# rvaser/rala

Hardware: AMD Instinct MI355X
Metric: overlaps/sec (pile build + transitive reduction) (higher is better)
Workload: dtype u16/u32 (+f64 compares)

## Files before the change

include/rala_hip.h:

```cpp
#ifndef RALA_HIP_H_
#define RALA_HIP_H_

#include <stddef.h>
#include <stdint.h>

#ifdef __cplusplus
extern "C" {
#endif

#define RALA_HIP_NO_READ 0xFFFFFFFFu

enum {
    RALA_HIP_OK = 0,
    RALA_HIP_EDEVICE = -1,
    RALA_HIP_EINVAL = -2,
    RALA_HIP_ECAPACITY = -3,
    RALA_HIP_EFILTERED = -4,
    RALA_HIP_ENOMEM = -5,
    RALA_HIP_ENOTAFILE = -6,
    RALA_HIP_ETOOLARGE = -7
};

enum { RALA_HIP_TYPE_X = 0, RALA_HIP_TYPE_A = 1, RALA_HIP_TYPE_B = 2, RALA_HIP_TYPE_AB = 3, RALA_HIP_TYPE_BA = 4 };

enum { RALA_HIP_MEM_HOST = 0, RALA_HIP_MEM_DEVICE = 1, RALA_HIP_MEM_HOST_ASYNC = 2 };

typedef struct rala_hip_ctx rala_hip_ctx;

typedef struct rala_hip_overlaps {
    const uint32_t* a_id;
    const uint32_t* b_id;
    const uint32_t* a_begin;
    const uint32_t* a_end;
    const uint32_t* b_begin;
    const uint32_t* b_end;
    const uint32_t* length;
    const uint8_t* strand;
} rala_hip_overlaps;

typedef struct rala_hip_timings {
    float dedupe_ms, bucket_ms, pile_ms, classify_ms, death_ms, finish_ms, tail_host_ms, tr_ms, total_ms;
    uint32_t pile_launches, death_rounds, pile_overflow_reads, pile_position_reads;
    uint32_t pile_unbounded_reads, pool_regrown;
    float repeats_ms;
} rala_hip_timings;

int rala_hip_create(int device, rala_hip_ctx** out);
void rala_hip_destroy(rala_hip_ctx* ctx);
const char* rala_hip_last_error(const rala_hip_ctx* ctx);
int rala_hip_set_option(rala_hip_ctx* ctx, const char* key, int64_t value);
void* rala_hip_stream(rala_hip_ctx* ctx);

int rala_hip_set_reads(rala_hip_ctx* ctx, const uint32_t* read_len, uint64_t n_reads);
int rala_hip_set_overlaps(rala_hip_ctx* ctx, const rala_hip_overlaps* ovl, uint64_t n, int mem);

typedef struct rala_hip_ingest_timings {
    float ship_ms;
    float tokenize_ms;
    uint64_t bytes, lines;
} rala_hip_ingest_timings;
int rala_hip_set_name_table(rala_hip_ctx* ctx, const void* buckets, uint64_t n_buckets, const char* arena, uint64_t arena_bytes);
int rala_hip_set_overlaps_from_paf(rala_hip_ctx* ctx, const char* path, int check_lengths, uint32_t threads,
                                   int64_t* length_error_read, int* irregular);
int rala_hip_set_overlaps_from_mhap(rala_hip_ctx* ctx, const char* path, int check_lengths, uint32_t threads,
                                    int64_t* length_error_read, int* irregular);
int rala_hip_get_ingest_timings(rala_hip_ctx* ctx, rala_hip_ingest_timings* out);
typedef struct rala_hip_inflate_timings {
    float inflate_ms;
    uint64_t compressed_bytes;
    uint64_t members;
} rala_hip_inflate_timings;
int rala_hip_get_inflate_timings(rala_hip_ctx* ctx, rala_hip_inflate_timings* out);
typedef struct rala_hip_gzip_timings {
    float find_ms;
    float decode_ms;
    float resolve_ms;
    uint64_t compressed_bytes;
    uint64_t text_bytes;
    uint64_t chunks;
    uint64_t chunks_with_candidate;
    uint64_t chunks_confirmed;
    uint64_t chunks_refuted;
    uint64_t max_wave_text_bytes;
} rala_hip_gzip_timings;
int rala_hip_get_gzip_timings(rala_hip_ctx* ctx, rala_hip_gzip_timings* out);
int rala_hip_gzip_head(const uint8_t* bytes, uint64_t n, uint64_t* deflate_off, int* valid);
int rala_hip_gzip_chain(const uint64_t* starts, const uint64_t* end_bit, const uint64_t* text, const uint32_t* next,
                        const uint32_t* status, const uint32_t* refuted, uint64_t n_chunks, uint64_t end, uint32_t isize, uint64_t cap,
                        uint64_t* n_jobs, uint64_t* start_bit, uint64_t* stop_bit, uint64_t* text_off, uint64_t* text_n,
                        rala_hip_gzip_timings* stats, int* valid);
int rala_hip_gzip_chain_members(const uint64_t* starts, const uint64_t* end_bit, const uint64_t* text, const uint32_t* next,
                                const uint32_t* status, const uint32_t* refuted, uint64_t n_chunks, const uint64_t* cand_header_off,
                                const uint64_t* cand_deflate_bit, const uint32_t* cand_prev_crc, const uint32_t* cand_prev_isize,
                                const uint64_t* cand_end_bit, const uint64_t* cand_text, const uint32_t* cand_next,
                                const uint32_t* cand_status, uint64_t n_cands, uint64_t file_n, uint32_t last_crc, uint32_t last_isize,
                                uint64_t cap, uint64_t* n_jobs, uint64_t* start_bit, uint64_t* stop_bit, uint64_t* text_off,
                                uint64_t* text_n, uint32_t* first, uint64_t member_cap, uint64_t* n_members, uint64_t* member_text_off,
                                uint64_t* member_text_n, uint32_t* member_crc32, rala_hip_gzip_timings* stats, int* valid);
int rala_hip_gzip_find_members(rala_hip_ctx* ctx, const uint8_t* bytes, uint64_t n, uint64_t cap, uint64_t* n_found, uint64_t* header_off,
                               uint64_t* deflate_off);
int rala_hip_get_gzip_members(rala_hip_ctx* ctx, uint64_t* n, uint64_t cap, uint64_t* text_off, uint64_t* text_n, uint32_t* crc32);
int rala_hip_bgzf_index(const uint8_t* bytes, uint64_t n, uint64_t block_bytes, uint64_t cap, uint64_t* n_members, uint64_t* file_off,
                        uint32_t* comp_bytes, uint32_t* text_bytes, uint64_t* text_off, int* valid);
int rala_hip_bgzf_index_range(const uint8_t* bytes, uint64_t n, uint64_t lo, uint64_t hi, uint64_t block_bytes, uint64_t cap,
                              uint64_t* n_members, uint64_t* file_off, uint32_t* comp_bytes, uint32_t* text_bytes, uint64_t* begin,
                              uint64_t* end, int* empty, int* valid);
int rala_hip_bgzf_pieces_chain(const uint64_t* begin, const uint64_t* end, const int* empty, uint32_t n_pieces, uint64_t file_bytes);
int rala_hip_index_sequences(rala_hip_ctx* ctx, const char* path, int format, uint32_t threads, uint64_t* n_records,
                             uint64_t* name_bytes, int* irregular);
int rala_hip_get_sequence_index(rala_hip_ctx* ctx, uint64_t* name_off, uint32_t* name_len, uint64_t* data_off,
                                uint64_t* data_span, uint32_t* length, char* names);
int rala_hip_get_sequence_timings(rala_hip_ctx* ctx, rala_hip_ingest_timings* out);
int rala_hip_build_name_table(rala_hip_ctx* ctx, uint64_t* n_buckets, uint64_t* n_distinct);
int rala_hip_get_name_table(rala_hip_ctx* ctx, void* buckets, char* arena, uint64_t* n_buckets, uint64_t* arena_bytes);
int rala_hip_copy_name_table(rala_hip_ctx* dst, rala_hip_ctx* src);
uint64_t rala_hip_name_hash(const char* p, uint64_t n);
typedef struct rala_hip_name_table_info {
    uint64_t names;
    uint64_t distinct;
    uint64_t n_buckets;
    uint32_t longest_probe;
    float device_ms;
} rala_hip_name_table_info;
int rala_hip_get_name_table_info(rala_hip_ctx* ctx, rala_hip_name_table_info* out);
int rala_hip_slice_sequences(rala_hip_ctx* ctx, const char* path, const uint64_t* wanted, uint64_t n_wanted, const uint64_t* base_off,
                             uint8_t* bases, uint32_t threads, int* irregular);
typedef struct rala_hip_sequence_slice_info {
    uint64_t windows;
    uint64_t max_window_text_bytes;
    uint64_t bases;
    float ship_ms;
    float kernel_ms;
    float gather_ms;
    float copy_ms;
} rala_hip_sequence_slice_info;
int rala_hip_get_sequence_slice_info(rala_hip_ctx* ctx, rala_hip_sequence_slice_info* out);
int rala_hip_set_bases(rala_hip_ctx* ctx, const uint8_t* bases, const uint64_t* base_off, uint64_t n_sources, int mem);
typedef struct rala_hip_span {
    uint32_t source, first, len, rc;
} rala_hip_span;
int rala_hip_spell(rala_hip_ctx* ctx, const rala_hip_span* spans, uint64_t n_spans, uint8_t* out, uint64_t out_bytes);
typedef struct rala_hip_spell_info {
    uint64_t sources, source_bytes;
    uint64_t spans, bytes;
    uint64_t windows, launches;
    float upload_ms;
    float kernel_ms;
    float copy_ms;
    uint32_t from_slice;
} rala_hip_spell_info;
int rala_hip_get_spell_info(rala_hip_ctx* ctx, rala_hip_spell_info* out);
uint32_t rala_hip_crc32_chain(const uint32_t* reg, const uint64_t* len, uint64_t n);
int rala_hip_tokenise_sensitive_paf(rala_hip_ctx* ctx, const char* path, uint64_t lo, uint64_t hi, uint32_t threads,
                                    rala_hip_overlaps* out, uint64_t* n, int* irregular);
int rala_hip_tokenise_sensitive(rala_hip_ctx* ctx, const char* path, int format, uint32_t part, uint32_t parts, uint32_t threads,
                                rala_hip_overlaps* out, uint64_t* n, uint64_t piece[3], int* irregular);
int rala_hip_get_overlap_columns(rala_hip_ctx* ctx, uint64_t* n, uint32_t* const cols[7], uint8_t* strand);

int rala_hip_initialize(rala_hip_ctx* ctx);
int rala_hip_construct(rala_hip_ctx* ctx, const rala_hip_overlaps* sens, uint64_t n_sens);
int rala_hip_find_repetitive_hills(rala_hip_ctx* ctx, uint64_t read, uint32_t begin, uint32_t end, uint16_t median,
                                   uint16_t p10, uint16_t dataset_median);
int rala_hip_remove_transitive_edges(rala_hip_ctx* ctx, uint32_t* n_pairs);
int rala_hip_tr_mark(rala_hip_ctx* ctx, uint32_t n_nodes, uint32_t n_edges, const uint32_t* src,
                     const uint32_t* dst, const uint32_t* len, uint8_t* marks, uint32_t* n_pairs);

int rala_hip_dedupe(rala_hip_ctx* ctx);
int rala_hip_emit_bound_tuples(rala_hip_ctx* ctx, uint64_t* tuples_dev);
int rala_hip_emit_bound_tuples_bucketed(rala_hip_ctx* ctx, uint32_t world, uint64_t* tuples_dev, uint64_t* counts);
int rala_hip_set_bound_tuples(rala_hip_ctx* ctx, const uint64_t* tuples, uint64_t n, int mem);
int rala_hip_bound_records_fit(const rala_hip_ctx* ctx, uint32_t world);
int rala_hip_emit_bound_records_bucketed(rala_hip_ctx* ctx, uint32_t world, uint64_t* records_dev, uint64_t* counts);
int rala_hip_set_bound_records(rala_hip_ctx* ctx, const uint64_t* records, uint64_t n, int mem);
int rala_hip_import_state(rala_hip_ctx* ctx, const uint8_t* valid, const uint32_t* begin, const uint32_t* end,
                          const uint16_t* median, const uint16_t* p10, const uint8_t* alive,
                          const uint64_t* pits_off, const uint32_t* pits_pairs, const uint32_t* pits_aux,
                          const uint64_t* hills_off, const uint32_t* hills_pairs);

typedef struct rala_hip_device_state {
    const uint32_t* begin;
    const uint32_t* end;
    const uint16_t* median;
    const uint16_t* p10;
    const uint8_t* alive;
    const uint32_t* n_pits;
    const uint32_t* n_hills;
    const uint32_t* slot;
    const void* pool;
    uint64_t pool_count;
    const uint8_t* valid;
} rala_hip_device_state;
int rala_hip_get_device_state(rala_hip_ctx* ctx, rala_hip_device_state* out);
int rala_hip_copy_device_state(rala_hip_ctx* ctx, const rala_hip_device_state* dst);
int rala_hip_import_state_device(rala_hip_ctx* ctx, const rala_hip_device_state* in);

enum { RALA_HIP_COMM_RCCL = 0, RALA_HIP_COMM_LOCAL = 1 };
typedef struct rala_hip_mg rala_hip_mg;
typedef struct rala_hip_mg_timings {
// ... 66 lines not shown
```

rala_amd/csrc/bucket_kernels.hip:

```cpp
#include <hip/hip_runtime.h>

#include <algorithm>

#include "device_utils.h"
#include "geom.h"
#include "kernels.h"
#include "scan_pass.h"

namespace rala_hip {

namespace {

constexpr uint32_t kInf = 0xFFFFFFFFu;
constexpr uint32_t kTile = 4096;
constexpr uint32_t kBlockP = 512;
constexpr uint32_t kPer = kTile / kBlockP;
constexpr uint32_t kL1Shift = 12;
constexpr uint32_t kL1Reads = 1u << kL1Shift;
constexpr uint32_t kGroupShift = 7;
constexpr uint32_t kGroupReads = 1u << kGroupShift;
constexpr uint32_t kGroupsPerPart = kL1Reads / kGroupReads;
constexpr uint32_t kKeyBits = 14;
constexpr uint32_t kCoordBits = 25;
constexpr uint32_t kCoordMax = (1u << kCoordBits) - 1u;
static_assert(kKeyBits + 2 * kCoordBits == 64, "a record is 8 bytes");

struct PartGeom {
    uint32_t shift, gpp, n_part;
};
inline PartGeom part_geom(uint32_t n_reads, const BucketTuning& bt) {
    uint32_t shift = kL1Shift;
    while (shift < kKeyBits && ((uint64_t)n_reads + (1u << shift) - 1) >> shift > 256) ++shift;
    if (bt.part_shift >= kL1Shift && bt.part_shift <= kKeyBits) shift = bt.part_shift;
    return PartGeom{shift, 1u << (shift - kGroupShift), (uint32_t)(((uint64_t)n_reads + (1u << shift) - 1) >> shift)};
}

constexpr uint32_t kCountWindow = 150u * 1024u / 4u;
inline uint32_t count_window(const BucketTuning& bt) { return bt.count_window ? bt.count_window : kCountWindow; }

__device__ __forceinline__ uint64_t pack_record(uint32_t b, uint32_t begin, uint32_t end) {
    return (uint64_t)(b & ((1u << kKeyBits) - 1u)) << (2 * kCoordBits) | (uint64_t)(begin < kCoordMax ? begin : kCoordMax) << kCoordBits |
           (uint64_t)(end < kCoordMax ? end : kCoordMax);
}
__device__ __forceinline__ uint32_t rec_key(uint64_t r) { return (uint32_t)(r >> (2 * kCoordBits)); }
__device__ __forceinline__ uint2 rec_events(uint64_t r, uint32_t shrink) {
    const uint32_t begin = (uint32_t)(r >> kCoordBits) & kCoordMax, end = (uint32_t)r & kCoordMax;
    return make_uint2((begin + shrink) << 1, ((end - shrink) << 1) | 1u);
}

__device__ __forceinline__ uint32_t segment_of(uint32_t key, bool active, uint32_t lane, uint32_t& leader) {
    const uint32_t prev = (uint32_t)__shfl_up((int)key, 1, 64);
    const bool prev_active = __shfl_up((int)active, 1, 64) != 0;
    const bool head = active && (lane == 0 || !prev_active || prev != key);
    const uint64_t heads = __ballot(head);
    const uint64_t act = __ballot(active);
    const uint64_t below = heads & ((lane == 63) ? ~0ull : ((2ull << lane) - 1ull));
    leader = below ? 63u - (uint32_t)__clzll((long long)below) : lane;
    const uint64_t after = (lane == 63) ? 0ull : ((heads | ~act) >> (lane + 1));
    const uint32_t len = after ? (uint32_t)__ffsll((unsigned long long)after) : (64u - lane);
    return head ? len : 0u;
}

constexpr uint32_t kBlockC = 1024;
constexpr uint32_t kCountPer = 8;
__global__ __launch_bounds__(kBlockC) void group_count_kernel(OvlSoA o, uint32_t n_reads, uint32_t g_lo, uint32_t n_groups, uint32_t* group_count) {
    extern __shared__ uint32_t s_hist[];
    for (uint32_t g = threadIdx.x; g < n_groups; g += kBlockC) s_hist[g] = 0;
    __syncthreads();
    constexpr uint32_t kC = kCountPer;
    const uint64_t last = o.n - 1;
    for (uint64_t i0 = (uint64_t)blockIdx.x * kBlockC * kC; i0 < o.n; i0 += (uint64_t)gridDim.x * kBlockC * kC) {
        uint32_t a[kC], b[kC];
#pragma unroll
        for (uint32_t u = 0; u < kC; ++u) {
            const uint64_t i = i0 + u * kBlockC + threadIdx.x;
            const uint64_t j = i < o.n ? i : last;
            a[u] = i < o.n ? __builtin_nontemporal_load(o.a_id + j) : kInf;
            b[u] = __builtin_nontemporal_load(o.b_id + j);
        }
#pragma unroll
        for (uint32_t u = 0; u < kC; ++u) {
            const uint32_t g = (b[u] >> kGroupShift) - g_lo;
            if (a[u] < n_reads && b[u] < n_reads && g < n_groups) atomicAdd(&s_hist[g], 1u);
        }
    }
    __syncthreads();
    for (uint32_t g = threadIdx.x; g < n_groups; g += kBlockC) {
        const uint32_t c = s_hist[g];
        if (c) atomicAdd(&group_count[g_lo + g], c);
    }
}

__device__ __forceinline__ void load4_ids(const uint32_t* p, uint64_t i0, uint64_t n, uint32_t (&out)[4]) {
    typedef uint32_t u32x4_t __attribute__((ext_vector_type(4)));
    if (i0 + 4 <= n) {
        const u32x4_t v = __builtin_nontemporal_load((const u32x4_t*)(p + i0));
        out[0] = v.x; out[1] = v.y; out[2] = v.z; out[3] = v.w;
    } else {
#pragma unroll
        for (uint32_t e = 0; e < 4; ++e) out[e] = i0 + e < n ? p[i0 + e] : kInf;
    }
}
constexpr uint32_t kCountVec = 2;
constexpr uint32_t kFlagStage = 512;
template <bool kShard>
__global__ __launch_bounds__(kBlockC) void group_count_dedupe_kernel(OvlSoA o, uint32_t n_reads, uint32_t n_groups, uint32_t* group_count,
                                                                     uint8_t* __restrict__ suspect, uint8_t* __restrict__ valid, uint32_t* list_pos,
                                                                     uint32_t* list_query, uint32_t list_cap, uint32_t* list_count,
                                                                     uint32_t world, uint32_t groups) {
    extern __shared__ uint32_t s_hist[];
    __shared__ uint32_t s_fpos[kFlagStage], s_fq[kFlagStage], s_fcnt, s_fbase;
    for (uint32_t g = threadIdx.x; g < n_groups; g += kBlockC) s_hist[g] = 0;
    if (threadIdx.x == 0) s_fcnt = 0;
    __syncthreads();
    const uint32_t lane = threadIdx.x & 63;
    auto mark = [&](uint32_t query, uint64_t at) {
        suspect[query] = 1;
        const uint32_t slot = atomicAdd(&s_fcnt, 1u);
        if (slot < kFlagStage) { s_fpos[slot] = (uint32_t)at; s_fq[slot] = query; }
    };
    constexpr uint64_t kTrip = (uint64_t)kBlockC * 4 * kCountVec;
    for (uint64_t c0 = (uint64_t)blockIdx.x * kTrip; c0 < o.n; c0 += (uint64_t)gridDim.x * kTrip) {
        uint32_t a[kCountVec][4], b[kCountVec][4];
#pragma unroll
        for (uint32_t u = 0; u < kCountVec; ++u) {
            const uint64_t i0 = c0 + ((uint64_t)u * kBlockC + threadIdx.x) * 4;
            load4_ids(o.a_id, i0, o.n, a[u]);
            load4_ids(o.b_id, i0, o.n, b[u]);
        }
#pragma unroll
        for (uint32_t u = 0; u < kCountVec; ++u) {
            const uint64_t i0 = c0 + ((uint64_t)u * kBlockC + threadIdx.x) * 4;
            uint32_t pa = (uint32_t)__shfl_up((int)a[u][3], 1, 64), pb = (uint32_t)__shfl_up((int)b[u][3], 1, 64);
            if (lane == 0 && i0 > 0 && i0 < o.n) { pa = o.a_id[i0 - 1]; pb = o.b_id[i0 - 1]; }
            bool have_prev = i0 > 0;
            uint32_t word = 0;
#pragma unroll
            for (uint32_t e = 0; e < 4; ++e) {
                const uint32_t x = a[u][e], y = b[u][e];
                const bool in = i0 + e < o.n;
                const bool ok = in && x < n_reads && y < n_reads;
                if (ok) {
                    if constexpr (kShard) {
                        atomicAdd(&s_hist[(x % world) * groups + ((x / world) >> kGroupShift)], 1u);
                        atomicAdd(&s_hist[(y % world) * groups + ((y / world) >> kGroupShift)], 1u);
                    } else {
                        if ((y >> kGroupShift) < n_groups) atomicAdd(&s_hist[y >> kGroupShift], 1u);
                    }
                }
                if (in && have_prev) {
                    const bool pok = pa < n_reads && pb < n_reads;
                    if (ok && pok) {
                        if (pa == x && y <= pb) mark(x, i0 + e);
                    } else {
                        if (x < n_reads) mark(x, i0 + e);
                        if (pa < n_reads) mark(pa, i0 + e - 1);
                    }
                }
                if (ok && x != y) word |= 1u << (8 * e);
                pa = x; pb = y; have_prev = true;
            }
            if (i0 + 4 <= o.n) *(uint32_t*)(valid + i0) = word;
            else for (uint32_t e = 0; e < 4 && i0 + e < o.n; ++e) valid[i0 + e] = (uint8_t)(word >> (8 * e));
        }
        __syncthreads();
        const uint32_t staged = s_fcnt;
        if (staged) {
            if (threadIdx.x == 0) s_fbase = staged > kFlagStage ? atomicOr(list_count, kDedupeListGivenUp) : atomicAdd(list_count, staged);
            __syncthreads();
            if (staged <= kFlagStage) {
                for (uint32_t k = threadIdx.x; k < staged; k += kBlockC) {
                    const uint32_t at = s_fbase + k;
                    if (at < list_cap) { list_pos[at] = s_fpos[k]; list_query[at] = s_fq[k]; }
                }
            }
            __syncthreads();
            if (threadIdx.x == 0) s_fcnt = 0;
            __syncthreads();
        }
    }
    for (uint32_t g = threadIdx.x; g < n_groups; g += kBlockC) {
        const uint32_t c = s_hist[g];
        if (c) atomicAdd(&group_count[g], c);
    }
}

__global__ __launch_bounds__(1024) void layout_kernel(const uint32_t* __restrict__ group_count, uint32_t n_part, uint32_t gpp,
                                                      uint32_t* __restrict__ group_base, uint32_t* __restrict__ group_cursor,
                                                      uint32_t* __restrict__ part_cursor, uint32_t* __restrict__ tile_part,
                                                      uint32_t* __restrict__ tile_lo, uint32_t* __restrict__ tile_hi, uint32_t* n_tiles) {
    __shared__ uint32_t tmp[1024 / 64 + 1];
    const uint32_t n = n_part * gpp;
    uint32_t carry = 0;
    for (uint32_t g0 = 0; g0 < n; g0 += 1024) {
        const uint32_t g = g0 + threadIdx.x;
        const uint32_t c = g < n ? group_count[g] : 0u;
        uint32_t tot;
        const uint32_t ex = block_scan_excl<1024>(c, OpAdd(), 0u, tmp, tot);
        if (g < n) {
            group_base[g] = carry + ex;
            group_cursor[g] = carry + ex;
            if (g % gpp == 0) part_cursor[g / gpp] = carry + ex;
        }
        carry += tot;
    }
    if (threadIdx.x == 0) group_base[n] = carry;
    __syncthreads();
    uint32_t tile_carry = 0;
    for (uint32_t p0 = 0; p0 < n_part; p0 += 1024) {
        const uint32_t p = p0 + threadIdx.x;
        const uint32_t lo = p < n_part ? group_base[p * gpp] : 0u;
        const uint32_t hi = p < n_part ? group_base[(p + 1u) * gpp] : 0u;
        const uint32_t tiles = (hi - lo + kTile - 1) / kTile;
        uint32_t ttot;
        const uint32_t tex = block_scan_excl<1024>(tiles, OpAdd(), 0u, tmp, ttot);
        for (uint32_t k = 0; k < tiles; ++k) {
            tile_part[tile_carry + tex + k] = p;
            tile_lo[tile_carry + tex + k] = lo + k * kTile;
            tile_hi[tile_carry + tex + k] = umin(hi, lo + (k + 1u) * kTile);
        }
        tile_carry += ttot;
    }
    if (threadIdx.x == 0) *n_tiles = tile_carry;
}

struct StageLds {
    uint64_t* stage;
    uint16_t* bin_of;
    uint32_t *hist, *off, *gbase;
    __device__ StageLds(unsigned char* base, uint32_t n_bins) {
        stage = (uint64_t*)base;
        bin_of = (uint16_t*)(stage + kTile);
        hist = (uint32_t*)(bin_of + kTile);
        off = hist + n_bins;
        gbase = off + n_bins;
    }
};
inline size_t stage_lds_bytes(uint32_t n_bins) { return (size_t)kTile * 10 + (size_t)n_bins * 12 + 16; }

__device__ __forceinline__ void stage_and_copy(StageLds& L, uint32_t n_bins, const uint64_t* rec, const uint32_t* bin, const bool* in,
                                               uint32_t* cursor, uint64_t* __restrict__ out, uint32_t* tmp) {
    for (uint32_t p = threadIdx.x; p < n_bins; p += kBlockP) L.hist[p] = 0;
    __syncthreads();
    uint32_t rank[kPer];
#pragma unroll
    for (uint32_t u = 0; u < kPer; ++u) rank[u] = in[u] ? atomicAdd(&L.hist[bin[u]], 1u) : 0u;
    __syncthreads();
    uint32_t carry = 0;
    for (uint32_t p0 = 0; p0 < n_bins; p0 += kBlockP) {
        const uint32_t p = p0 + threadIdx.x;
        const uint32_t c = p < n_bins ? L.hist[p] : 0u;
        uint32_t tot;
        const uint32_t ex = block_scan_excl<(int)kBlockP>(c, OpAdd(), 0u, tmp, tot);
        if (p < n_bins) {
            L.off[p] = carry + ex;
            L.gbase[p] = c ? atomicAdd(&cursor[p], c) : 0u;
        }
        carry += tot;
    }
    __syncthreads();
    const uint32_t total = carry;
#pragma unroll
    for (uint32_t u = 0; u < kPer; ++u) {
        if (in[u]) {
            const uint32_t at = L.off[bin[u]] + rank[u];
            L.stage[at] = rec[u];
            L.bin_of[at] = (uint16_t)bin[u];
        }
    }
    __syncthreads();
    for (uint32_t j = threadIdx.x; j < total; j += kBlockP) {
        const uint32_t p = L.bin_of[j];
        out[L.gbase[p] + (j - L.off[p])] = L.stage[j];
    }
}

__global__ __launch_bounds__(kBlockP) void l1_scatter_kernel(OvlSoA o, uint32_t n_reads, uint32_t n_part, uint32_t shift, uint32_t* part_cursor,
                                                             uint64_t* __restrict__ rec1, uint32_t* acount) {
    extern __shared__ __align__(16) unsigned char s_raw[];
    __shared__ uint32_t tmp[kBlockP / 64 + 1];
    StageLds L(s_raw, n_part);
    uint64_t rec[kPer];
    uint32_t bin[kPer];
    bool in[kPer];
    const uint32_t lane = threadIdx.x & 63;
    const uint64_t last = o.n - 1;
#pragma unroll
    for (uint32_t u = 0; u < kPer; ++u) {
        const uint64_t i = (uint64_t)blockIdx.x * kTile + u * kBlockP + threadIdx.x;
        const uint64_t j = i < o.n ? i : last;
        const uint32_t a = o.a_id[j], b = o.b_id[j];
        in[u] = i < o.n && a < n_reads && b < n_reads;
        rec[u] = pack_record(b, o.b_begin[j], o.b_end[j]);
        bin[u] = in[u] ? b >> shift : 0u;
        uint32_t leader;
        const uint32_t seg = segment_of(a, in[u], lane, leader);
        if (seg) atomicAdd(&acount[a], seg);
    }
    stage_and_copy(L, n_part, rec, bin, in, part_cursor, rec1, tmp);
}

__device__ __forceinline__ uint32_t bound_record_read(uint64_t r) { return (uint32_t)(r >> (2 * kBoundRecordCoordBits)); }

__global__ __launch_bounds__(kBlockC) void group_count_records_kernel(const uint64_t* __restrict__ records, uint64_t n, uint32_t n_reads,
                                                                      uint32_t g_lo, uint32_t n_groups, uint32_t* group_count) {
    extern __shared__ uint32_t s_hist[];
    for (uint32_t g = threadIdx.x; g < n_groups; g += kBlockC) s_hist[g] = 0;
    __syncthreads();
    constexpr uint32_t kC = kCountPer;
    for (uint64_t i0 = (uint64_t)blockIdx.x * kBlockC * kC; i0 < n; i0 += (uint64_t)gridDim.x * kBlockC * kC) {
        uint32_t key[kC];
#pragma unroll
        for (uint32_t u = 0; u < kC; ++u) {
            const uint64_t i = i0 + u * kBlockC + threadIdx.x;
            key[u] = i < n ? bound_record_read(__builtin_nontemporal_load(records + i)) : kInf;
        }
#pragma unroll
        for (uint32_t u = 0; u < kC; ++u) {
            const uint32_t g = (key[u] >> kGroupShift) - g_lo;
            if (key[u] < n_reads && g < n_groups) atomicAdd(&s_hist[g], 1u);
        }
    }
    __syncthreads();
    for (uint32_t g = threadIdx.x; g < n_groups; g += kBlockC) {
        const uint32_t c = s_hist[g];
        if (c) atomicAdd(&group_count[g_lo + g], c);
    }
}

__global__ __launch_bounds__(kBlockP) void l1_scatter_records_kernel(const uint64_t* __restrict__ records, uint64_t n, uint32_t n_reads,
                                                                     uint32_t n_part, uint32_t shift, uint32_t* part_cursor, uint64_t* __restrict__ rec1) {
    extern __shared__ __align__(16) unsigned char s_raw[];
    __shared__ uint32_t tmp[kBlockP / 64 + 1];
    StageLds L(s_raw, n_part);
    uint64_t rec[kPer];
    uint32_t bin[kPer];
    bool in[kPer];
    constexpr uint32_t kMask = (1u << kBoundRecordCoordBits) - 1u;
#pragma unroll
    for (uint32_t u = 0; u < kPer; ++u) {
        const uint64_t i = (uint64_t)blockIdx.x * kTile + u * kBlockP + threadIdx.x;
        const uint64_t r = i < n ? __builtin_nontemporal_load(records + i) : ~0ull;
        const uint32_t key = bound_record_read(r);
        in[u] = i < n && key < n_reads;
        rec[u] = pack_record(key, (uint32_t)(r >> kBoundRecordCoordBits) & kMask, (uint32_t)r & kMask);
        bin[u] = in[u] ? key >> shift : 0u;
    }
    stage_and_copy(L, n_part, rec, bin, in, part_cursor, rec1, tmp);
}

constexpr uint32_t kTileOtherBase = 0x80000000u;
__global__ __launch_bounds__(kBlockP) void l2_scatter_kernel(const uint64_t* __restrict__ rec1, const uint64_t* __restrict__ rec1b,
                                                             const uint32_t* __restrict__ tile_part,
                                                             const uint32_t* __restrict__ tile_lo, const uint32_t* __restrict__ tile_hi,
                                                             const uint32_t* __restrict__ n_tiles, uint32_t* group_cursor,
                                                             uint64_t* __restrict__ rec2, uint32_t gpp) {
    extern __shared__ __align__(16) unsigned char s_raw[];
    __shared__ uint32_t tmp[kBlockP / 64 + 1];
    if (blockIdx.x >= *n_tiles) return;
    StageLds L(s_raw, gpp);
    const uint32_t part_mask = gpp * kGroupReads - 1u;
    const uint32_t part_word = tile_part[blockIdx.x], lo = tile_lo[blockIdx.x], hi = tile_hi[blockIdx.x];
    const uint32_t part = part_word & ~kTileOtherBase;
    const uint64_t* __restrict__ src = (part_word & kTileOtherBase) ? rec1b : rec1;
    uint64_t rec[kPer];
    uint32_t bin[kPer];
    bool in[kPer];
#pragma unroll
    for (uint32_t u = 0; u < kPer; ++u) {
        const uint32_t j = lo + u * kBlockP + threadIdx.x;
        in[u] = j < hi;
        rec[u] = in[u] ? src[j] : 0ull;
        bin[u] = (rec_key(rec[u]) & part_mask) >> kGroupShift;
    }
    stage_and_copy(L, gpp, rec, bin, in, group_cursor + part * gpp, rec2, tmp);
}

__global__ __launch_bounds__(kGroupReads) void group_query_sum_kernel(const uint32_t* __restrict__ acount, uint32_t n_reads,
                                                                      uint32_t* __restrict__ qsum) {
    __shared__ uint32_t tmp[kGroupReads / 64 + 1];
    const uint32_t r = blockIdx.x * kGroupReads + threadIdx.x;
    const uint32_t v = block_reduce<(int)kGroupReads>(r < n_reads ? acount[r] : 0u, OpAdd(), 0u, tmp);
    if (threadIdx.x == 0) qsum[blockIdx.x] = v;
}

__global__ __launch_bounds__(1024) void group_event_base_kernel(const uint32_t* __restrict__ qsum, const uint32_t* __restrict__ group_base,
                                                                uint32_t n_groups, uint32_t* __restrict__ pair_base) {
    __shared__ uint32_t tmp[1024 / 64 + 1];
    uint32_t carry = 0;
    for (uint32_t g0 = 0; g0 < n_groups; g0 += 1024) {
        const uint32_t g = g0 + threadIdx.x;
        const uint32_t c = g < n_groups ? qsum[g] + (group_base[g + 1] - group_base[g]) : 0u;
        uint32_t tot;
        const uint32_t ex = block_scan_excl<1024>(c, OpAdd(), 0u, tmp, tot);
        if (g < n_groups) pair_base[g] = carry + ex;
        carry += tot;
    }
    if (threadIdx.x == 0) pair_base[n_groups] = carry;
}

__global__ __launch_bounds__(kBlockP) void final_kernel(const uint64_t* __restrict__ rec2, const uint32_t* __restrict__ group_base,
                                                        const uint32_t* __restrict__ pair_base, uint32_t n_reads,
                                                        const uint32_t* __restrict__ acount, uint32_t* __restrict__ ev_off,
                                                        uint32_t* __restrict__ ev, uint32_t shrink, uint32_t ev_shift) {
    extern __shared__ __align__(16) unsigned char s_raw[];
    __shared__ uint32_t tmp[kBlockP / 64 + 1];
    __shared__ uint32_t s_cursor[kGroupReads];
    __shared__ uint32_t s_cnt[kGroupReads];
    static_assert(kGroupReads <= kBlockP, "one thread per read of the group");
    StageLds L(s_raw, kGroupReads);
    const uint32_t g = blockIdx.x;
    if (threadIdx.x < kGroupReads) s_cnt[threadIdx.x] = 0;
    __syncthreads();
    const uint32_t lo = group_base[g], hi = group_base[g + 1];
    uint64_t first[kPer];
#pragma unroll
    for (uint32_t u = 0; u < kPer; ++u) {
        const uint32_t j = lo + u * kBlockP + threadIdx.x;
        first[u] = j < hi ? rec2[j] : 0ull;
        if (j < hi) atomicAdd(&s_cnt[rec_key(first[u]) & (kGroupReads - 1u)], 1u);
    }
    for (uint32_t j = lo + kTile + threadIdx.x; j < hi; j += kBlockP) atomicAdd(&s_cnt[rec_key(rec2[j]) & (kGroupReads - 1u)], 1u);
    __syncthreads();
    {
        const uint32_t r = g * kGroupReads + threadIdx.x;
        const bool mine = threadIdx.x < kGroupReads && r < n_reads;
        const uint32_t q = mine && acount ? acount[r] : 0u;
        const uint32_t pairs = mine ? q + s_cnt[threadIdx.x] : 0u;
        uint32_t tot;
        const uint32_t before = pair_base[g] + block_scan_excl<(int)kBlockP>(pairs, OpAdd(), 0u, tmp, tot);
        if (mine) {
            ev_off[r] = before << (1u - ev_shift);
            s_cursor[threadIdx.x] = before + q;
            if (r == n_reads - 1u) ev_off[n_reads] = (before + pairs) << (1u - ev_shift);
        }
    }
    __syncthreads();
    for (uint32_t j0 = lo; j0 < hi; j0 += kTile) {
        uint64_t pair[kPer];
        uint32_t bin[kPer];
        bool in[kPer];
#pragma unroll
        for (uint32_t u = 0; u < kPer; ++u) {
            const uint32_t j = j0 + u * kBlockP + threadIdx.x;
            in[u] = j < hi;
            const uint64_t rec = j0 == lo ? first[u] : in[u] ? rec2[j] : 0ull;
            const uint2 e = rec_events(rec, shrink);
            pair[u] = (uint64_t)e.x | (uint64_t)e.y << 32;
            bin[u] = rec_key(rec) & (kGroupReads - 1u);
        }
        stage_and_copy(L, kGroupReads, pair, bin, in, s_cursor, (uint64_t*)ev, tmp);
        __syncthreads();
    }
}

template <uint32_t kQ>
__global__ __launch_bounds__(256) void query_side_kernel(OvlSoA o, uint32_t n_reads, const uint32_t* __restrict__ ev_off,
                                                         uint32_t* written, uint32_t* __restrict__ ev, uint32_t ev_shift) {
    const uint32_t lane = threadIdx.x & 63;
    uint32_t a[kQ], b[kQ], begin[kQ], end[kQ];
#pragma unroll
    for (uint32_t u = 0; u < kQ; ++u) {
        const uint64_t i = ((uint64_t)blockIdx.x * kQ + u) * 256 + threadIdx.x;
        a[u] = kInf; b[u] = kInf; begin[u] = 0; end[u] = 0;
        if (i < o.n) { a[u] = o.a_id[i]; b[u] = o.b_id[i]; begin[u] = __builtin_nontemporal_load(o.a_begin + i); end[u] = __builtin_nontemporal_load(o.a_end + i); }
    }
    uint32_t base[kQ], leader[kQ];
    bool ok[kQ];
#pragma unroll
    for (uint32_t u = 0; u < kQ; ++u) {
        ok[u] = a[u] < n_reads && b[u] < n_reads;
        const uint32_t seg = segment_of(a[u], ok[u], lane, leader[u]);
        base[u] = 0;
        if (seg) base[u] = ev_off[a[u]] + atomicAdd(&written[a[u]], (2u >> ev_shift) * seg);
    }
#pragma unroll
    for (uint32_t u = 0; u < kQ; ++u) {
        const uint32_t at = (uint32_t)__shfl((int)base[u], (int)leader[u], 64);
        if (ok[u]) *(uint2*)(ev + ((size_t)at << ev_shift) + 2u * (lane - leader[u])) = make_uint2((begin[u] + 15u) << 1, ((end[u] - 15u) << 1) | 1u);
    }
}


__global__ __launch_bounds__(kBlockC) void shard_count_kernel(OvlSoA o, uint32_t n_reads, uint32_t world, uint32_t groups,
                                                              uint32_t n_bins, uint32_t* group_count) {
    extern __shared__ uint32_t s_hist[];
    for (uint32_t g = threadIdx.x; g < n_bins; g += kBlockC) s_hist[g] = 0;
    __syncthreads();
    constexpr uint32_t kC = kCountPer;
    const uint64_t last = o.n - 1;
    for (uint64_t i0 = (uint64_t)blockIdx.x * kBlockC * kC; i0 < o.n; i0 += (uint64_t)gridDim.x * kBlockC * kC) {
        uint32_t a[kC], b[kC];
#pragma unroll
        for (uint32_t u = 0; u < kC; ++u) {
            const uint64_t i = i0 + u * kBlockC + threadIdx.x;
            const uint64_t j = i < o.n ? i : last;
            a[u] = i < o.n ? __builtin_nontemporal_load(o.a_id + j) : kInf;
            b[u] = __builtin_nontemporal_load(o.b_id + j);
        }
#pragma unroll
        for (uint32_t u = 0; u < kC; ++u) {
            if (a[u] < n_reads && b[u] < n_reads) {
                atomicAdd(&s_hist[(a[u] % world) * groups + ((a[u] / world) >> kGroupShift)], 1u);
                atomicAdd(&s_hist[(b[u] % world) * groups + ((b[u] / world) >> kGroupShift)], 1u);
            }
        }
    }
    __syncthreads();
    for (uint32_t g = threadIdx.x; g < n_bins; g += kBlockC) {
        const uint32_t c = s_hist[g];
        if (c) atomicAdd(&group_count[g], c);
    }
}

__global__ __launch_bounds__(1024) void shard_send_layout_kernel(const uint32_t* __restrict__ group_count, ShardGeometry g,
                                                                 uint64_t* __restrict__ send, uint32_t* __restrict__ part_cursor,
                                                                 uint32_t* __restrict__ send_words) {
    __shared__ uint32_t tmp[1024 / 64 + 1];
    uint32_t block_start = 0;
    for (uint32_t p = 0; p < g.world; ++p) {
        uint32_t* header = (uint32_t*)(send + block_start);
        uint32_t carry = block_start + g.header;
        for (uint32_t g0 = 0; g0 < g.groups; g0 += 1024) {
            const uint32_t k = g0 + threadIdx.x;
            const uint32_t c = k < g.groups ? group_count[p * g.groups + k] : 0u;
            uint32_t tot;
            const uint32_t ex = block_scan_excl<1024>(c, OpAdd(), 0u, tmp, tot);
            if (k < g.groups) {
                header[k] = c;
                if (k % kGroupsPerPart == 0) part_cursor[p * g.n_part + k / kGroupsPerPart] = carry + ex;
            }
            carry += tot;
        }
        if (threadIdx.x == 0) send_words[p] = carry - block_start;
        block_start = carry;
    }
}

__global__ __launch_bounds__(kBlockP) void shard_l1_scatter_kernel(OvlSoA o, uint32_t n_reads, uint32_t world, uint32_t n_part,
                                                                   uint32_t* part_cursor, uint64_t* __restrict__ send) {
    extern __shared__ __align__(16) unsigned char s_raw[];
    __shared__ uint32_t tmp[kBlockP / 64 + 1];
    const uint32_t n_bins = world * n_part;
    StageLds L(s_raw, n_bins);
    uint64_t rec[kPer];
    uint32_t bin[kPer];
    bool in[kPer];
    const uint64_t last = o.n - 1;
    static_assert(kPer % 2 == 0, "two records per overlap");
#pragma unroll
    for (uint32_t u = 0; u < kPer / 2; ++u) {
        const uint64_t i = (uint64_t)blockIdx.x * (kTile / 2) + u * kBlockP + threadIdx.x;
        const uint64_t j = i < o.n ? i : last;
        const uint32_t a = o.a_id[j], b = o.b_id[j];
        const bool ok = i < o.n && a < n_reads && b < n_reads;
        const uint32_t la = a / world, lb = b / world;
        in[2 * u] = in[2 * u + 1] = ok;
        rec[2 * u] = pack_record(la, __builtin_nontemporal_load(o.a_begin + j), __builtin_nontemporal_load(o.a_end + j));
        rec[2 * u + 1] = pack_record(lb, __builtin_nontemporal_load(o.b_begin + j), __builtin_nontemporal_load(o.b_end + j));
        bin[2 * u] = ok ? (a - la * world) * n_part + (la >> kL1Shift) : 0u;
        bin[2 * u + 1] = ok ? (b - lb * world) * n_part + (lb >> kL1Shift) : 0u;
    }
    stage_and_copy(L, n_bins, rec, bin, in, part_cursor, send, tmp);
}

__global__ __launch_bounds__(1024) void shard_owner_layout_kernel(const uint64_t* __restrict__ base, const uint64_t* __restrict__ base_self,
                                                                  ShardBlocks blocks, ShardGeometry g,
                                                                  uint32_t* __restrict__ group_base, uint32_t* __restrict__ group_cursor,
                                                                  uint32_t* __restrict__ pair_pref, uint32_t* __restrict__ tile_part,
                                                                  uint32_t* __restrict__ tile_lo, uint32_t* __restrict__ tile_hi,
                                                                  uint32_t* n_tiles) {
    __shared__ uint32_t tmp[1024 / 64 + 1];
    auto header_of = [&](uint32_t p) { return (const uint32_t*)((p == blocks.self ? base_self : base) + blocks.off[p]); };
    uint32_t carry = 0;
    for (uint32_t g0 = 0; g0 < g.groups; g0 += 1024) {
        const uint32_t k = g0 + threadIdx.x;
        uint32_t c = 0;
        if (k < g.groups) {
            for (uint32_t p = 0; p < g.world; ++p) c += header_of(p)[k];
        }
        uint32_t tot;
        const uint32_t ex = block_scan_excl<1024>(c, OpAdd(), 0u, tmp, tot);
        if (k < g.groups) { group_base[k] = carry + ex; group_cursor[k] = carry + ex; }
        carry += tot;
    }
    if (threadIdx.x == 0) group_base[g.groups] = carry;
    const uint32_t n_pairs = g.world * g.n_part;
    uint32_t pcarry = 0;
    for (uint32_t j0 = 0; j0 < n_pairs; j0 += 1024) {
        const uint32_t j = j0 + threadIdx.x;
        uint32_t len = 0;
        if (j < n_pairs) {
            const uint32_t* header = header_of(j / g.n_part) + (j % g.n_part) * kGroupsPerPart;
            for (uint32_t k = 0; k < kGroupsPerPart; ++k) len += header[k];
        }
        uint32_t tot;
        const uint32_t ex = block_scan_excl<1024>(len, OpAdd(), 0u, tmp, tot);
        if (j < n_pairs) pair_pref[j] = pcarry + ex;
        pcarry += tot;
    }
    if (threadIdx.x == 0) pair_pref[n_pairs] = pcarry;
    __syncthreads();
    uint32_t tile_carry = 0;
    for (uint32_t j0 = 0; j0 < n_pairs; j0 += 1024) {
        const uint32_t j = j0 + threadIdx.x;
        uint32_t lo = 0, len = 0, tiles = 0;
        if (j < n_pairs) {
            const uint32_t p = j / g.n_part;
            len = pair_pref[j + 1] - pair_pref[j];
            lo = blocks.off[p] + g.header + (pair_pref[j] - pair_pref[p * g.n_part]);
            tiles = (len + kTile - 1) / kTile;
        }
        uint32_t ttot;
        const uint32_t tex = block_scan_excl<1024>(tiles, OpAdd(), 0u, tmp, ttot);
        for (uint32_t k = 0; k < tiles; ++k) {
            tile_part[tile_carry + tex + k] = (j % g.n_part) | (j / g.n_part == blocks.self ? kTileOtherBase : 0u);
            tile_lo[tile_carry + tex + k] = lo + k * kTile;
            tile_hi[tile_carry + tex + k] = umin(lo + len, lo + (k + 1u) * kTile);
        }
        tile_carry += ttot;
    }
    if (threadIdx.x == 0) *n_tiles = tile_carry;
}

}

uint32_t partition_count(uint32_t n_reads, const BucketTuning& bt) { return part_geom(n_reads, bt).n_part; }
uint32_t partition_group_slots(uint32_t n_reads, const BucketTuning& bt) { const PartGeom G = part_geom(n_reads, bt); return G.n_part * G.gpp + 2; }
size_t partition_records_needed(uint32_t, uint64_t n_overlaps) { return (size_t)n_overlaps + 64; }
size_t partition_tile_slots(uint32_t n_reads, uint64_t n_overlaps, const BucketTuning& bt) { return (size_t)(n_overlaps / kTile) + partition_count(n_reads, bt) + 4; }
bool partition_path_fits(uint32_t n_reads, uint32_t max_read_len, uint64_t n_overlaps, const BucketTuning& bt) {
    if (n_reads == 0 || n_overlaps == 0) return false;
    const PartGeom G = part_geom(n_reads, bt);
    const uint64_t n_part = G.n_part;
    return max_read_len < kCoordMax - 32u && n_part * G.gpp <= 8ull * kCountWindow &&
           stage_lds_bytes((uint32_t)n_part) <= 60u * 1024u && 2ull * n_overlaps < 0xFFFFFFF0ull && n_overlaps / n_part >= 512;
}

namespace {
struct PartitionBuffers {
    uint32_t n_part, n_groups, group_slots, shift, gpp, window;
    size_t tile_slots;
    uint32_t *group_count, *group_base, *group_cursor, *tile_part, *tile_lo, *tile_hi, *n_tiles;
    PartitionBuffers(uint32_t n_reads, uint64_t n_records, const BucketTuning& bt, uint32_t* group, uint32_t* tiles) {
        const PartGeom G = part_geom(n_reads, bt);
        n_part = G.n_part; shift = G.shift; gpp = G.gpp;
        window = std::min(n_part * gpp, count_window(bt));
        n_groups = (n_reads + kGroupReads - 1) / kGroupReads;
        group_slots = partition_group_slots(n_reads, bt);
        tile_slots = partition_tile_slots(n_reads, n_records, bt);
        group_count = group; group_base = group + group_slots; group_cursor = group + 2 * (size_t)group_slots;
        tile_part = tiles; tile_lo = tiles + tile_slots; tile_hi = tiles + 2 * tile_slots; n_tiles = tiles + 3 * tile_slots;
    }
};

hipError_t count_attribute(size_t lds_count) {
    if (lds_count + 8192 > 64 * 1024) {
        hipError_t e = hipFuncSetAttribute((const void*)group_count_kernel, hipFuncAttributeMaxDynamicSharedMemorySize, (int)lds_count);
        if (e == hipSuccess) e = hipFuncSetAttribute((const void*)group_count_dedupe_kernel<false>, hipFuncAttributeMaxDynamicSharedMemorySize, (int)lds_count);
        if (e == hipSuccess) e = hipFuncSetAttribute((const void*)group_count_records_kernel, hipFuncAttributeMaxDynamicSharedMemorySize, (int)lds_count);
        return e;
    }
    return hipSuccess;
}

void launch_partition_rest(const PartitionBuffers& B, uint32_t n_reads, const uint32_t* acount, const uint64_t* rec1, uint64_t* rec2,
                           uint32_t* ev_off, uint32_t* ev, hipStream_t s, uint32_t ev_shift, uint32_t shrink = 15u) {
    const uint32_t tiles2 = (uint32_t)(B.tile_slots - 4);
    hipLaunchKernelGGL(l2_scatter_kernel, dim3(tiles2), dim3(kBlockP), stage_lds_bytes(B.gpp), s, rec1, (const uint64_t*)nullptr,
                       (const uint32_t*)B.tile_part, (const uint32_t*)B.tile_lo, (const uint32_t*)B.tile_hi, (const uint32_t*)B.n_tiles,
                       B.group_cursor, rec2, B.gpp);
    uint32_t *qsum = B.group_count, *pair_base = B.group_cursor;
    hipLaunchKernelGGL(group_query_sum_kernel, dim3(B.n_groups), dim3(kGroupReads), 0, s, acount, n_reads, qsum);
    hipLaunchKernelGGL(group_event_base_kernel, dim3(1), dim3(1024), 0, s, (const uint32_t*)qsum, (const uint32_t*)B.group_base, B.n_groups,
                       pair_base);
    hipLaunchKernelGGL(final_kernel, dim3(B.n_groups), dim3(kBlockP), stage_lds_bytes(kGroupReads), s, (const uint64_t*)rec2,
                       (const uint32_t*)B.group_base, (const uint32_t*)pair_base, n_reads, acount, ev_off, ev, shrink, ev_shift);
}
}

bool bucket_count_can_dedupe(const OvlSoA& o, const uint8_t* valid) {
    return (((uintptr_t)o.a_id | (uintptr_t)o.b_id) & 15u) == 0 && ((uintptr_t)valid & 3u) == 0 && getenv("RALA_DEDUPE_APART") == nullptr;
}

hipError_t launch_bucket_partitioned(const OvlSoA& o, uint32_t n_reads, const BucketTuning& bt, uint32_t* acount, uint32_t* written,
                                     uint32_t* part_cursor, uint32_t* group, uint32_t* tiles, uint64_t* rec1, uint64_t* rec2,
                                     uint32_t* ev_off, uint32_t* ev, uint32_t workgroups, FillList& fills, hipStream_t s,
                                     const BucketDedupe* dedupe, uint32_t ev_shift) {
    const PartitionBuffers B(n_reads, o.n, bt, group, tiles);
    fills.add(acount, 0, (size_t)n_reads * 4);
    fills.add(written, 0, (size_t)n_reads * 4);
    fills.add(B.group_count, 0, (size_t)B.group_slots * 4);
    if (dedupe) fills.add(dedupe->suspect, 0, n_reads);
    hipError_t e = fills.launch(s);
    if (e != hipSuccess) return e;
    const uint32_t all_groups = B.n_part * B.gpp, window = B.window;
    const size_t lds_count = (size_t)window * 4;
    e = count_attribute(lds_count);
    if (e != hipSuccess) return e;
    const uint32_t chunks = (uint32_t)((o.n + kBlockC * kCountPer - 1) / (kBlockC * kCountPer));
    auto wait_for = [&](hipEvent_t ev) { return dedupe && ev ? hipStreamWaitEvent(s, ev, 0) : hipSuccess; };
    e = wait_for(dedupe ? dedupe->ids : nullptr);
    if (e != hipSuccess) return e;
    const uint32_t count_groups = (workgroups ? workgroups : 256u) * (2 * lds_count <= 150u * 1024u ? 2u : 1u);
    if (dedupe) {
        hipLaunchKernelGGL(group_count_dedupe_kernel<false>, dim3(std::min<uint32_t>(count_groups, chunks)), dim3(kBlockC), lds_count, s, o,
                           n_reads, window, B.group_count, dedupe->suspect, dedupe->valid, dedupe->list_pos,
                           dedupe->list_query, dedupe->list_cap, dedupe->list_count, 1u, 0u);
        if (dedupe->counted) {
            e = hipEventRecord(dedupe->counted, s);
            if (e != hipSuccess) return e;
        }
    } else {
        hipLaunchKernelGGL(group_count_kernel, dim3(std::min<uint32_t>(count_groups, chunks)), dim3(kBlockC), lds_count, s, o,
                           n_reads, 0u, window, B.group_count);
    }
    for (uint32_t g_lo = window; g_lo < all_groups; g_lo += window) {
        hipLaunchKernelGGL(group_count_kernel, dim3(std::min<uint32_t>(count_groups, chunks)), dim3(kBlockC), lds_count, s, o,
                           n_reads, g_lo, std::min(window, all_groups - g_lo), B.group_count);
    }
    hipLaunchKernelGGL(layout_kernel, dim3(1), dim3(1024), 0, s, (const uint32_t*)B.group_count, B.n_part, B.gpp, B.group_base, B.group_cursor,
                       part_cursor, B.tile_part, B.tile_lo, B.tile_hi, B.n_tiles);
    const uint32_t tiles1 = (uint32_t)((o.n + kTile - 1) / kTile);
    e = wait_for(dedupe ? dedupe->b_coords : nullptr);
    if (e != hipSuccess) return e;
    hipLaunchKernelGGL(l1_scatter_kernel, dim3(tiles1), dim3(kBlockP), stage_lds_bytes(B.n_part), s, o, n_reads, B.n_part, B.shift, part_cursor, rec1,
                       acount);
    launch_partition_rest(B, n_reads, acount, rec1, rec2, ev_off, ev, s, ev_shift);
    e = wait_for(dedupe ? dedupe->a_coords : nullptr);
    if (e != hipSuccess) return e;
    static const int q_per = getenv("RALA_QUERY_PER") ? atoi(getenv("RALA_QUERY_PER")) : 2;
    if (q_per == 4) hipLaunchKernelGGL(query_side_kernel<4>, dim3((uint32_t)((o.n + 1023) / 1024)), dim3(256), 0, s, o, n_reads, (const uint32_t*)ev_off, written, ev, ev_shift);
    else if (q_per == 2) hipLaunchKernelGGL(query_side_kernel<2>, dim3((uint32_t)((o.n + 511) / 512)), dim3(256), 0, s, o, n_reads, (const uint32_t*)ev_off, written, ev, ev_shift);
    else hipLaunchKernelGGL(query_side_kernel<1>, dim3((uint32_t)((o.n + 255) / 256)), dim3(256), 0, s, o, n_reads, (const uint32_t*)ev_off, written, ev, ev_shift);
    return hipGetLastError();
}

hipError_t launch_bucket_partitioned_records(const uint64_t* records, uint64_t n, uint32_t n_reads, const BucketTuning& bt, uint32_t* zero_counts,
                                             uint32_t* part_cursor, uint32_t* group, uint32_t* tiles, uint64_t* rec1, uint64_t* rec2,
                                             uint32_t* ev_off, uint32_t* ev, uint32_t workgroups, FillList& fills, hipStream_t s,
                                             uint32_t shrink, uint32_t ev_shift) {
    const PartitionBuffers B(n_reads, n, bt, group, tiles);
    fills.add(zero_counts, 0, (size_t)n_reads * 4);
    fills.add(B.group_count, 0, (size_t)B.group_slots * 4);
    hipError_t e = fills.launch(s);
    if (e != hipSuccess) return e;
    const uint32_t all_groups = B.n_part * B.gpp, window = B.window;
    const size_t lds_count = (size_t)window * 4;
    e = count_attribute(lds_count);
    if (e != hipSuccess) return e;
    const uint32_t chunks = (uint32_t)((n + kBlockC * kCountPer - 1) / (kBlockC * kCountPer));
    const uint32_t count_groups = (workgroups ? workgroups : 256u) * (2 * lds_count <= 150u * 1024u ? 2u : 1u);
    for (uint32_t g_lo = 0; g_lo < all_groups; g_lo += window) {
        hipLaunchKernelGGL(group_count_records_kernel, dim3(std::min<uint32_t>(count_groups, std::max<uint32_t>(chunks, 1u))), dim3(kBlockC),
                           lds_count, s, records, n, n_reads, g_lo, std::min(window, all_groups - g_lo), B.group_count);
    }
    hipLaunchKernelGGL(layout_kernel, dim3(1), dim3(1024), 0, s, (const uint32_t*)B.group_count, B.n_part, B.gpp, B.group_base, B.group_cursor,
                       part_cursor, B.tile_part, B.tile_lo, B.tile_hi, B.n_tiles);
    const uint32_t tiles1 = (uint32_t)((n + kTile - 1) / kTile);
    if (tiles1) {
        hipLaunchKernelGGL(l1_scatter_records_kernel, dim3(tiles1), dim3(kBlockP), stage_lds_bytes(B.n_part), s, records, n, n_reads,
                           B.n_part, B.shift, part_cursor, rec1);
    }
    launch_partition_rest(B, n_reads, zero_counts, rec1, rec2, ev_off, ev, s, ev_shift, shrink);
    return hipGetLastError();
}

bool partition_path_fits_records(uint32_t n_reads, uint32_t max_read_len, uint64_t n_records, const BucketTuning& bt) {
    return max_read_len < (1u << kBoundRecordCoordBits) - 32u && partition_path_fits(n_reads, max_read_len, (n_records + 1) / 2, bt);
}

ShardGeometry shard_geometry(uint64_t n_reads, uint32_t world) {
    ShardGeometry g;
    g.world = world;
    const uint64_t most = (n_reads + world - 1) / world;
    g.n_part = (uint32_t)std::max<uint64_t>(1, (most + kL1Reads - 1) / kL1Reads);
    g.groups = g.n_part * kGroupsPerPart;
    g.header = g.groups / 2;
    return g;
}
bool shard_path_fits(uint64_t n_reads, uint32_t max_read_len, uint32_t world) {
    if (n_reads == 0 || world == 0 || world > 64 || n_reads >= 0x7FFFFFFFull) return false;
    const ShardGeometry g = shard_geometry(n_reads, world);
    return max_read_len < kCoordMax - 32u && (uint64_t)g.world * g.groups * 4u <= 150u * 1024u &&
           stage_lds_bytes(g.world * g.n_part) <= 60u * 1024u;
}
size_t shard_send_words(const ShardGeometry& g, uint64_t n_overlaps) { return 2 * (size_t)n_overlaps + (size_t)g.world * g.header + 64; }
size_t shard_tile_slots(const ShardGeometry& g, uint64_t n_records) { return (size_t)(n_records / kTile) + (size_t)g.world * g.n_part + 4; }

hipError_t launch_shard_emit(const OvlSoA& o, uint32_t n_reads, const ShardGeometry& g, uint32_t* group_count, uint32_t* part_cursor,
                             uint64_t* send, uint32_t* send_words, uint32_t workgroups, FillList& fills, hipStream_t s,
                             const BucketDedupe* dedupe) {
    const uint32_t n_bins = g.world * g.groups;
    fills.add(group_count, 0, (size_t)n_bins * 4);
    if (dedupe) fills.add(dedupe->suspect, 0, n_reads);
    hipError_t e = fills.launch(s);
    if (e != hipSuccess) return e;
    const size_t lds_count = (size_t)n_bins * 4;
    if (lds_count + 8192 > 64 * 1024) {
        e = hipFuncSetAttribute((const void*)shard_count_kernel, hipFuncAttributeMaxDynamicSharedMemorySize, (int)lds_count);
        if (e == hipSuccess) e = hipFuncSetAttribute((const void*)group_count_dedupe_kernel<true>, hipFuncAttributeMaxDynamicSharedMemorySize, (int)lds_count);
        if (e != hipSuccess) return e;
    }
    if (o.n) {
        const uint32_t chunks = (uint32_t)((o.n + kBlockC * kCountPer - 1) / (kBlockC * kCountPer));
        const uint32_t count_groups = (workgroups ? workgroups : 256u) * (2 * lds_count <= 150u * 1024u ? 2u : 1u);
        if (dedupe) {
            hipLaunchKernelGGL(group_count_dedupe_kernel<true>, dim3(std::min<uint32_t>(count_groups, chunks)), dim3(kBlockC), lds_count, s, o,
                               n_reads, n_bins, group_count, dedupe->suspect, dedupe->valid, dedupe->list_pos, dedupe->list_query,
                               dedupe->list_cap, dedupe->list_count, g.world, g.groups);
            if (dedupe->counted) {
                e = hipEventRecord(dedupe->counted, s);
                if (e != hipSuccess) return e;
            }
        } else {
            hipLaunchKernelGGL(shard_count_kernel, dim3(std::min<uint32_t>(count_groups, chunks)), dim3(kBlockC), lds_count, s, o, n_reads,
                               g.world, g.groups, n_bins, group_count);
        }
    }
    hipLaunchKernelGGL(shard_send_layout_kernel, dim3(1), dim3(1024), 0, s, (const uint32_t*)group_count, g, send, part_cursor, send_words);
    if (o.n) {
        const uint32_t tiles1 = (uint32_t)((o.n + kTile / 2 - 1) / (kTile / 2));
        hipLaunchKernelGGL(shard_l1_scatter_kernel, dim3(tiles1), dim3(kBlockP), stage_lds_bytes(g.world * g.n_part), s, o, n_reads, g.world,
                           g.n_part, part_cursor, send);
    }
    return hipGetLastError();
}

hipError_t launch_bucket_from_blocks(const uint64_t* base, const uint64_t* base_self, const ShardBlocks& blocks, const ShardGeometry& g,
                                     uint32_t n_reads_local,
                                     uint64_t n_records, uint32_t* group, uint32_t* tiles, uint64_t* rec2, uint32_t* ev_off, uint32_t* ev,
                                     FillList& fills, hipStream_t s, uint32_t ev_shift) {
    hipError_t e = fills.launch(s);
    if (e != hipSuccess) return e;
    const uint32_t slots = g.groups + 2;
    uint32_t *group_base = group, *group_cursor = group + slots, *pair_pref = group + 2 * (size_t)slots;
    const size_t tile_slots = shard_tile_slots(g, n_records);
    uint32_t *tile_part = tiles, *tile_lo = tiles + tile_slots, *tile_hi = tiles + 2 * tile_slots, *n_tiles = tiles + 3 * tile_slots;
    hipLaunchKernelGGL(shard_owner_layout_kernel, dim3(1), dim3(1024), 0, s, base, base_self, blocks, g, group_base, group_cursor, pair_pref, tile_part,
                       tile_lo, tile_hi, n_tiles);
    hipLaunchKernelGGL(l2_scatter_kernel, dim3((uint32_t)(tile_slots - 4)), dim3(kBlockP), stage_lds_bytes(kGroupsPerPart), s, base, base_self,
                       (const uint32_t*)tile_part, (const uint32_t*)tile_lo, (const uint32_t*)tile_hi, (const uint32_t*)n_tiles, group_cursor,
                       rec2, kGroupsPerPart);
    const uint32_t n_groups = (n_reads_local + kGroupReads - 1) / kGroupReads;
    if (n_groups) {
        hipLaunchKernelGGL(final_kernel, dim3(n_groups), dim3(kBlockP), stage_lds_bytes(kGroupReads), s, (const uint64_t*)rec2,
                           (const uint32_t*)group_base, (const uint32_t*)group_base, n_reads_local, (const uint32_t*)nullptr, ev_off, ev, 15u, ev_shift);
    }
    return hipGetLastError();
}
size_t shard_group_words(const ShardGeometry& g) { return 3 * ((size_t)g.groups + 2) + (size_t)g.world * g.n_part + 2; }

}
```

rala_amd/csrc/context.h:

```cpp
#pragma once

#include <hip/hip_runtime.h>
#include <stdint.h>

#include <algorithm>

#include <memory>
#include <string>
#include <vector>

#include "geom.h"
#include "host_pool.h"
#include "kernels.h"
#include "rala_hip.h"

namespace rala_hip {

struct HostOvl {
    uint32_t src;
    uint32_t a, b;
    Coords c;
    uint8_t strand;
    uint8_t dead;
    uint8_t type;
// ... 15 lines not shown
    size_t reserved = 0, chunk_size = 0;
    ~DevBuf() { release(); }
    void release() {
        if (reserved) {
            (void)hipDeviceSynchronize();
            for (size_t i = 0; i < chunks.size(); ++i) {
                if (mapped[i]) (void)hipMemUnmap(mapped[i], chunk_size);
                (void)hipMemRelease(chunks[i]);
            }
            chunks.clear();
            mapped.clear();
            reserved = 0;
            chunk_size = 0;
        } else if (p) {
            (void)hipFree(p);
        }
        p = nullptr;
        n = 0;
    }
    hipError_t ensure_chunked(size_t count, size_t chunk_bytes, int order, int device, int64_t fail_at = -1) {
        if (count <= n && p) return hipSuccess;
        release();
        hipMemAllocationProp prop = {};
        prop.type = hipMemAllocationTypePinned;
        prop.location.type = hipMemLocationTypeDevice;
        prop.location.id = device;
        size_t gran = 0;
        hipError_t e = hipMemGetAllocationGranularity(&gran, &prop, hipMemAllocationGranularityRecommended);
        if (e != hipSuccess) return e;
        if (gran == 0) gran = 2u << 20;
        chunk_bytes = (chunk_bytes + gran - 1) / gran * gran;
        const size_t n_chunks = (count * sizeof(T) + chunk_bytes - 1) / chunk_bytes;
        const size_t bytes = n_chunks * chunk_bytes;
        void* base = nullptr;
        e = hipMemAddressReserve(&base, bytes, 0, nullptr, 0);
        if (e != hipSuccess) return e;
        p = (T*)base;
        reserved = bytes;
        chunk_size = chunk_bytes;
        size_t stride = 1;
        if (order == 1 && n_chunks > 2) {
            stride = (size_t)((double)n_chunks * 0.6180339887) | 1u;
            auto gcd = [](size_t a, size_t b) { while (b) { const size_t t = a % b; a = b; b = t; } return a; };
            while (gcd(stride, n_chunks) != 1) stride += 2;
        }
        for (size_t i = 0; i < n_chunks && e == hipSuccess; ++i) {
            hipMemGenericAllocationHandle_t h;
            if (fail_at >= 0 && (size_t)fail_at == i) { e = hipErrorOutOfMemory; break; }
            e = hipMemCreate(&h, chunk_bytes, &prop, 0);
            if (e != hipSuccess) break;
            chunks.push_back(h);
            mapped.push_back(nullptr);
            void* at = (char*)base + ((i * stride) % n_chunks) * chunk_bytes;
            e = hipMemMap(at, chunk_bytes, 0, h, 0);
            if (e == hipSuccess) mapped.back() = at;
        }
        if (e == hipSuccess) {
            hipMemAccessDesc acc = {};
            acc.location = prop.location;
            acc.flags = hipMemAccessFlagsProtReadWrite;
            e = hipMemSetAccess(base, bytes, &acc, 1);
        }
        if (e != hipSuccess) { release(); return e; }
        n = bytes / sizeof(T);
        return hipSuccess;
    }
    hipError_t ensure(size_t count) {
        if (count <= n && p) return hipSuccess;
        release();
        if (count == 0) count = 1;
        hipError_t e = hipMalloc((void**)&p, count * sizeof(T));
        if (e == hipSuccess) n = count;
        return e;
    }
    hipError_t copy_to_host(void* dst, size_t first, size_t count) const {
        const char* src = (const char*)(p + first);
        size_t left = count * sizeof(T);
        while (left) {
            size_t take = left;
            if (chunk_size) take = std::min(left, chunk_size - (size_t)(src - (const char*)p) % chunk_size);
            const hipError_t e = hipMemcpy(dst, src, take, hipMemcpyDeviceToHost);
            if (e != hipSuccess) return e;
            dst = (char*)dst + take; src += take; left -= take;
        }
        return hipSuccess;
    }
    hipError_t grow(size_t keep, size_t count) {
        if (count <= n && p) return hipSuccess;
        T* q = nullptr;
        const size_t want = count + count / 4 + 1;
        hipError_t e = hipMalloc((void**)&q, want * sizeof(T));
        if (e != hipSuccess) return e;
        if (keep && p) e = hipMemcpy(q, p, keep * sizeof(T), hipMemcpyDeviceToDevice);
        if (e != hipSuccess) { (void)hipFree(q); return e; }
        if (p) (void)hipFree(p);
        p = q;
        n = want;
        return hipSuccess;
    }
};

template <class T>
struct PinnedBuf {
    T* p = nullptr;
    size_t n = 0;
    ~PinnedBuf() { release(); }
    void release() {
        if (p) (void)hipHostFree(p);
        p = nullptr;
        n = 0;
    }
    hipError_t ensure(size_t count) {
        if (count <= n && p) return hipSuccess;
        release();
        if (count == 0) count = 1;
        count += count / 4;
        hipError_t e = hipHostMalloc((void**)&p, count * sizeof(T), hipHostMallocDefault);
        if (e == hipSuccess) n = count;
        return e;
    }
};

}

struct rala_hip_ctx {
    int device = 0;
    uint32_t n_compute_units = 256;
    hipStream_t stream = nullptr;
    hipStream_t side = nullptr;
    hipStream_t aux = nullptr;
    bool use_side_stream = true;
    std::string err;
    hipEvent_t ev[12] = {};
    hipStream_t copy = nullptr;
    hipEvent_t ev_up[4] = {};
    bool upload_pending = false, upload_queued = false;
    const uint32_t* up_src[7] = {};
    const uint8_t* up_strand = nullptr;

    int64_t pool_per_read_x1000 = 1000;
    int64_t max_lds_read_len = 22000;
    int64_t debug_pile_stop_after = 99;
    int64_t host_threads = 0;
    std::unique_ptr<rala_hip::HostPool> pool;
    bool use_run_kernel = true;
    bool debug_fail_construct = false;
    uint32_t debug_pile_variant = 0;
    uint32_t debug_dedupe_list_cap = 0;
    uint32_t debug_fp_lds_limit = 0xFFFFFFFFu;
    uint32_t debug_fp_give_up = 0;
    int64_t debug_chunk_fail = -1;
    uint32_t debug_part_shift = 0;
    uint32_t debug_count_window = 0;
    bool use_bound_records = true;
    bool use_round_batches = true;
    rala_hip::DevBuf<uint32_t> d_round_log;

    uint64_t n_reads = 0;
    uint32_t max_read_len = 0;
    uint32_t n_class[rala_hip::kPileClasses] = {};
    rala_hip::DevBuf<uint32_t> d_class_order;
    rala_hip::DevBuf<uint32_t> d_seg_base;
    rala_hip::DevBuf<uint32_t> d_dense;
    std::vector<uint32_t> h_read_len;
    std::vector<uint64_t> h_pile_off;
    uint64_t pile_elems = 0;
    rala_hip::DevBuf<uint32_t> d_read_len;
    rala_hip::DevBuf<uint64_t> d_pile_off;
    rala_hip::DevBuf<uint16_t> d_pile;
    rala_hip::DevBuf<uint32_t> d_order, d_overflow;
    rala_hip::DevBuf<uint32_t> d_big_list[2], d_big_space;
    int64_t debug_big_caps = 0;
    bool debug_force_big = false;
    rala_hip::DevBuf<uint16_t> d_slab;
    std::vector<rala_hip::LaunchClass> classes;

    rala_hip::DevBuf<uint8_t> d_name_buckets, d_name_arena, d_paf_text, d_paf_strand;
    uint64_t n_name_buckets = 0, n_name_arena_bytes = 0;
    rala_hip::DevBuf<uint32_t> d_name_stats;
    hipEvent_t ev_names[2] = {};
    rala_hip_name_table_info name_table_info = {};
    rala_hip::DevBuf<uint32_t> d_paf_col[7], d_paf_chunk[2], d_paf_win[7];
    rala_hip::DevBuf<uint8_t> d_paf_win_strand;
    int64_t ingest_window_bytes = 0;
    rala_hip::DevBuf<unsigned long long> d_paf_bad;
    rala_hip_ingest_timings ingest_tm = {};
    rala_hip::DevBuf<uint8_t> d_bgzf_comp, d_bgzf_jobs;
    rala_hip::DevBuf<uint32_t> d_bgzf_flag;
    rala_hip_inflate_timings inflate_tm = {};
    bool gzip_on_device = false;
    bool gzip_members = false;
    bool bgzf_in_pieces = false;
    int64_t gzip_chunk_bytes = 64 << 10;
    uint32_t debug_gzip_false_sync = 0;
    rala_hip::DevBuf<uint64_t> d_gzip_starts, d_gzip_off, d_gzip_floor;
    rala_hip::DevBuf<uint8_t> d_gzip_spans, d_gzip_jobs, d_gzip_text;
    rala_hip::DevBuf<uint16_t> d_gzip_sym;
    rala_hip::DevBuf<uint32_t> d_gzip_crc;
    rala_hip::DevBuf<uint32_t> d_gzip_tile, d_gzip_piece_crc;
    rala_hip::DevBuf<uint8_t> d_gzip_cands, d_gzip_mspans, d_gzip_pieces;
    std::vector<rala_hip::GzipMember> gzip_members_last;
    rala_hip_gzip_timings gzip_tm = {};
    int64_t debug_sequence_window = 0;
    rala_hip::DevBuf<uint64_t> d_seq_event[2], d_seq_name_pos, d_seq_data_off, d_seq_data_stripped, d_seq_name_off, d_seq_span;
    rala_hip::DevBuf<uint32_t> d_seq_name_len, d_seq_length, d_seq_tile[2], d_seq_name_at, d_seq_flags;
    rala_hip::DevBuf<uint8_t> d_seq_arena;
    uint64_t n_seq_records = 0, n_seq_name_bytes = 0;
    bool seq_index_valid = false;
    rala_hip_ingest_timings seq_tm = {};
    int seq_source = 0;
    bool seq_fastq = false;
    uint64_t seq_file_n = 0, seq_text_n = 0, seq_n_stripped = 0;
    std::vector<rala_hip::GzipJob> seq_gzip_chain;
    std::vector<rala_hip::GzipMember> seq_gzip_members;
    uint32_t seq_gzip_crc = 0;
    rala_hip::DevBuf<uint16_t> d_gzip_carry;
    rala_hip::DevBuf<uint8_t> d_gzip_hold, d_slice_out;
    rala_hip::DevBuf<uint64_t> d_slice_w[3];
    rala_hip_sequence_slice_info slice_info = {};
    bool keep_bases = false;
    uint32_t spell_window_mb = 256;
    int64_t debug_spell_window = 0;
    rala_hip::DevBuf<uint8_t> d_bases, d_spell_out;
    rala_hip::DevBuf<uint64_t> d_base_off, d_spell_off;
    rala_hip::DevBuf<rala_hip_span> d_spell_spans;
    std::vector<uint64_t> h_base_off;
    uint64_t n_base_sources = 0;
    bool bases_from_slice = false;
    rala_hip_spell_info spell_info = {};

    uint64_t n_ovl = 0;
    rala_hip::OvlSoA ovl = {};
    rala_hip::DevBuf<uint32_t> d_ovl_u32[7];
    rala_hip::DevBuf<uint8_t> d_ovl_strand;
    rala_hip::DevBuf<uint8_t> d_valid, d_suspect;
    rala_hip::DevBuf<uint32_t> d_dedupe_list;
    bool valid_ready = false;
    bool inputs_set = false;

    bool tuple_mode = false;
    uint64_t n_tuples = 0;
    const uint2* tuples = nullptr;
    const uint64_t* records = nullptr;
    uint64_t n_records = 0;
    rala_hip::DevBuf<uint64_t> d_record;
    rala_hip::DevBuf<uint2> d_tuple;
    rala_hip::DevBuf<uint32_t> d_owner_cnt;
    bool piles_resident = false;
    bool use_fused_emit = true;
    rala_hip::DevBuf<uint32_t> d_shard_group, d_shard_part, d_shard_words, d_shard_tiles;
    bool dedupe_pending = false;
    bool lists_pending = false;
    bool blocks_mode = false;
    const uint64_t* blocks_base = nullptr;
    const uint64_t* blocks_base_self = nullptr;
    rala_hip::ShardBlocks blocks = {};
    rala_hip::ShardGeometry shard_geom = {};
    uint64_t n_block_records = 0;

    rala_hip::DevBuf<uint32_t> d_ev_off, d_cursor, d_ev, d_slot_rank[2], d_ev_fixed;
    uint32_t pile_chunk_mb = 1024;
    uint32_t pile_rows = 1;
    uint32_t pile_rows_scratch_mb = 256;
    bool rowless = false;
    bool sens_csr_ready = false;
    bool sens_pass_running = false;
    uint64_t rows_materialised = 0;
    rala_hip::DevBuf<uint16_t> d_rows_scratch;
    rala_hip::DevBuf<uint64_t> d_rows_off;
    rala_hip::DevBuf<uint32_t> d_rows_list;
    std::vector<uint64_t> h_rows_off;
    bool debug_ev_events = false;
    uint32_t ev_shift = 0;
    rala_hip::DevBuf<unsigned char> d_scan_ws;

    rala_hip::DevBuf<uint32_t> d_begin, d_end, d_iv_slot;
    rala_hip::DevBuf<uint16_t> d_median, d_p10;
    rala_hip::DevBuf<uint8_t> d_alive;
    rala_hip::DevBuf<uint32_t> d_n_pits, d_n_hills;
    rala_hip::DevBuf<rala_hip::Interval> d_pool;
    rala_hip::DevBuf<uint32_t> d_small;
    uint32_t pool_cap = 0;
    uint32_t pool_cap_first = 0;
    uint32_t rep_pool_cap = 0;

    rala_hip::DevBuf<uint8_t> d_cls;
    rala_hip::DevBuf<uint32_t> d_death[2];
    rala_hip::DevBuf<uint32_t> d_chunk[4];
    rala_hip::DevBuf<uint4> d_rec;
    rala_hip::DevBuf<uint8_t> d_crec;
    rala_hip::DevBuf<uint8_t> d_fate;
    rala_hip::DevBuf<uint64_t> d_scan_state;
    rala_hip::DevBuf<uint32_t> d_counts;
    rala_hip::DevBuf<uint32_t> d_surv_u32[8];
    rala_hip::DevBuf<uint8_t> d_surv_u8[2];
    rala_hip::DevBuf<uint8_t> d_list_block[2];
    rala_hip::PinnedBuf<uint32_t> p_surv_u32[8];
    rala_hip::PinnedBuf<uint8_t> p_surv_u8[2];

    bool initialized = false, constructed = false;
    uint64_t n_prefiltered = 0;
    std::vector<uint32_t> h_begin, h_end, h_slot;
    std::vector<uint16_t> h_median, h_p10;
    std::vector<uint8_t> h_alive;
    std::vector<uint32_t> h_n_pits, h_n_hills;
    std::vector<rala_hip::Interval> h_pool;
    rala_hip::DevBuf<uint32_t> d_overflow_mid, d_overflow_long, d_chain_cnt;
    bool ev_ready = false, ev_fixed = false;
    rala_hip::DevBuf<uint32_t> d_sens_off, d_sens_cur, d_sens_ev, d_sens_list, d_sens_split;
    rala_hip::DevBuf<double> d_layout[4];
    rala_hip::DevBuf<uint32_t> d_layout_adj[2];
    rala_hip::DevBuf<unsigned char> d_layout_batch;
    rala_hip::PinnedBuf<unsigned char> p_layout_batch;
    hipEvent_t ev_layout[2] = {};
    int64_t layout_fused_max = 1024;
    rala_hip_layout_info layout_info = {};
    struct StagedCopy { void* dst; size_t offset, bytes; };
    rala_hip::PinnedBuf<uint32_t> p_stage;
    std::vector<StagedCopy> stage_pending;
    size_t stage_used = 0;
    int64_t use_fixed_buckets = 1;
    bool use_partitioned_buckets = true;
    rala_hip::DevBuf<uint32_t> d_bk_u32[3], d_bk_part, d_bk_group, d_bk_tiles;
    rala_hip::DevBuf<uint64_t> d_bk_rec[2];
    bool host_state_fresh = false;
    uint32_t pool_used = 0;

    rala_hip::DevBuf<uint16_t> d_dataset_median;
    rala_hip::DevBuf<uint32_t> d_n_rep;
    rala_hip::DevBuf<uint32_t> d_sens_col[7], d_sens_tb[2], d_sens_c[5];
    rala_hip::DevBuf<uint2> d_sens_tuples, d_sens_part, d_sens_recv;
    rala_hip::DevBuf<uint64_t> d_sens_rec;
    rala_hip::DevBuf<uint8_t> d_gather[2];
    rala_hip::DevBuf<uint8_t> d_sens_strand, d_sens_state;
    bool sens_in_device = false;
    rala_hip::DevBuf<uint32_t> d_rep_slot;
    rala_hip::DevBuf<rala_hip::Interval> d_rep_pool;
    std::vector<uint32_t> h_n_rep;
    std::vector<uint32_t> h_rep_slot;
    std::vector<rala_hip::Interval> h_rep_pool;
    bool have_repeats = false;
    bool rep_host_stale = false;
    uint32_t n_rep_hills = 0;

    bool use_gpu_tail = true;
    bool tail_on_device = false;
    bool host_stale = false;
    bool marks_on_device = false;
    uint32_t t_n0 = 0, t_n1 = 0, t_rounds = 0, t_n_kept = 0, t_n_nodes = 0, t_n_edges = 0, t_n_alive = 0;
    size_t t_med_tmp = 0;
    rala_hip::DevBuf<uint8_t> d_t_state, d_t_round, d_dirty, d_touched;
    rala_hip::DevBuf<uint32_t> d_n_pits0;
    rala_hip::DevBuf<uint16_t> d_cmed;
    rala_hip::DevBuf<uint8_t> d_med_tmp;
    rala_hip::DevBuf<uint32_t> d_cc_flags;
    rala_hip::DevBuf<uint32_t> d_kill[3], d_kill2[3], d_kill_count, d_death_sure;
    rala_hip::DevBuf<uint32_t> d_rank, d_alive_reads, d_t_tmp[2], d_kept_item, d_dovetail, d_epos, d_node_rank,
        d_node_read, d_e[3], d_t_death[2], d_t_work[2], d_t_fin, d_fp_map, d_fp_pack;
    rala_hip::DevBuf<uint8_t> d_t_mark;
    rala_hip::PinnedBuf<uint32_t> p_alive_reads, p_sens_rest;
    rala_hip::PinnedBuf<uint8_t> p_touched;
    rala_hip::PinnedBuf<uint16_t> p_cmed;

    std::vector<uint8_t> dirty, ever_dirty;
    std::vector<uint32_t> dirty_list;
    rala_hip::DevBuf<uint32_t> d_cc_edges, d_cc_label;
    rala_hip::DevBuf<uint32_t> d_tr[7];
    rala_hip::DevBuf<uint8_t> d_tr_marks;
    std::vector<rala_hip::HostOvl> overlaps, internals, scratch_ovl;
    std::vector<rala_hip::EdgePair> scratch_ep;
    std::vector<uint8_t> scratch_has, scratch_touched;
    std::vector<uint32_t> h_n_pits0;
    std::vector<uint32_t> scratch_u32a, scratch_u32b, scratch_u32c, alive_rank, alive_reads;
    rala_hip::PinnedBuf<uint32_t> p_cc_edges, p_cc_label;
    std::vector<uint32_t> node_read;
    std::vector<uint32_t> e_src, e_dst, e_len;
    std::vector<uint8_t> e_mark;

    rala_hip_timings tm = {};
};
```

rala_amd/csrc/context.hip:

```cpp
#include <hip/hip_runtime.h>
#include <stdlib.h>
#include <string.h>

#include <algorithm>
#include <thread>

#include "ctx_check.h"
#include "lifecycle.h"
#include "scan_pass.h"
#include "slots.h"
#include "stages.h"

using namespace rala_hip;

namespace {

int bound_inputs_adopted(rala_hip_ctx* ctx, Inputs kind, uint64_t n_events) {
    HIPCHECK(ctx->d_ev.ensure(n_events + 8));
    HIPCHECK(ctx->d_scan_ws.ensure(scan_workspace_bytes(std::max<uint64_t>(n_events, ctx->n_reads) + 2)));
    ctx->n_tuples = n_events;
    inputs_adopted(ctx, kind);
    return RALA_HIP_OK;
}

// ... 8 lines not shown
    hipStream_t s = ctx->stream;
    ctx->tm = rala_hip_timings();
    ctx->overlaps.clear(); ctx->internals.clear();
    uint32_t small[kInstallSmallWords] = {};
    small[kSmallPoolCount] = (uint32_t)pool_count;
    HIPCHECK(hipMemcpyAsync(ctx->d_small.p, small, sizeof(small), hipMemcpyHostToDevice, s));
    HIPCHECK(ctx->d_cc_flags.ensure(kCcFlagsWords));
    HIPCHECK(hipMemsetAsync(ctx->d_cc_flags.p + kCcInstallDead, 0, 4, s));
    launch_count_zero_u8(ctx->d_alive.p, (uint32_t)ctx->n_reads, ctx->d_cc_flags.p + kCcInstallDead, s);
    uint32_t n_dead = 0;
    HIPCHECK(d2h_small(ctx, &n_dead, ctx->d_cc_flags.p + kCcInstallDead, 4, s));
    HIPCHECK(stream_sync(ctx, s));
    results_dropped(ctx);
    state_installed(ctx, n_dead, (uint32_t)pool_count, false, false, valid_ready);
    if (n_dead == ctx->n_reads) return fail(ctx, RALA_HIP_EFILTERED, "filtered all sequences");
    return RALA_HIP_OK;
}

}

hipError_t rala_hip::d2h_small(rala_hip_ctx* ctx, void* dst, const void* src, size_t bytes, hipStream_t s) {
    if (ctx->p_stage.ensure(256) != hipSuccess || ctx->stage_used + bytes > 256 * sizeof(uint32_t) ||
        ctx->stage_pending.size() >= 16) {
        return hipMemcpyAsync(dst, src, bytes, hipMemcpyDeviceToHost, s);
    }
    char* at = (char*)ctx->p_stage.p + ctx->stage_used;
    const hipError_t e = hipMemcpyAsync(at, src, bytes, hipMemcpyDeviceToHost, s);
    if (e != hipSuccess) return e;
    ctx->stage_pending.push_back({dst, ctx->stage_used, bytes});
    ctx->stage_used += (bytes + 7) & ~(size_t)7;
    return hipSuccess;
}

hipError_t rala_hip::stream_sync(rala_hip_ctx* ctx, hipStream_t s) {
    const hipError_t e = hipStreamSynchronize(s);
    if (e == hipSuccess) {
        for (const auto& c : ctx->stage_pending) memcpy(c.dst, (const char*)ctx->p_stage.p + c.offset, c.bytes);
    }
    ctx->stage_pending.clear();
    ctx->stage_used = 0;
    return e;
}

int rala_hip::flush_upload(rala_hip_ctx* ctx) {
    if (!ctx->upload_pending) return RALA_HIP_OK;
    for (int k = 0; k < 7; ++k) HIPCHECK(hipMemcpy(ctx->d_ovl_u32[k].p, ctx->up_src[k], (size_t)ctx->n_ovl * 4, hipMemcpyHostToDevice));
    HIPCHECK(hipMemcpy(ctx->d_ovl_strand.p, ctx->up_strand, ctx->n_ovl, hipMemcpyHostToDevice));
    upload_done(ctx);
    return RALA_HIP_OK;
}

int rala_hip::set_bound_blocks(rala_hip_ctx* ctx, const uint64_t* base, const uint64_t* base_self, const ShardBlocks& blocks,
                               const ShardGeometry& g, uint64_t n_records) {
    if (!ctx) return RALA_HIP_EINVAL;
    if (ctx->n_reads == 0) return fail(ctx, RALA_HIP_EINVAL, "no reads set");
    if (n_records >= 0x7FFFFFF0ull) return fail(ctx, RALA_HIP_EINVAL, "too many records");
    HIPCHECK(hipSetDevice(ctx->device));
    inputs_withdrawn(ctx);
    ctx->blocks_base = base; ctx->blocks_base_self = base_self; ctx->blocks = blocks; ctx->shard_geom = g;
    ctx->n_block_records = n_records;
    return bound_inputs_adopted(ctx, Inputs::kBlocks, 2 * n_records);
}

int rala_hip::install_read_state(rala_hip_ctx* ctx, uint64_t pool_count) {
    if (!ctx) return RALA_HIP_EINVAL;
    if (ctx->n_reads == 0) return fail(ctx, RALA_HIP_EINVAL, "no reads set");
    if (ctx->n_ovl && !ctx->valid_ready) return fail(ctx, RALA_HIP_EINVAL, "validity bits required (rala_hip_dedupe)");
    if (pool_count > ctx->pool_cap) return fail(ctx, RALA_HIP_ECAPACITY, "interval pool smaller than the installed state");
    HIPCHECK(hipSetDevice(ctx->device));
    { const int rcu = flush_upload(ctx); if (rcu != RALA_HIP_OK) return rcu; }
    return finish_install(ctx, pool_count, ctx->valid_ready);
}

extern "C" {

int rala_hip_create(int device, rala_hip_ctx** out) {
    if (!out) return RALA_HIP_EINVAL;
    *out = nullptr;
    int count = 0;
    if (hipGetDeviceCount(&count) != hipSuccess || count <= 0 || device < 0 || device >= count) return RALA_HIP_EDEVICE;
    if (hipSetDevice(device) != hipSuccess) return RALA_HIP_EDEVICE;
    rala_hip_ctx* ctx = new rala_hip_ctx;
    ctx->device = device;
    if (const char* mb = getenv("RALA_HIP_PILE_CHUNK_MB")) ctx->pile_chunk_mb = (uint32_t)std::max(0, atoi(mb));
    {
        hipDeviceProp_t prop;
        if (hipGetDeviceProperties(&prop, device) == hipSuccess && prop.multiProcessorCount > 0) {
            ctx->n_compute_units = (uint32_t)prop.multiProcessorCount;
        }
    }
    int prio_least = 0, prio_greatest = 0;
    (void)hipDeviceGetStreamPriorityRange(&prio_least, &prio_greatest);
    bool ok = hipStreamCreate(&ctx->stream) == hipSuccess &&
              hipStreamCreateWithPriority(&ctx->side, hipStreamDefault, prio_greatest) == hipSuccess &&
              hipStreamCreate(&ctx->aux) == hipSuccess;
    for (auto& e : ctx->ev) ok = ok && hipEventCreate(&e) == hipSuccess;
    static_assert(sizeof(ctx->ev) / sizeof(ctx->ev[0]) == kEvCount, "one event per name of slots.h");
    ok = ok && ctx->d_small.ensure(kSmallWords) == hipSuccess;
    if (!ok) {
        rala_hip_destroy(ctx);
        return RALA_HIP_EDEVICE;
    }
    ctx->pool.reset(new HostPool(std::min(16u, std::max(1u, std::thread::hardware_concurrency()))));
    *out = ctx;
    return RALA_HIP_OK;
}

void rala_hip_destroy(rala_hip_ctx* ctx) {
    if (!ctx) return;
    (void)hipSetDevice(ctx->device);
    ctx->stage_pending.clear();
    if (ctx->stream) (void)hipStreamSynchronize(ctx->stream);
    if (ctx->side) (void)hipStreamSynchronize(ctx->side);
    if (ctx->aux) (void)hipStreamSynchronize(ctx->aux);
    for (auto& e : ctx->ev) if (e) (void)hipEventDestroy(e);
    for (auto& e : ctx->ev_up) if (e) (void)hipEventDestroy(e);
    for (auto& e : ctx->ev_layout) if (e) (void)hipEventDestroy(e);
    for (auto& e : ctx->ev_names) if (e) (void)hipEventDestroy(e);
    if (ctx->copy) (void)hipStreamDestroy(ctx->copy);
    if (ctx->side) (void)hipStreamDestroy(ctx->side);
    if (ctx->aux) (void)hipStreamDestroy(ctx->aux);
    if (ctx->stream) (void)hipStreamDestroy(ctx->stream);
    delete ctx;
}

const char* rala_hip_last_error(const rala_hip_ctx* ctx) { return ctx ? ctx->err.c_str() : "no context"; }

int rala_hip_set_option(rala_hip_ctx* ctx, const char* key, int64_t value) {
    if (!ctx || !key) return RALA_HIP_EINVAL;
    if (!strcmp(key, "interval_pool_per_read_x1000")) { ctx->pool_per_read_x1000 = value; return RALA_HIP_OK; }
    if (!strcmp(key, "debug_big_caps")) { ctx->debug_big_caps = value; return RALA_HIP_OK; }
    if (!strcmp(key, "debug_force_big")) { ctx->debug_force_big = value != 0; return RALA_HIP_OK; }
    if (!strcmp(key, "max_lds_read_len")) { ctx->max_lds_read_len = value; return RALA_HIP_OK; }
    if (!strcmp(key, "debug_pile_stop_after")) { ctx->debug_pile_stop_after = value; return RALA_HIP_OK; }
    if (!strcmp(key, "use_run_kernel")) { ctx->use_run_kernel = value != 0; return RALA_HIP_OK; }
    if (!strcmp(key, "use_round_batches")) { ctx->use_round_batches = value != 0; return RALA_HIP_OK; }
    if (!strcmp(key, "use_bound_records")) { ctx->use_bound_records = value != 0; return RALA_HIP_OK; }
    if (!strcmp(key, "use_fused_emit")) { ctx->use_fused_emit = value != 0; return RALA_HIP_OK; }
    if (!strcmp(key, "ingest_window_bytes")) { ctx->ingest_window_bytes = std::max<int64_t>(0, value); return RALA_HIP_OK; }
    if (!strcmp(key, "debug_sequence_window")) { ctx->debug_sequence_window = std::max<int64_t>(0, value); return RALA_HIP_OK; }
    if (!strcmp(key, "gzip_on_device")) { ctx->gzip_on_device = value != 0; return RALA_HIP_OK; }
    if (!strcmp(key, "gzip_members")) { ctx->gzip_members = value != 0; return RALA_HIP_OK; }
    if (!strcmp(key, "bgzf_in_pieces")) { ctx->bgzf_in_pieces = value != 0; return RALA_HIP_OK; }
    if (!strcmp(key, "gzip_chunk_bytes")) { ctx->gzip_chunk_bytes = value > 0 ? value : 64 << 10; return RALA_HIP_OK; }
    if (!strcmp(key, "debug_gzip_false_sync")) { ctx->debug_gzip_false_sync = (uint32_t)std::max<int64_t>(0, value); return RALA_HIP_OK; }
    if (!strcmp(key, "pile_rows")) { ctx->pile_rows = value ? 1u : 0u; return RALA_HIP_OK; }
    if (!strcmp(key, "pile_rows_scratch_mb")) { ctx->pile_rows_scratch_mb = (uint32_t)std::max<int64_t>(0, std::min<int64_t>(value, 1 << 20)); return RALA_HIP_OK; }
    if (!strcmp(key, "keep_bases")) { ctx->keep_bases = value != 0; return RALA_HIP_OK; }
    if (!strcmp(key, "spell_window_mb")) { ctx->spell_window_mb = (uint32_t)std::max<int64_t>(0, std::min<int64_t>(value, 1 << 20)); return RALA_HIP_OK; }
    if (!strcmp(key, "debug_spell_window")) { ctx->debug_spell_window = std::max<int64_t>(0, value); return RALA_HIP_OK; }
    if (!strcmp(key, "pile_chunk_mb")) { ctx->pile_chunk_mb = (uint32_t)std::max<int64_t>(0, std::min<int64_t>(value, 1 << 20)); return RALA_HIP_OK; }
    if (!strcmp(key, "debug_ev_events")) { ctx->debug_ev_events = value != 0; return RALA_HIP_OK; }
    if (!strcmp(key, "debug_count_window")) { ctx->debug_count_window = (uint32_t)std::max<int64_t>(0, value); return RALA_HIP_OK; }
    if (!strcmp(key, "debug_part_shift")) { ctx->debug_part_shift = (uint32_t)std::max<int64_t>(0, value); return RALA_HIP_OK; }
    if (!strcmp(key, "debug_pile_variant")) { ctx->debug_pile_variant = (uint32_t)std::max<int64_t>(0, value); return RALA_HIP_OK; }
    if (!strcmp(key, "debug_dedupe_list_cap")) { ctx->debug_dedupe_list_cap = (uint32_t)std::max<int64_t>(0, value); return RALA_HIP_OK; }
    if (!strcmp(key, "debug_fp_lds_limit")) { ctx->debug_fp_lds_limit = (uint32_t)std::max<int64_t>(0, value); return RALA_HIP_OK; }
    if (!strcmp(key, "debug_fp_give_up")) { ctx->debug_fp_give_up = value == 2 ? 2u : value != 0 ? 1u : 0u; return RALA_HIP_OK; }
    if (!strcmp(key, "debug_chunk_fail")) { ctx->debug_chunk_fail = value; return RALA_HIP_OK; }
    if (!strcmp(key, "debug_fail_construct")) { ctx->debug_fail_construct = value != 0; return RALA_HIP_OK; }
    if (!strcmp(key, "use_gpu_tail")) { ctx->use_gpu_tail = value != 0; return RALA_HIP_OK; }
    if (!strcmp(key, "use_fixed_buckets")) { ctx->use_fixed_buckets = value != 0; return RALA_HIP_OK; }
    if (!strcmp(key, "use_partitioned_buckets")) { ctx->use_partitioned_buckets = value != 0; return RALA_HIP_OK; }
    if (!strcmp(key, "use_side_stream")) { ctx->use_side_stream = value != 0; return RALA_HIP_OK; }
    if (!strcmp(key, "sensitive_in_device_memory")) { ctx->sens_in_device = value != 0; return RALA_HIP_OK; }
    if (!strcmp(key, "layout_fused_max")) {
        if (value < 0 || value > 1024) return fail(ctx, RALA_HIP_EINVAL, "layout_fused_max: 0 .. 1024");
        ctx->layout_fused_max = value;
        return RALA_HIP_OK;
    }
    if (!strcmp(key, "host_threads")) {
        ctx->host_threads = value;
        ctx->pool.reset(new HostPool((unsigned)std::max<int64_t>(1, std::min<int64_t>(value, 256))));
        return RALA_HIP_OK;
    }
    return fail(ctx, RALA_HIP_EINVAL, "unknown option");
}

void* rala_hip_stream(rala_hip_ctx* ctx) { return ctx ? (void*)ctx->stream : nullptr; }

int rala_hip_set_reads(rala_hip_ctx* ctx, const uint32_t* read_len, uint64_t n_reads) {
    if (!ctx || (!read_len && n_reads)) return RALA_HIP_EINVAL;
    if (n_reads >= 0x7FFFFFFFull) return fail(ctx, RALA_HIP_EINVAL, "too many reads");
    HIPCHECK(hipSetDevice(ctx->device));
    HIPCHECK(hipStreamSynchronize(ctx->side));
    HIPCHECK(hipStreamSynchronize(ctx->aux));
    ctx->n_reads = n_reads;
    ctx->h_read_len.assign(read_len, read_len + n_reads);
    ctx->max_read_len = 0;
    for (uint64_t r = 0; r < n_reads; ++r) ctx->max_read_len = std::max(ctx->max_read_len, read_len[r]);
    {
        uint32_t cnt[kPileClasses] = {};
        auto cls = [](uint32_t n) {
            uint32_t c = 0;
            while (c + 1 < kPileClasses && n > kPileClassBases[c]) ++c;
            return c;
        };
        for (uint64_t r = 0; r < n_reads; ++r) ++cnt[cls(read_len[r])];
        for (uint32_t c = 0; c < kPileClasses; ++c) ctx->n_class[c] = cnt[c];
        if (cnt[0] != n_reads) {
            std::vector<uint32_t> order(n_reads);
            uint32_t at[kPileClasses] = {};
            for (uint32_t c = 1; c < kPileClasses; ++c) at[c] = at[c - 1] + cnt[c - 1];
            for (uint64_t r = 0; r < n_reads; ++r) order[at[cls(read_len[r])]++] = (uint32_t)r;
            HIPCHECK(ctx->d_class_order.ensure(n_reads));
            HIPCHECK(hipMemcpy(ctx->d_class_order.p, order.data(), n_reads * 4, hipMemcpyHostToDevice));
        }
    }
    ctx->h_pile_off.resize(n_reads + 1);
    static const uint64_t row_align = [] {
        uint64_t want = getenv("RALA_PILE_ROW_ALIGN") ? (uint64_t)atoll(getenv("RALA_PILE_ROW_ALIGN")) : 64ull, a = 8;
        while (a * 2 <= want && a < (1ull << 20)) a *= 2;
        return a;
    }();
    uint64_t off = 0;
    for (uint64_t r = 0; r < n_reads; ++r) {
        ctx->h_pile_off[r] = off;
        off += ((uint64_t)read_len[r] + row_align - 1) & ~(row_align - 1);
    }
    ctx->h_pile_off[n_reads] = off;
    ctx->pile_elems = off;
    HIPCHECK(ctx->d_read_len.ensure(n_reads + 1));
    HIPCHECK(ctx->d_pile_off.ensure(n_reads + 1));
    ctx->d_pile.release();
    HIPCHECK(hipMemcpy(ctx->d_read_len.p, read_len, n_reads * 4, hipMemcpyHostToDevice));
    HIPCHECK(hipMemcpy(ctx->d_pile_off.p, ctx->h_pile_off.data(), (n_reads + 1) * 8, hipMemcpyHostToDevice));
    HIPCHECK(ctx->d_order.ensure(n_reads + 1));
    HIPCHECK(ctx->d_overflow.ensure(n_reads + 1));
    HIPCHECK(ctx->d_ev_off.ensure(n_reads + 2)); HIPCHECK(ctx->d_cursor.ensure(n_reads + 2));
    HIPCHECK(ctx->d_suspect.ensure(n_reads + 1));
    HIPCHECK(ctx->d_begin.ensure(n_reads)); HIPCHECK(ctx->d_end.ensure(n_reads));
    HIPCHECK(ctx->d_median.ensure(n_reads)); HIPCHECK(ctx->d_p10.ensure(n_reads));
    HIPCHECK(ctx->d_alive.ensure(n_reads)); HIPCHECK(ctx->d_n_pits.ensure(n_reads));
    HIPCHECK(ctx->d_n_hills.ensure(n_reads)); HIPCHECK(ctx->d_iv_slot.ensure(n_reads));
    HIPCHECK(ctx->d_death[0].ensure(n_reads)); HIPCHECK(ctx->d_death[1].ensure(n_reads));
    HIPCHECK(ctx->d_scan_ws.ensure(scan_workspace_bytes(std::max<uint64_t>(std::max(ctx->n_ovl, ctx->n_tuples), n_reads) + 2)));
    ctx->h_begin.resize(n_reads); ctx->h_end.resize(n_reads); ctx->h_median.resize(n_reads);
    ctx->h_p10.resize(n_reads); ctx->h_alive.resize(n_reads); ctx->h_n_pits.resize(n_reads);
    ctx->h_n_hills.resize(n_reads); ctx->h_slot.resize(n_reads);
    ctx->pool_cap = (uint32_t)std::max<int64_t>(ctx->pool_per_read_x1000 == 0 ? 16 : 1024, (int64_t)n_reads * ctx->pool_per_read_x1000 / 1000);
    ctx->pool_cap_first = ctx->pool_cap;
    ctx->rep_pool_cap = 0;
    HIPCHECK(ctx->d_pool.ensure(ctx->pool_cap));
    results_dropped(ctx);
    return RALA_HIP_OK;
}

int rala_hip_set_overlaps(rala_hip_ctx* ctx, const rala_hip_overlaps* o, uint64_t n, int mem) {
    if (!ctx || (!o && n)) return RALA_HIP_EINVAL;
    if (n >= 0xFFFFFFF0ull / 2) return fail(ctx, RALA_HIP_EINVAL, "too many overlaps for 32-bit bound offsets");
    HIPCHECK(hipSetDevice(ctx->device));
    HIPCHECK(hipStreamSynchronize(ctx->side));
    HIPCHECK(hipStreamSynchronize(ctx->aux));
    if (ctx->copy) HIPCHECK(hipStreamSynchronize(ctx->copy));
    inputs_withdrawn(ctx);
    upload_done(ctx);
    if (mem == RALA_HIP_MEM_HOST_ASYNC && !ctx->copy) {
        hipStream_t made = nullptr;
        HIPCHECK(hipStreamCreate(&made));
        hipError_t bad = hipSuccess;
        for (auto& e : ctx->ev_up) {
            e = nullptr;
            if (bad == hipSuccess) bad = hipEventCreateWithFlags(&e, hipEventDisableTiming);
        }
        if (bad != hipSuccess) {
            for (auto& e : ctx->ev_up) { if (e) (void)hipEventDestroy(e); e = nullptr; }
            (void)hipStreamDestroy(made);
            HIPCHECK(bad);
        }
        ctx->copy = made;
    }
    const uint32_t* src[7] = {nullptr, nullptr, nullptr, nullptr, nullptr, nullptr, nullptr};
    if (n) {
        src[0] = o->a_id; src[1] = o->b_id; src[2] = o->a_begin; src[3] = o->a_end;
        src[4] = o->b_begin; src[5] = o->b_end; src[6] = o->length;
    }
    const uint32_t* dev[7];
    const uint8_t* dev_strand;
    if (mem == RALA_HIP_MEM_DEVICE) {
        for (int k = 0; k < 7; ++k) dev[k] = src[k];
        dev_strand = n ? o->strand : nullptr;
    } else {
        const bool later = mem == RALA_HIP_MEM_HOST_ASYNC && n != 0;
        for (int k = 0; k < 7; ++k) {
            HIPCHECK(ctx->d_ovl_u32[k].ensure(n));
            if (n && !later) HIPCHECK(hipMemcpy(ctx->d_ovl_u32[k].p, src[k], n * 4, hipMemcpyHostToDevice));
            dev[k] = ctx->d_ovl_u32[k].p;
            ctx->up_src[k] = src[k];
        }
        HIPCHECK(ctx->d_ovl_strand.ensure(n));
        if (n && !later) HIPCHECK(hipMemcpy(ctx->d_ovl_strand.p, o->strand, n, hipMemcpyHostToDevice));
        dev_strand = ctx->d_ovl_strand.p;
        ctx->up_strand = n ? o->strand : nullptr;
        if (later) upload_deferred(ctx);
    }
    ctx->ovl.a_id = dev[0]; ctx->ovl.b_id = dev[1]; ctx->ovl.a_begin = dev[2]; ctx->ovl.a_end = dev[3];
    ctx->ovl.b_begin = dev[4]; ctx->ovl.b_end = dev[5]; ctx->ovl.length = dev[6]; ctx->ovl.strand = dev_strand;
    ctx->ovl.n = n;
    ctx->ovl.base = 0;
    HIPCHECK(ctx->d_valid.ensure(n));
    HIPCHECK(ctx->d_ev.ensure(4 * n + 8));
    HIPCHECK(ctx->d_cls.ensure(n / 4 + 64));
    for (int k = 0; k < 4; ++k) HIPCHECK(ctx->d_chunk[k].ensure(pass2_chunks(n) + 2));
    HIPCHECK(ctx->d_scan_ws.ensure(scan_workspace_bytes(std::max<uint64_t>(n, ctx->n_reads) + 2)));
    ctx->n_ovl = n;
    inputs_adopted(ctx, Inputs::kOverlaps);
// ... 164 lines not shown
```

rala_amd/csrc/kernels.h:

```cpp
#pragma once

#include <hip/hip_runtime.h>
#include <stdint.h>

#include "gzip_types.h"
#include "rala_hip.h"

namespace rala_hip {

constexpr uint32_t kPadL = 848;

enum : uint32_t {
    kErrRegionCapacity = 1u,
    kErrPoolCapacity = 2u,
    kErrRawCapacity = 4u,
};

struct Interval {
    uint32_t first, second;
    uint32_t aux;
};

struct PileArgs {
    const uint32_t* read_len;
// ... 168 lines not shown
                       hipStream_t s);
uint32_t pass2_chunks(uint64_t n_overlaps);
void launch_classify(const OvlSoA& o, uint32_t n_reads, const uint8_t* valid, const void* crec, bool small_records,
                     const KillList& kl, uint32_t* lo, hipStream_t s);
void launch_death_lower(const KillList& kl, uint32_t* lo, hipStream_t s, uint64_t at_most = ~0ull);
void launch_death_decide(const KillList& in, const uint32_t* lo, const uint32_t* up, uint32_t* sure, const KillList& out,
                         hipStream_t s, uint64_t at_most = ~0ull);
void launch_death_diff(uint32_t* older, const uint32_t* newer, uint32_t n, uint32_t* changed, hipStream_t s);
void launch_death_tighten(const uint32_t* sure, uint32_t* up, uint32_t* lo, uint32_t n, hipStream_t s, const uint32_t* count = nullptr,
                          uint32_t* status = nullptr);
void launch_survivor_masks(const OvlSoA& o, uint32_t n_reads, const uint8_t* valid, const uint8_t* fate, const uint32_t* death, const void* crec, bool small_records,
                           const uint4* rec, Interval* pool, uint64_t* mask_ov, uint64_t* mask_in, uint32_t* chunk_ov,
                           uint32_t* chunk_in, hipStream_t s);
void launch_apply_death(const uint32_t* death, uint8_t* alive, const uint32_t* n_hills, uint8_t* fate, uint32_t n_reads,
                        uint32_t* n_alive, hipStream_t s);

struct Survivors {
    uint32_t *src, *a_id, *b_id, *a_begin, *a_end, *b_begin, *b_end, *length;
    uint8_t *strand, *type;
};
void launch_gather_survivors(const OvlSoA& o, const uint64_t* mask_ov, const uint64_t* mask_in, const void* crec,
                             bool small_records, const uint32_t* chunk_ov_off, const uint32_t* chunk_in_off, uint32_t n_ov_total,
                             const Survivors& out, hipStream_t s);
struct ListBlocks {
    uint64_t block_off[64];
    uint32_t n0[64], n1[64];
    uint32_t dst0[64], dst1[64];
    uint32_t world;
};
struct RankOffsets {
    uint32_t v[64];
};
void launch_partition_tuples(const uint2* in, uint64_t n, uint32_t world, uint32_t pass, uint32_t* counters, uint2* out,
                             hipStream_t s);
void launch_localize_u32(const uint32_t* global, uint64_t n_local, uint32_t world, uint32_t rank, uint32_t* local, hipStream_t s);
void launch_localize_u16(const uint16_t* global, uint64_t n_local, uint32_t world, uint32_t rank, uint16_t* local, hipStream_t s);
void launch_localize_u8(const uint8_t* global, uint64_t n_local, uint32_t world, uint32_t rank, uint8_t* local, hipStream_t s);
void launch_pack_median(const uint16_t* median, const uint16_t* p10, uint64_t n_local, uint64_t nl_pad, uint32_t* out, hipStream_t s);
void launch_unpack_median(const uint32_t* all, uint32_t world, uint64_t nl_pad, uint64_t n_reads, uint16_t* median, uint16_t* p10,
                          hipStream_t s);
void launch_pack_rep(const uint32_t* n_rep, const uint32_t* rep_slot, uint64_t n_local, uint64_t nl_pad, uint64_t* out, hipStream_t s);
void launch_unpack_rep(const uint64_t* all, uint32_t world, uint64_t nl_pad, uint64_t n_reads, const RankOffsets& pool_base,
                       uint32_t* n_rep, uint32_t* rep_slot, hipStream_t s);
void launch_pool_aux(Interval* pool, uint32_t n, uint32_t* dense, uint32_t mode, hipStream_t s);
void launch_death_status(const uint32_t* count, uint32_t* status, hipStream_t s);
void launch_pack_killers(const uint32_t* key, const uint32_t* target, const uint32_t* keeper, const uint32_t* count, uint32_t each,
                         uint32_t* block, hipStream_t s);
void launch_unpack_killers(const uint32_t* blocks, uint32_t world, uint32_t each, uint32_t* key, uint32_t* target, uint32_t* keeper,
                           uint32_t* count, hipStream_t s);
void launch_hill_counts(const ReadState& rs, uint32_t n_reads, uint32_t* dense, uint32_t mode, hipStream_t s);
void launch_unpack_lists(const uint8_t* blocks, const ListBlocks& lb, const Survivors& out, hipStream_t s);

struct TailList {
    uint32_t n;
    uint32_t *src, *a, *b, *a_begin, *a_end, *b_begin, *b_end, *length;
    uint8_t *strand, *type;
    uint8_t* state;
    uint8_t* round;
};
struct TailReads {
    uint32_t *begin, *end;
    uint8_t *alive, *dirty;
    uint32_t *n_pits, *n_hills;
    const uint32_t* n_pits0;
    const uint32_t* iv_slot;
    Interval* pool;
};
void launch_sens_filter(const TailList& L, const uint32_t* begin, const uint32_t* end, const uint32_t* n_rep,
                        const uint32_t* rep_slot, const Interval* rep_pool, hipStream_t s);
void launch_finalize_states(const TailList& L, const uint8_t* alive, hipStream_t s);
void launch_list_targets(const uint32_t* off, uint32_t n, uint32_t* list, uint32_t* count, hipStream_t s);
void launch_list_members(const uint32_t* alive_reads, const uint8_t* touched, uint32_t n_alive, uint32_t world, uint32_t rank,
                         uint32_t* list, uint32_t* count, hipStream_t s);
struct SensSplitArgs {
    const uint32_t* read_len;
    const uint32_t* ev_off;
    const uint32_t* ev_cnt;
    uint32_t ev_stride;
    uint32_t ev_shift;
    const uint32_t* sens_off;
    const uint32_t* begin;
    const uint32_t* end;
    uint32_t* out[5];
    uint32_t* counts;
};
void launch_sens_split(const uint32_t* list, uint32_t bound, const uint32_t* n_dev, const SensSplitArgs& args, hipStream_t s);
void launch_status_clear(uint32_t* status, uint32_t bits, uint32_t* zero, hipStream_t s);
void launch_scatter_component_medians(const uint32_t* alive_reads, const uint8_t* touched, const uint16_t* cmed, uint32_t n_alive,
                                      uint16_t* out, hipStream_t s);
void launch_break_hills(const TailReads& R, uint32_t n_reads, hipStream_t s);
void launch_break_pits(const TailReads& R, const uint32_t* alive_reads, const uint8_t* touched, const uint16_t* comp_median,
                       uint32_t n_alive, hipStream_t s, const uint32_t* gate = nullptr);
void launch_retrim(const TailList& L, const TailReads& R, uint32_t promote, uint32_t round, uint32_t* dropped,
                   hipStream_t s, const uint32_t* gate = nullptr);
void launch_cc_edges(const TailList& L, const uint32_t* rank, uint32_t* edges, uint8_t* touched, uint32_t* label, uint32_t n_labels,
                     hipStream_t s);
void launch_refresh_types(const TailList& L, const TailReads& R, hipStream_t s);
hipError_t launch_tail_contain(const TailList& L, const TailReads& R, uint8_t* alive, uint32_t* const lists[6], uint32_t* zeroed21, uint32_t* const work[4],
                               uint32_t* base2, uint8_t* mark2, uint32_t* map, uint32_t* pack, uint32_t n_reads, uint32_t lds_limit, uint32_t debug_give_up, hipStream_t s);
void launch_count_zero_u8(const uint8_t* x, uint32_t n, uint32_t* out, hipStream_t s);
void launch_tail_init(const TailList& L, uint32_t n0, const TailReads& R, uint32_t* n_pits0, uint32_t n_reads, uint32_t* base2,
                      uint8_t* mark2, uint32_t* map, uint32_t* zero22, hipStream_t s);
struct ScanSpace;
bool launch_rank_pass(const uint8_t* alive, uint32_t* rank, uint32_t* alive_reads, uint32_t n_reads, ScanSpace& space, hipStream_t s);
bool launch_node_pass(const uint8_t* alive, uint32_t* node_rank, uint32_t* node_read, uint32_t* n_final, uint32_t n_reads,
                      ScanSpace& space, hipStream_t s);
bool launch_segment_pass(const TailList& L, const TailReads& R, uint32_t want_state, uint32_t want_round, uint32_t* base,
                         uint32_t* next, uint32_t* kept_item, const uint32_t* node_rank, uint32_t* e_src, uint32_t* e_dst,
                         uint32_t* e_len, ScanSpace& space, hipStream_t s);
bool launch_offsets_pass(const uint32_t* in, uint32_t* out, uint32_t* copy, uint32_t n, ScanSpace& space, hipStream_t s);
bool launch_pair_offsets_pass(const uint32_t* in0, const uint32_t* in1, uint32_t* out0, uint32_t* out1, uint32_t* totals, uint32_t n,
                              ScanSpace& space, hipStream_t s);

struct FixedPointList {
    const uint32_t *key, *target, *keeper;
    const uint32_t* count;
    uint32_t lds_limit = 0xFFFFFFFFu;
    uint32_t debug_give_up = 0;
};
size_t fixed_point_pack_words();
hipError_t launch_fixed_point_finish(const FixedPointList& list, uint32_t* base, uint32_t* map, uint32_t* pack, uint32_t* const work[4],
                                     uint32_t* sync8, uint32_t* error, uint32_t* rounds_out, hipStream_t s);

struct FillList {
    static constexpr uint32_t kMost = 8;
    void* ptr[kMost];
    size_t bytes[kMost];
    uint8_t value[kMost];
    uint32_t n = 0;
    bool overflow = false;
    void add(void* p, int byte, size_t n_bytes);
    hipError_t launch(hipStream_t s);
};

struct BucketTuning {
    uint32_t part_shift = 0;
    uint32_t count_window = 0;
};
size_t partition_records_needed(uint32_t n_reads, uint64_t n_overlaps);
uint32_t partition_count(uint32_t n_reads, const BucketTuning& bt);
uint32_t partition_group_slots(uint32_t n_reads, const BucketTuning& bt);
size_t partition_tile_slots(uint32_t n_reads, uint64_t n_overlaps, const BucketTuning& bt);
bool partition_path_fits(uint32_t n_reads, uint32_t max_read_len, uint64_t n_overlaps, const BucketTuning& bt);
constexpr uint32_t kDedupeListGivenUp = 0x80000000u;
struct BucketDedupe {
    uint8_t* suspect;
    uint8_t* valid;
    uint32_t* list_pos;
    uint32_t* list_query;
    uint32_t list_cap;
    uint32_t* list_count;
    hipEvent_t counted;
    hipEvent_t ids = nullptr, b_coords = nullptr, a_coords = nullptr;
};
bool bucket_count_can_dedupe(const OvlSoA& o, const uint8_t* valid);
constexpr uint32_t kBucketPairShift = 1;
hipError_t launch_bucket_partitioned(const OvlSoA& o, uint32_t n_reads, const BucketTuning& bt, uint32_t* acount, uint32_t* written,
                                     uint32_t* part_cursor, uint32_t* group, uint32_t* tiles, uint64_t* rec1, uint64_t* rec2,
                                     uint32_t* ev_off, uint32_t* ev, uint32_t workgroups, FillList& fills, hipStream_t s,
                                     const BucketDedupe* dedupe = nullptr, uint32_t ev_shift = kBucketPairShift);
void launch_dedupe_fix(const OvlSoA& o, uint32_t n_reads, const BucketDedupe& d, hipStream_t s);
bool partition_path_fits_records(uint32_t n_reads, uint32_t max_read_len, uint64_t n_records, const BucketTuning& bt);
hipError_t launch_bucket_partitioned_records(const uint64_t* records, uint64_t n, uint32_t n_reads, const BucketTuning& bt, uint32_t* zero_counts,
                                             uint32_t* part_cursor, uint32_t* group, uint32_t* tiles, uint64_t* rec1, uint64_t* rec2,
                                             uint32_t* ev_off, uint32_t* ev, uint32_t workgroups, FillList& fills, hipStream_t s,
                                             uint32_t shrink = 15u, uint32_t ev_shift = kBucketPairShift);

struct ShardGeometry {
    uint32_t world;
    uint32_t n_part;
    uint32_t groups;
    uint32_t header;
};
struct ShardBlocks {
    uint32_t off[64];
    uint32_t self;
};
ShardGeometry shard_geometry(uint64_t n_reads, uint32_t world);
bool shard_path_fits(uint64_t n_reads, uint32_t max_read_len, uint32_t world);
size_t shard_send_words(const ShardGeometry& g, uint64_t n_overlaps);
size_t shard_tile_slots(const ShardGeometry& g, uint64_t n_records);
size_t shard_group_words(const ShardGeometry& g);
hipError_t launch_shard_emit(const OvlSoA& o, uint32_t n_reads, const ShardGeometry& g, uint32_t* group_count, uint32_t* part_cursor,
                             uint64_t* send, uint32_t* send_words, uint32_t workgroups, FillList& fills, hipStream_t s,
                             const BucketDedupe* dedupe = nullptr);
hipError_t launch_bucket_from_blocks(const uint64_t* base, const uint64_t* base_self, const ShardBlocks& blocks, const ShardGeometry& g, uint32_t n_reads_local,
                                     uint64_t n_records, uint32_t* group, uint32_t* tiles, uint64_t* rec2, uint32_t* ev_off, uint32_t* ev,
                                     FillList& fills, hipStream_t s, uint32_t ev_shift = kBucketPairShift);

struct PafColumns {
    uint32_t *a_id, *b_id, *a_begin, *a_end, *b_begin, *b_end, *length;
    uint8_t* strand;
};
uint32_t paf_chunk_bytes();
uint32_t paf_halo_bytes();
void launch_paf_count(const uint8_t* text, uint64_t n, bool first_is_start, uint32_t* chunk_lines, hipStream_t s);
void launch_paf_parse(const uint8_t* text, uint64_t n, uint64_t n_avail, bool first_is_start, const uint32_t* chunk_row, const void* buckets,
                      uint64_t n_buckets, const char* arena, const uint32_t* read_len, uint32_t n_reads, bool check_lengths,
                      const PafColumns& out, uint32_t* flags, unsigned long long* first_bad, hipStream_t s, bool mhap = false);

void launch_name_table_build(const uint8_t* arena, const uint64_t* name_off, const uint32_t* name_len, uint32_t n, void* buckets,
                             uint64_t n_buckets, uint32_t* stats, hipStream_t s);

constexpr uint32_t kSeqNotFourLines = 1;
constexpr uint32_t kSeqLongName = 2;
constexpr uint32_t kSeqHeaderBeyondHalo = 4;
constexpr uint32_t kSeqTooLong = 16;
uint32_t sequence_tile_bytes();
uint32_t sequence_halo_bytes();
struct SequenceWindow {
    const uint8_t* text;
    uint64_t n, n_avail, text_off, text_n;
    uint32_t first_is_start;
    const uint32_t *tile_event0, *tile_stripped0;
    uint64_t event0, stripped0;
};
struct SequenceColumns {
    uint64_t *event_pos, *event_stripped;
    uint64_t* name_pos;
    uint32_t* name_len;
    uint64_t *data_off, *data_stripped;
};
void launch_sequence_count(const uint8_t* text, uint64_t n, bool first_is_start, bool fastq, uint32_t* tile_events, uint32_t* tile_stripped,
                           hipStream_t s);
void launch_sequence_records(const SequenceWindow& W, bool fastq, const SequenceColumns& out, uint32_t* flags, hipStream_t s);
void launch_sequence_names(const uint8_t* text, uint64_t text_off, const uint64_t* name_pos, const uint32_t* name_len, const uint32_t* name_at,
                           uint64_t n, uint64_t arena_off, uint8_t* arena, uint64_t* name_off, hipStream_t s);
void launch_sequence_finish(uint64_t n_records, uint64_t n_events, uint64_t text_n, uint64_t stripped_n, bool fastq, const SequenceColumns& c,
                            uint64_t* data_span, uint32_t* length, uint32_t* flags, hipStream_t s);
constexpr uint32_t kSeqSliceMismatch = 32;
struct SequenceGather {
    const uint8_t* text;
    uint64_t n, text_off;
    const uint32_t* tile_stripped0;
    uint64_t stripped0;
    const uint64_t *w_off, *w_end, *w_adj;
    uint64_t k_lo, k_hi;
    uint64_t out_lo, out_n;
    uint8_t* out;
    uint32_t* flags;
};
void launch_sequence_gather(const SequenceGather& G, hipStream_t s);

struct SpellArgs {
    const uint8_t* bases;
    const uint64_t* base_off;
    const rala_hip_span* spans;
    const uint64_t* out_off;
    uint32_t n_spans;
    uint64_t lo, hi;
    uint8_t* out;
};
uint32_t spell_tile_bytes();
void launch_spell(const SpellArgs& A, hipStream_t s);

struct BgzfJob {
    uint64_t comp_off, text_off;
    uint32_t deflate_len, isize;
};
void launch_bgzf_inflate(const uint8_t* comp, const BgzfJob* jobs, uint32_t n_jobs, uint8_t* text, uint64_t text_cap, uint32_t* flags,
                         hipStream_t s);

void launch_gzip_find(const uint8_t* comp, uint64_t end, uint64_t n_words, uint64_t deflate_off, uint64_t chunk_bytes, uint32_t n_chunks,
                      uint32_t false_sync, uint64_t* starts, hipStream_t s);
void launch_gzip_count(const uint8_t* comp, uint64_t end, const uint64_t* starts, uint32_t n_chunks, GzipSpan* spans, hipStream_t s,
                       const GzipMemberCand* cands = nullptr, uint32_t n_cands = 0, uint64_t deflate_off = 0, uint64_t chunk_bytes = 1,
                       GzipSpan* mspans = nullptr);
uint32_t gzip_member_tile_bytes();
void launch_gzip_member_count(const uint8_t* comp, uint64_t n, uint32_t* tile_count, hipStream_t s);
void launch_gzip_member_write(const uint8_t* comp, uint64_t n, const uint32_t* tile_first, GzipMemberCand* out, hipStream_t s);
void launch_gzip_piece_crc(const uint8_t* text, const GzipPiece* pieces, uint32_t n_pieces, uint32_t* reg, hipStream_t s);
void launch_gzip_write(const uint8_t* comp, uint64_t end, const GzipJob* jobs, uint32_t n_jobs, uint16_t* sym, uint32_t* flags, hipStream_t s);
void launch_gzip_resolve(uint16_t* sym, const uint64_t* text_off, const uint64_t* mfloor, uint32_t n_true, uint64_t text_n, uint8_t* text,
                         uint32_t* seg_crc, uint32_t* flags, hipStream_t s, uint64_t front = 0);
uint32_t gzip_segment_bytes();
uint32_t gzip_ring_symbols();
uint32_t gzip_crc_of_segments(const uint32_t* seg_crc, uint64_t text_n);
void launch_gzip_carry(uint16_t* sym, const uint8_t* text, uint64_t text_n, uint16_t* tmp, hipStream_t s);
uint32_t gzip_crc_register(const uint32_t* seg_crc, uint64_t text_n);
uint32_t gzip_crc_chain(const uint32_t* reg, const uint64_t* len, uint64_t n);
uint32_t gzip_crc_register_chain(const uint32_t* reg, const uint64_t* len, uint64_t n);

size_t scan_workspace_bytes(uint64_t n);
void launch_exclusive_scan(const uint32_t* in, uint32_t* out, uint64_t n, void* workspace, hipStream_t s);

void launch_tr_mark(const uint32_t* row_ptr, const uint32_t* adj_edge, const uint32_t* edge_src,
                    const uint32_t* edge_dst, const uint32_t* edge_len, uint32_t n_nodes, uint32_t first_edge,
                    uint32_t last_edge, uint8_t* marks, hipStream_t s);
void launch_tr_degree(const uint32_t* src, const uint32_t* dst, uint32_t n_nodes, uint32_t n_edges, uint32_t* deg,
                      uint32_t* bad, hipStream_t s);
void launch_tr_fill(const uint32_t* src, const uint32_t* dst, uint32_t n_nodes, uint32_t n_edges, uint32_t* cursor, uint32_t* adj,
                    hipStream_t s);
void launch_cc_init(uint32_t* label, uint32_t n, hipStream_t s);
void launch_cc_hook(const uint32_t* edges, uint32_t n_edges, uint32_t sample, uint32_t* label, uint32_t* changed,
                    hipStream_t s);
void launch_cc_compress(uint32_t* label, uint32_t n, hipStream_t s);
void launch_cc_compress_count(uint32_t* label, uint32_t n, const uint8_t* touched, uint32_t* size, hipStream_t s);
size_t component_median_workspace(uint32_t n);
void component_median_clear(void* tmp, uint32_t n, FillList& fills);
uint32_t* component_median_sizes(void* tmp, uint32_t n);
hipError_t launch_component_medians(const uint32_t* label, const uint8_t* touched, const uint32_t* alive_reads,
                                    const uint16_t* median, uint32_t n_alive, void* tmp, uint16_t* cmed, hipStream_t s);
void launch_tr_count(uint8_t* marks, uint32_t n_edges, uint32_t* n_pairs, hipStream_t s);

void launch_layout_step(uint32_t n, const double* x, const double* y, double* x_out, double* y_out,
                        const uint32_t* adj_off, const uint32_t* adj, double k, double t, hipStream_t s);
constexpr uint32_t kLayoutTile = 256;
void launch_layout_fused(uint32_t block, uint32_t n_list, const uint32_t* list, const uint32_t* comp_off, const double* x,
// ... 8 lines not shown
```

rala_amd/csrc/pipeline.hip:

```cpp
#include <hip/hip_runtime.h>
#include <stdio.h>
#include <stdlib.h>
#include <string.h>

#include <algorithm>
#include <chrono>
#include <numeric>

#include "ctx_check.h"
#include "lifecycle.h"
#include "scan_pass.h"
#include "slots.h"
#include "stages.h"

using namespace rala_hip;


int rala_hip::download_read_state(rala_hip_ctx* ctx) {
    const uint64_t n = ctx->n_reads;
    HIPCHECK(hipSetDevice(ctx->device));
    ctx->h_begin.resize(n); ctx->h_end.resize(n); ctx->h_median.resize(n); ctx->h_p10.resize(n);
    ctx->h_alive.resize(n); ctx->h_n_pits.resize(n); ctx->h_n_hills.resize(n); ctx->h_slot.resize(n);
    hipStream_t s = ctx->stream;
    HIPCHECK(hipMemcpyAsync(ctx->h_begin.data(), ctx->d_begin.p, n * 4, hipMemcpyDeviceToHost, s));
// ... 1802 lines not shown
    if (!ctx->constructed) return fail(ctx, RALA_HIP_EINVAL, "construct must succeed first");
    HIPCHECK(hipSetDevice(ctx->device));
    if (ctx->tail_on_device) {
        const int rc = tr_mark_device(ctx, ctx->t_n_nodes, ctx->t_n_edges, ctx->d_e[0].p, ctx->d_e[1].p, ctx->d_e[2].p, n_pairs, comm);
        marks_left_on_device(ctx, rc == RALA_HIP_OK);
        return rc;
    }
    const uint32_t ne = (uint32_t)ctx->e_src.size();
    ctx->e_mark.assign(ne, 0);
    return tr_mark_impl(ctx, (uint32_t)ctx->node_read.size(), ne, ctx->e_src.data(), ctx->e_dst.data(),
                        ctx->e_len.data(), ctx->e_mark.data(), n_pairs);
}

int rala_hip::shard_emit(rala_hip_ctx* ctx, const ShardGeometry& g, uint64_t* send, uint64_t* words) {
    if (!ctx || !send || !words) return RALA_HIP_EINVAL;
    if (ctx->n_reads == 0) return fail(ctx, RALA_HIP_EINVAL, "no reads set");
    if (!ctx->inputs_set || ctx->tuple_mode) return fail(ctx, RALA_HIP_EINVAL, "no overlaps set");
    HIPCHECK(hipSetDevice(ctx->device));
    { const int rcu = flush_upload(ctx); if (rcu != RALA_HIP_OK) return rcu; }
    hipStream_t s = ctx->stream;
    const uint32_t n_reads = (uint32_t)ctx->n_reads;
    const bool counted = ctx->use_side_stream && bucket_count_can_dedupe(ctx->ovl, ctx->d_valid.p);
    constexpr uint32_t kMarks = 1u << 20;
    BucketDedupe bd = {};
    if (counted) {
        HIPCHECK(ctx->d_dedupe_list.ensure(2 * (size_t)kMarks + 4));
        HIPCHECK(hipMemsetAsync(ctx->d_dedupe_list.p + 2 * (size_t)kMarks, 0, 4, s));
        bd.suspect = ctx->d_suspect.p; bd.valid = ctx->d_valid.p; bd.list_pos = ctx->d_dedupe_list.p; bd.list_query = ctx->d_dedupe_list.p + kMarks;
        bd.list_cap = ctx->debug_dedupe_list_cap ? std::min(kMarks, ctx->debug_dedupe_list_cap) : kMarks; bd.list_count = ctx->d_dedupe_list.p + 2 * (size_t)kMarks; bd.counted = ctx->ev[kEvEmitCounted];
    } else if (ctx->use_side_stream) {
        HIPCHECK(hipEventRecord(ctx->ev[kEvEmitCounted], s));
        HIPCHECK(hipStreamWaitEvent(ctx->side, ctx->ev[kEvEmitCounted], 0));
        launch_dedupe(ctx->ovl, n_reads, ctx->d_suspect.p, ctx->d_valid.p, ctx->side);
        HIPCHECK(hipEventRecord(ctx->ev[kEvEmitDedupeDone], ctx->side));
        dedupe_forked(ctx);
    } else {
        launch_dedupe(ctx->ovl, n_reads, ctx->d_suspect.p, ctx->d_valid.p, s);
    }
    validity_bits_ready(ctx);
    HIPCHECK(ctx->d_shard_group.ensure((size_t)g.world * g.groups + 2));
    HIPCHECK(ctx->d_shard_part.ensure((size_t)g.world * g.n_part + 2));
    HIPCHECK(ctx->d_shard_words.ensure(64));
    FillList fills;
    HIPCHECK(launch_shard_emit(ctx->ovl, n_reads, g, ctx->d_shard_group.p, ctx->d_shard_part.p, send, ctx->d_shard_words.p,
                               ctx->n_compute_units, fills, s, counted ? &bd : nullptr));
    if (counted && ctx->n_ovl) {
        HIPCHECK(hipStreamWaitEvent(ctx->side, ctx->ev[kEvEmitCounted], 0));
        launch_dedupe_fix(ctx->ovl, n_reads, bd, ctx->side);
        HIPCHECK(hipEventRecord(ctx->ev[kEvEmitDedupeDone], ctx->side));
        dedupe_forked(ctx);
    }
    uint32_t h[64];
    HIPCHECK(d2h_small(ctx, h, ctx->d_shard_words.p, g.world * 4, s));
    HIPCHECK(stream_sync(ctx, s));
    HIPCHECK(hipGetLastError());
    for (uint32_t p = 0; p < g.world; ++p) words[p] = h[p];
    return RALA_HIP_OK;
}

extern "C" {

static int initialize_stages(rala_hip_ctx* ctx);
int rala_hip_initialize(rala_hip_ctx* ctx) {
    if (!ctx) return RALA_HIP_EINVAL;
    const int rc = initialize_stages(ctx);
    if (ctx->upload_pending && ctx->copy) {
        (void)hipSetDevice(ctx->device);
        (void)hipStreamSynchronize(ctx->copy);
        if (ctx->upload_queued) upload_done(ctx);
    }
    ctx->upload_queued = false;
    return rc;
}
static int initialize_stages(rala_hip_ctx* ctx) {
    if (ctx->n_reads == 0) return fail(ctx, RALA_HIP_EINVAL, "no reads set");
    if (!ctx->inputs_set) return fail(ctx, RALA_HIP_EINVAL, "no overlaps or bound tuples set");
    HIPCHECK(hipSetDevice(ctx->device));
    hipStream_t s = ctx->stream;
    const uint32_t n_reads = (uint32_t)ctx->n_reads;
    ctx->tm = rala_hip_timings();
    ctx->overlaps.clear(); ctx->internals.clear();
    initialize_begun(ctx);
    ctx->rows_materialised = 0;
    if (ctx->rowless && ctx->debug_pile_stop_after != 99) {
        return fail(ctx, RALA_HIP_EINVAL, "debug_pile_stop_after is a diagnostic of the kernels that store rows: not with pile_rows = 0");
    }
    if (ctx->rowless) {
        ctx->d_pile.release();
    } else {
        static const char* chunk_order = getenv("RALA_HIP_PILE_CHUNK_ORDER");
        hipError_t ec = hipErrorNotSupported;
        if (ctx->pile_chunk_mb > 0 && (ctx->pile_elems + 8) * sizeof(uint16_t) >= ((size_t)ctx->pile_chunk_mb << 20)) {
            ec = ctx->d_pile.ensure_chunked(ctx->pile_elems + 8, (size_t)ctx->pile_chunk_mb << 20, chunk_order ? atoi(chunk_order) : 0, ctx->device,
                                            ctx->debug_chunk_fail);
            if (ec != hipSuccess) (void)hipGetLastError();
        }
        if (ec != hipSuccess) HIPCHECK(ctx->d_pile.ensure(ctx->pile_elems + 8));
    }
    HIPCHECK(hipEventRecord(ctx->ev[kEvAuxDrained], ctx->aux));
    HIPCHECK(hipStreamWaitEvent(s, ctx->ev[kEvAuxDrained], 0));
    HIPCHECK(hipEventRecord(ctx->ev[kEvInitBegin], s));
    const bool uploading = ctx->upload_pending;
    if (uploading) {
        const size_t n4 = (size_t)ctx->n_ovl * 4;
        auto up = [&](int k) { return hipMemcpyAsync(ctx->d_ovl_u32[k].p, ctx->up_src[k], n4, hipMemcpyHostToDevice, ctx->copy); };
        HIPCHECK(hipStreamWaitEvent(ctx->copy, ctx->ev[kEvInitBegin], 0));
        HIPCHECK(up(0)); HIPCHECK(up(1));
        HIPCHECK(hipEventRecord(ctx->ev_up[0], ctx->copy));
        HIPCHECK(up(4)); HIPCHECK(up(5));
        HIPCHECK(hipEventRecord(ctx->ev_up[1], ctx->copy));
        HIPCHECK(up(2)); HIPCHECK(up(3));
        HIPCHECK(hipEventRecord(ctx->ev_up[2], ctx->copy));
        HIPCHECK(up(6));
        HIPCHECK(hipMemcpyAsync(ctx->d_ovl_strand.p, ctx->up_strand, ctx->n_ovl, hipMemcpyHostToDevice, ctx->copy));
        HIPCHECK(hipEventRecord(ctx->ev_up[3], ctx->copy));
        ctx->upload_queued = true;
    }
    auto wait_for_all_columns = [&]() -> int {
        HIPCHECK(hipStreamWaitEvent(s, ctx->ev_up[3], 0));
        HIPCHECK(hipStreamWaitEvent(ctx->side, ctx->ev_up[3], 0));
        return (int)RALA_HIP_OK;
    };
    FillList fills;
    fills.add(ctx->d_small.p, 0, kSmallWords * 4);
    const bool forked = !ctx->tuple_mode && ctx->use_side_stream;
    if (uploading && !forked) {
        const int rcw = wait_for_all_columns();
        if (rcw != RALA_HIP_OK) return rcw;
    }
    if (!forked) {
        if (!ctx->tuple_mode) launch_dedupe(ctx->ovl, n_reads, ctx->d_suspect.p, ctx->d_valid.p, s);
        HIPCHECK(hipEventRecord(ctx->ev[kEvInitDedupeDone], s));
    }
    const uint32_t slot = kRunEventCapBig;
    const bool partition_allowed = ctx->use_fixed_buckets && ctx->use_partitioned_buckets;
    const BucketTuning bt = {ctx->debug_part_shift, ctx->debug_count_window};
    const bool from_records = ctx->tuple_mode && ctx->records != nullptr && partition_allowed &&
                              partition_path_fits_records(n_reads, ctx->max_read_len, ctx->n_records, bt);
    if (ctx->tuple_mode && ctx->records != nullptr && !from_records) {
        HIPCHECK(ctx->d_tuple.ensure(2 * ctx->n_records + 8));
        launch_records_to_tuples(ctx->records, ctx->n_records, ctx->d_tuple.p, s);
        ctx->tuples = ctx->d_tuple.p;
        ctx->n_tuples = 2 * ctx->n_records;
    }
    const bool from_blocks = ctx->tuple_mode && ctx->blocks_mode;
    const bool partitioned = from_blocks || from_records || (!ctx->tuple_mode && partition_allowed &&
                                                             partition_path_fits(n_reads, ctx->max_read_len, ctx->n_ovl, bt));
    if (!partitioned && !ctx->tuple_mode && ctx->n_ovl >= 0xFFFFFFF0ull / 4) {
        return fail(ctx, RALA_HIP_ETOOLARGE, "2^30 overlaps and more need the partitioned bucketing (its offsets count bound pairs); this input or these options rule it out");
    }
    const uint64_t n_bounds = from_blocks ? ctx->n_block_records : from_records ? ctx->n_records : 2 * ctx->n_ovl;
    const uint32_t ev_shift = !partitioned || (ctx->debug_ev_events && 2 * n_bounds < 0xFFFFFFF0ull) ? 0u : kBucketPairShift;
    bool fixed = !partitioned && ctx->use_run_kernel && ctx->use_fixed_buckets && (uint64_t)n_reads * slot * 4ull <= (64ull << 30);
    static const bool dedupe_late = getenv("RALA_DEDUPE_LATE") != nullptr;
    const bool dedupe_early = forked && partitioned && !dedupe_late;
    const bool dedupe_counted = dedupe_early && !from_records && !from_blocks && bucket_count_can_dedupe(ctx->ovl, ctx->d_valid.p);
    const bool fine_upload = uploading && dedupe_counted && partitioned;
    if (uploading && forked && !fine_upload) {
        const int rcw = wait_for_all_columns();
        if (rcw != RALA_HIP_OK) return rcw;
    }
    if (dedupe_early && !dedupe_counted) {
        HIPCHECK(hipStreamWaitEvent(ctx->side, ctx->ev[kEvInitBegin], 0));
        launch_dedupe(ctx->ovl, n_reads, ctx->d_suspect.p, ctx->d_valid.p, ctx->side);
        HIPCHECK(hipEventRecord(ctx->ev[kEvInitDedupeDone], ctx->side));
    }
    if (from_blocks) {
        const ShardGeometry& g = ctx->shard_geom;
        HIPCHECK(ctx->d_shard_group.ensure(shard_group_words(g)));
        HIPCHECK(ctx->d_shard_tiles.ensure(3 * shard_tile_slots(g, ctx->n_block_records) + 2));
        HIPCHECK(ctx->d_bk_rec[1].ensure((size_t)ctx->n_block_records + 64));
        HIPCHECK(launch_bucket_from_blocks(ctx->blocks_base, ctx->blocks_base_self, ctx->blocks, g, n_reads, ctx->n_block_records,
                                           ctx->d_shard_group.p, ctx->d_shard_tiles.p, ctx->d_bk_rec[1].p, ctx->d_ev_off.p, ctx->d_ev.p, fills, s, ev_shift));
    } else if (partitioned) {
        const uint64_t n_rec = from_records ? ctx->n_records : ctx->n_ovl;
        for (int k = 0; k < 3; ++k) HIPCHECK(ctx->d_bk_u32[k].ensure(n_reads + 2));
        HIPCHECK(ctx->d_bk_part.ensure(partition_count(n_reads, bt) + 2));
        HIPCHECK(ctx->d_bk_group.ensure(3 * (size_t)partition_group_slots(n_reads, bt)));
        HIPCHECK(ctx->d_bk_tiles.ensure(3 * partition_tile_slots(n_reads, n_rec, bt) + 2));
        for (int k = 0; k < 2; ++k) HIPCHECK(ctx->d_bk_rec[k].ensure(partition_records_needed(n_reads, n_rec)));
        if (from_records) {
            HIPCHECK(launch_bucket_partitioned_records(ctx->records, ctx->n_records, n_reads, bt, ctx->d_bk_u32[0].p, ctx->d_bk_part.p,
                                                       ctx->d_bk_group.p, ctx->d_bk_tiles.p, ctx->d_bk_rec[0].p, ctx->d_bk_rec[1].p,
                                                       ctx->d_ev_off.p, ctx->d_ev.p, ctx->n_compute_units, fills, s, 15u, ev_shift));
        } else {
            constexpr uint32_t kMarks = 1u << 20;
            if (dedupe_counted) HIPCHECK(ctx->d_dedupe_list.ensure(2 * (size_t)kMarks));
            BucketDedupe bd = {ctx->d_suspect.p, ctx->d_valid.p, ctx->d_dedupe_list.p, ctx->d_dedupe_list.p + kMarks,
                               ctx->debug_dedupe_list_cap ? std::min(kMarks, ctx->debug_dedupe_list_cap) : kMarks,
                               ctx->d_small.p + kInitDedupeMarks, ctx->ev[kEvBucketCounted]};
            if (fine_upload) { bd.ids = ctx->ev_up[0]; bd.b_coords = ctx->ev_up[1]; bd.a_coords = ctx->ev_up[2]; }
            HIPCHECK(launch_bucket_partitioned(ctx->ovl, n_reads, bt, ctx->d_bk_u32[0].p, ctx->d_bk_u32[2].p,
                                               ctx->d_bk_part.p, ctx->d_bk_group.p, ctx->d_bk_tiles.p, ctx->d_bk_rec[0].p,
                                               ctx->d_bk_rec[1].p, ctx->d_ev_off.p, ctx->d_ev.p, ctx->n_compute_units, fills, s,
                                               dedupe_counted ? &bd : nullptr, ev_shift));
            if (dedupe_counted) {
                HIPCHECK(hipStreamWaitEvent(ctx->side, ctx->ev[kEvBucketCounted], 0));
                if (fine_upload) HIPCHECK(hipStreamWaitEvent(ctx->side, ctx->ev_up[3], 0));
                launch_dedupe_fix(ctx->ovl, n_reads, bd, ctx->side);
                HIPCHECK(hipEventRecord(ctx->ev[kEvInitDedupeDone], ctx->side));
            }
        }
    }
    if (fixed) {
        HIPCHECK(ctx->d_ev_fixed.ensure((size_t)n_reads * slot + 8));
        HIPCHECK(ctx->d_cc_flags.ensure(kCcFlagsWords));
        fills.add(ctx->d_cursor.p, 0, (size_t)(n_reads + 1) * 4);
        HIPCHECK(fills.launch(s));
        if (ctx->tuple_mode) {
            launch_bucket_fixed_tuples(ctx->tuples, ctx->n_tuples, n_reads, slot, ctx->d_cursor.p,
                                       ctx->d_ev_fixed.p, ctx->d_small.p + kInitSlotOverflow, s);
        } else {
            launch_bucket_fixed(ctx->ovl, n_reads, slot, ctx->d_cursor.p, ctx->d_ev_fixed.p, ctx->d_small.p + kInitSlotOverflow, s);
        }
    }
    if (!fixed && !partitioned) {
    fills.add(ctx->d_cursor.p, 0, (size_t)(n_reads + 1) * 4);
    HIPCHECK(fills.launch(s));
    if (ctx->tuple_mode) {
        launch_count_tuples(ctx->tuples, ctx->n_tuples, n_reads, ctx->d_cursor.p, s);
    } else {
        HIPCHECK(ctx->d_slot_rank[0].ensure(ctx->n_ovl + 1)); HIPCHECK(ctx->d_slot_rank[1].ensure(ctx->n_ovl + 1));
        launch_count_bounds(ctx->ovl, n_reads, ctx->d_cursor.p, ctx->d_slot_rank[0].p, ctx->d_slot_rank[1].p, s);
    }
    launch_exclusive_scan(ctx->d_cursor.p, ctx->d_ev_off.p, n_reads, ctx->d_scan_ws.p, s);
    if (ctx->tuple_mode) {
        HIPCHECK(hipMemcpyAsync(ctx->d_cursor.p, ctx->d_ev_off.p, (size_t)n_reads * 4, hipMemcpyDeviceToDevice, s));
        launch_scatter_tuples(ctx->tuples, ctx->n_tuples, n_reads, ctx->d_cursor.p, ctx->d_ev.p, s);
    } else {
        launch_scatter_bounds(ctx->ovl, n_reads, ctx->d_ev_off.p, ctx->d_slot_rank[0].p, ctx->d_slot_rank[1].p, ctx->d_ev.p, s);
    }
    }
    HIPCHECK(hipEventRecord(ctx->ev[kEvInitBucketed], s));
    if (forked && !dedupe_early) {
        HIPCHECK(hipStreamWaitEvent(ctx->side, ctx->ev[kEvInitBucketed], 0));
        launch_dedupe(ctx->ovl, n_reads, ctx->d_suspect.p, ctx->d_valid.p, ctx->side);
        HIPCHECK(hipEventRecord(ctx->ev[kEvInitDedupeDone], ctx->side));
    }

    static_assert(slot == kRunEventCapBig, "pile_args' stride is the fixed slot");
    ctx->ev_shift = ev_shift;
    PileArgs a = pile_args(ctx, primary_events(ctx, fixed, ev_shift));
    a.rows_chunked = ctx->d_pile.reserved ? 1u : 0u;
    a.slab = ctx->d_slab.p;
    a.stop_after = (uint32_t)ctx->debug_pile_stop_after;
    a.variant = ctx->debug_pile_variant;
    a.alive = ctx->d_alive.p; a.n_pits = ctx->d_n_pits.p; a.n_hills = ctx->d_n_hills.p; a.iv_slot = ctx->d_iv_slot.p;
    a.pool = ctx->d_pool.p; a.pool_count = ctx->d_small.p + kInitPoolCount; a.pool_cap = ctx->pool_cap;
    a.error = ctx->d_small.p + kInitStatus;
    HIPCHECK(ctx->d_big_list[0].ensure(n_reads + 1));
    a.big_list = ctx->d_big_list[0].p; a.big_count = ctx->d_small.p + kInitNotedReads;
    a.force_big = ctx->debug_force_big ? 1u : 0u;
    if (ctx->use_run_kernel) {
        HIPCHECK(ctx->d_overflow_mid.ensure(n_reads + 1));
        HIPCHECK(ctx->d_dense.ensure(n_reads + 1));
        uint32_t* list_dense = ctx->d_dense.p;
        uint32_t* list1 = ctx->d_overflow.p;
        uint32_t* list2 = ctx->d_overflow_mid.p;
        uint32_t* list3 = ctx->d_order.p;
        uint32_t* cnt_dense = ctx->d_small.p + kInitDenseReads;
        uint32_t* cnt1 = ctx->d_small.p + kInitToCap1024;
        uint32_t* cnt2 = ctx->d_small.p + kInitToCap2048;
        uint32_t* cnt3 = ctx->d_small.p + kInitToPosition;
        const uint32_t n_short = ctx->n_class[0], n_medium = ctx->n_class[1], n_long = ctx->n_class[2];
        const uint32_t* by_class = n_short != n_reads ? ctx->d_class_order.p : nullptr;
        static const bool force_order = getenv("RALA_PILE_FORCE_ORDER") != nullptr;
        const bool short_by_list = by_class && (force_order || (uint64_t)(n_reads - n_short) * 8 > n_reads);
        static const bool no_aux = getenv("RALA_PILE_NO_AUX") != nullptr;
        hipStream_t aux = ctx->use_side_stream && !no_aux ? ctx->aux : s;
        if (aux != s) HIPCHECK(hipStreamWaitEvent(aux, ctx->ev[kEvInitBucketed], 0));
        a.lw = 0;
        a.skip_dense = 1;
        launch_pile_dense_list(a, n_reads, list_dense, cnt_dense, aux);
        a.order = list_dense;
        a.n_items = n_reads;
        a.n_items_dev = cnt_dense;
        launch_pile_runs(a, std::min<uint32_t>(n_reads, 8192), 1, list2, cnt2, aux);
        a.n_items_dev = nullptr;
        a.order = by_class ? by_class + n_short : nullptr;
        a.n_items = n_medium;
        static const int anylen_from = getenv("RALA_PILE_ANYLEN_FROM") ? atoi(getenv("RALA_PILE_ANYLEN_FROM")) : 3;
        launch_pile_runs(a, std::min<uint32_t>(n_medium, 16384), anylen_from <= 1 ? 4 : 3, list1, cnt1, aux);
        a.order = by_class ? by_class + n_short + n_medium : nullptr;
        a.n_items = n_long;
        launch_pile_runs(a, std::min<uint32_t>(n_long, 20480), 4, list1, cnt1, aux);
        if (aux != s) HIPCHECK(hipEventRecord(ctx->ev[kEvPileAuxDone], aux));
        a.order = short_by_list ? by_class : nullptr;
        a.n_items = short_by_list ? n_short : n_reads;
        launch_pile_runs(a, a.n_items, 0, list1, cnt1, s);
        if (aux != s) HIPCHECK(hipStreamWaitEvent(s, ctx->ev[kEvPileAuxDone], 0));
        a.n_items = n_reads;
        a.order = list1;
        a.n_items_dev = cnt1;
        launch_pile_runs(a, std::min<uint32_t>(n_reads, 8192), 1, list2, cnt2, s);
        a.order = list2;
        a.n_items_dev = cnt2;
        launch_pile_runs(a, std::min<uint32_t>(n_reads, 2048), 2, list3, cnt3, s);
        a.order = list3;
        a.n_items_dev = cnt3;
        const uint32_t max_len = ctx->max_read_len;
        const bool in_lds = (int64_t)max_len <= ctx->max_lds_read_len && pile_lw_for(max_len) <= 24576;
        a.lw = pile_lw_for(max_len);
        const uint32_t grid = std::min<uint32_t>(n_reads, 256);
        if (!in_lds) HIPCHECK(ctx->d_slab.ensure((size_t)grid * 3 * a.lw));
        a.slab = ctx->d_slab.p;
        launch_pile_build_annotate(a, grid, in_lds, s);
        ctx->tm.pile_launches = 5 + (n_medium ? 1 : 0) + (n_long ? 1 : 0);
    } else {
        std::vector<uint32_t> reads(n_reads);
        std::iota(reads.begin(), reads.end(), 0u);
        const int rc2 = run_position_kernel(ctx, a, reads);
        if (rc2 != RALA_HIP_OK) return rc2;
    }
    HIPCHECK(hipEventRecord(ctx->ev[kEvInitPilesDone], s));
    HIPCHECK(hipGetLastError());
    if (forked) HIPCHECK(hipStreamWaitEvent(s, ctx->ev[kEvInitDedupeDone], 0));

    launch_count_zero_u8(ctx->d_alive.p, n_reads, ctx->d_small.p + kInitDeadReads, s);
    uint32_t small[kSmallWords];
    HIPCHECK(d2h_small(ctx, small, ctx->d_small.p, sizeof(small), s));
    HIPCHECK(stream_sync(ctx, s));
    if (uploading) {
        HIPCHECK(hipStreamSynchronize(ctx->copy));
        upload_done(ctx);
    }
    const uint32_t slot_overflow = fixed ? small[kInitSlotOverflow] : 0;
    if (small[kInitNotedReads] && !slot_overflow) {
        const int rc_big = run_unbounded_piles(ctx, a, small[kInitNotedReads], ctx->d_small.p + kInitNotedReads);
        if (rc_big != RALA_HIP_OK) return rc_big;
        HIPCHECK(hipMemsetAsync(ctx->d_small.p + kInitDeadReads, 0, 4, s));
        launch_count_zero_u8(ctx->d_alive.p, n_reads, ctx->d_small.p + kInitDeadReads, s);
        const uint32_t noted = small[kInitNotedReads];
        HIPCHECK(d2h_small(ctx, small, ctx->d_small.p, sizeof(small), s));
        HIPCHECK(stream_sync(ctx, s));
        small[kInitNotedReads] = noted;
    }
    const uint32_t n_dead = small[kInitDeadReads];
    if (slot_overflow) {
        const int64_t keep = ctx->use_fixed_buckets;
        ctx->use_fixed_buckets = 0;
        const int rc_again = rala_hip_initialize(ctx);
        ctx->use_fixed_buckets = keep;
        return rc_again;
    }
// ... 454 lines not shown
```

rala_amd/hip.py:

```python
import ctypes
import os

import numpy as np

from . import build as _build

TYPE_X, TYPE_A, TYPE_B, TYPE_AB, TYPE_BA = range(5)
NO_READ = 0xFFFFFFFF
MEM_HOST, MEM_DEVICE, MEM_HOST_ASYNC = 0, 1, 2

ERRORS = {0: "OK", -1: "EDEVICE", -2: "EINVAL", -3: "ECAPACITY", -4: "EFILTERED", -5: "ENOMEM", -6: "ENOTAFILE", -7: "ETOOLARGE"}

LIB_PATH = os.path.join(os.path.dirname(os.path.abspath(__file__)), "csrc", "librala_hip.so")

SYMBOLS = (
    "rala_hip_create", "rala_hip_destroy", "rala_hip_last_error", "rala_hip_set_option", "rala_hip_stream",
    "rala_hip_set_reads", "rala_hip_set_overlaps", "rala_hip_initialize", "rala_hip_construct",
    "rala_hip_remove_transitive_edges", "rala_hip_tr_mark", "rala_hip_get_valid", "rala_hip_get_piles",
    "rala_hip_get_pile_data", "rala_hip_get_pile_row_digests", "rala_hip_get_pile_rows_info", "rala_hip_get_intervals", "rala_hip_get_overlaps", "rala_hip_get_graph_size",
    "rala_hip_get_graph", "rala_hip_get_timings", "rala_hip_get_num_prefiltered",
    "rala_hip_dedupe", "rala_hip_emit_bound_tuples", "rala_hip_set_bound_tuples", "rala_hip_import_state",
    "rala_hip_emit_bound_tuples_bucketed", "rala_hip_get_device_state", "rala_hip_import_state_device",
    "rala_hip_bound_records_fit", "rala_hip_emit_bound_records_bucketed", "rala_hip_set_bound_records",
    "rala_hip_copy_device_state", "rala_hip_layout", "rala_hip_layout_batch", "rala_hip_get_layout_info",
    "rala_hip_find_repetitive_hills",
    "rala_hip_mg_unique_id", "rala_hip_mg_local_group_create", "rala_hip_mg_local_group_destroy", "rala_hip_mg_create",
    "rala_hip_mg_create_contexts", "rala_hip_mg_join", "rala_hip_set_name_table", "rala_hip_set_overlaps_from_paf", "rala_hip_set_overlaps_from_mhap",
    "rala_hip_get_ingest_timings", "rala_hip_get_inflate_timings", "rala_hip_get_gzip_timings", "rala_hip_gzip_head", "rala_hip_gzip_chain", "rala_hip_gzip_chain_members", "rala_hip_gzip_find_members", "rala_hip_get_gzip_members", "rala_hip_bgzf_index", "rala_hip_get_overlap_columns", "rala_hip_tokenise_sensitive_paf",
    "rala_hip_bgzf_index_range", "rala_hip_bgzf_pieces_chain", "rala_hip_tokenise_sensitive", "rala_hip_mg_set_overlaps_from_mhap",
    "rala_hip_mg_set_overlaps_from_paf", "rala_hip_mg_get_slice",
    "rala_hip_index_sequences", "rala_hip_get_sequence_index", "rala_hip_get_sequence_timings",
    "rala_hip_build_name_table", "rala_hip_get_name_table", "rala_hip_copy_name_table", "rala_hip_name_hash",
    "rala_hip_get_name_table_info",
    "rala_hip_slice_sequences", "rala_hip_get_sequence_slice_info", "rala_hip_crc32_chain",
    "rala_hip_set_bases", "rala_hip_spell", "rala_hip_get_spell_info",
    "rala_hip_mg_destroy", "rala_hip_mg_last_error", "rala_hip_mg_set_reads", "rala_hip_mg_slice_cuts",
    "rala_hip_mg_set_overlaps", "rala_hip_mg_run", "rala_hip_mg_run_threads", "rala_hip_mg_context",
    "rala_hip_mg_owner_context",
    "rala_hip_mg_get_pile_data", "rala_hip_mg_get_pile_row_digests", "rala_hip_mg_get_timings",
)
COMM_RCCL, COMM_LOCAL = 0, 1


class OverlapsC(ctypes.Structure):
    _fields_ = [(n, ctypes.c_void_p) for n in
                ("a_id", "b_id", "a_begin", "a_end", "b_begin", "b_end", "length", "strand")]


class DeviceState(ctypes.Structure):
    _fields_ = [(n, ctypes.c_void_p) for n in ("begin", "end", "median", "p10", "alive", "n_pits", "n_hills", "slot",
                                               "pool")] + [("pool_count", ctypes.c_uint64), ("valid", ctypes.c_void_p)]


class Timings(ctypes.Structure):
    _fields_ = [(n, ctypes.c_float) for n in
                ("dedupe_ms", "bucket_ms", "pile_ms", "classify_ms", "death_ms", "finish_ms", "tail_host_ms",
                 "tr_ms", "total_ms")] + [("pile_launches", ctypes.c_uint32), ("death_rounds", ctypes.c_uint32),
                                  ("pile_overflow_reads", ctypes.c_uint32),
                                  ("pile_position_reads", ctypes.c_uint32),
                                  ("pile_unbounded_reads", ctypes.c_uint32), ("pool_regrown", ctypes.c_uint32),
                                  ("repeats_ms", ctypes.c_float)]

    def as_dict(self):
        return {n: getattr(self, n) for n, _ in self._fields_}


class MgTimings(ctypes.Structure):
    _fields_ = [(n, ctypes.c_float) for n in ("emit_ms", "exchange_ms", "owner_ms", "gather_ms", "construct_ms",
                                              "repeats_ms", "tr_ms", "total_ms")] + [("tuples_sent", ctypes.c_uint64)]

    def as_dict(self):
        return {n: getattr(self, n) for n, _ in self._fields_}


class IngestTimings(ctypes.Structure):
    _fields_ = [("ship_ms", ctypes.c_float), ("tokenize_ms", ctypes.c_float), ("bytes", ctypes.c_uint64), ("lines", ctypes.c_uint64)]

    def as_dict(self):
        return {n: getattr(self, n) for n, _ in self._fields_}


class GzipTimings(ctypes.Structure):
    _fields_ = [(n, ctypes.c_float) for n in ("find_ms", "decode_ms", "resolve_ms")] + [(n, ctypes.c_uint64) for n in (
        "compressed_bytes", "text_bytes", "chunks", "chunks_with_candidate", "chunks_confirmed", "chunks_refuted",
        "max_wave_text_bytes")]

    def as_dict(self):
        return {n: getattr(self, n) for n, _ in self._fields_}


class LayoutInfo(ctypes.Structure):
    _fields_ = [("components_fused_256", ctypes.c_uint32), ("components_fused_1024", ctypes.c_uint32),
                ("components_stepped", ctypes.c_uint32), ("components_empty", ctypes.c_uint32),
                ("points_fused_256", ctypes.c_uint64), ("points_fused_1024", ctypes.c_uint64),
                ("points_stepped", ctypes.c_uint64), ("step_tiles", ctypes.c_uint32), ("launches", ctypes.c_uint32),
                ("device_ms", ctypes.c_float)]


class NameTableInfo(ctypes.Structure):
    _fields_ = [("names", ctypes.c_uint64), ("distinct", ctypes.c_uint64), ("n_buckets", ctypes.c_uint64),
                ("longest_probe", ctypes.c_uint32), ("device_ms", ctypes.c_float)]

    def as_dict(self):
        return {n: getattr(self, n) for n, _ in self._fields_}


class SequenceSliceInfo(ctypes.Structure):
    _fields_ = [(n, ctypes.c_uint64) for n in ("windows", "max_window_text_bytes", "bases")] + [(n, ctypes.c_float) for n in (
        "ship_ms", "kernel_ms", "gather_ms", "copy_ms")]

    def as_dict(self):
        return {n: getattr(self, n) for n, _ in self._fields_}


class SpellInfo(ctypes.Structure):
    _fields_ = [(n, ctypes.c_uint64) for n in ("sources", "source_bytes", "spans", "bytes", "windows", "launches")] + [(n, ctypes.c_float) for n in (
        "upload_ms", "kernel_ms", "copy_ms")] + [("from_slice", ctypes.c_uint32)]

    def as_dict(self):
        return {n: getattr(self, n) for n, _ in self._fields_}


_lib = None


def name_hash(name):
    name = bytes(name)
    return int(lib().rala_hip_name_hash(ctypes.c_char_p(name), len(name)))


def lib(build=True):
    global _lib
    if _lib is None:
        path = LIB_PATH
        if build:
            path = _build.build_hip()
        if os.environ.get("RALA_HIP_LIB_AB"):
            path = os.environ["RALA_HIP_LIB_AB"]
        if not os.path.exists(path):
            raise RuntimeError("librala_hip.so is missing: run __graft_entry__.build()")
        L = ctypes.CDLL(path)
        vp, u64, u32, i32 = ctypes.c_void_p, ctypes.c_uint64, ctypes.c_uint32, ctypes.c_int
        L.rala_hip_create.argtypes = [i32, ctypes.POINTER(vp)]
        L.rala_hip_destroy.argtypes = [vp]
        L.rala_hip_destroy.restype = None
        L.rala_hip_last_error.argtypes = [vp]
        L.rala_hip_last_error.restype = ctypes.c_char_p
        L.rala_hip_set_option.argtypes = [vp, ctypes.c_char_p, ctypes.c_int64]
        L.rala_hip_stream.argtypes = [vp]
        L.rala_hip_stream.restype = vp
        L.rala_hip_set_reads.argtypes = [vp, vp, u64]
        L.rala_hip_set_overlaps.argtypes = [vp, ctypes.POINTER(OverlapsC), u64, i32]
        L.rala_hip_initialize.argtypes = [vp]
        L.rala_hip_construct.argtypes = [vp, ctypes.POINTER(OverlapsC), u64]
        L.rala_hip_remove_transitive_edges.argtypes = [vp, ctypes.POINTER(u32)]
        L.rala_hip_tr_mark.argtypes = [vp, u32, u32, vp, vp, vp, vp, ctypes.POINTER(u32)]
        L.rala_hip_get_valid.argtypes = [vp, vp]
        L.rala_hip_get_piles.argtypes = [vp, vp, vp, vp, vp, vp]
        L.rala_hip_get_pile_data.argtypes = [vp, u64, vp]
        L.rala_hip_get_pile_row_digests.argtypes = [vp, vp, vp, vp]
        L.rala_hip_get_pile_rows_info.argtypes = [vp, vp, vp]
        L.rala_hip_get_intervals.argtypes = [vp, i32, vp, vp, vp]
        L.rala_hip_get_overlaps.argtypes = [vp, i32, ctypes.POINTER(u64), vp, vp, vp, vp, vp, vp, vp]
        L.rala_hip_get_graph_size.argtypes = [vp, ctypes.POINTER(u64), ctypes.POINTER(u64)]
        L.rala_hip_get_graph.argtypes = [vp, vp, vp, vp, vp, vp]
        L.rala_hip_get_timings.argtypes = [vp, ctypes.POINTER(Timings)]
        L.rala_hip_get_num_prefiltered.argtypes = [vp, ctypes.POINTER(u64)]
        L.rala_hip_dedupe.argtypes = [vp]
        L.rala_hip_emit_bound_tuples.argtypes = [vp, vp]
        L.rala_hip_set_bound_tuples.argtypes = [vp, vp, u64, i32]
        L.rala_hip_import_state.argtypes = [vp] + [vp] * 11
        L.rala_hip_emit_bound_tuples_bucketed.argtypes = [vp, u32, vp, vp]
        L.rala_hip_get_device_state.argtypes = [vp, ctypes.POINTER(DeviceState)]
        L.rala_hip_import_state_device.argtypes = [vp, ctypes.POINTER(DeviceState)]
        L.rala_hip_copy_device_state.argtypes = [vp, ctypes.POINTER(DeviceState)]
        L.rala_hip_layout.argtypes = [vp, u32, vp, vp, vp, vp, u32, ctypes.c_double, ctypes.c_double, ctypes.c_double]
        L.rala_hip_layout_batch.argtypes = [vp, u32, vp, vp, vp, vp, vp, vp, u32, ctypes.c_double, ctypes.c_double]
        L.rala_hip_get_layout_info.argtypes = [vp, ctypes.POINTER(LayoutInfo)]
        L.rala_hip_find_repetitive_hills.argtypes = [vp, u64, u32, u32, ctypes.c_uint16, ctypes.c_uint16, ctypes.c_uint16]
        L.rala_hip_mg_unique_id.argtypes = [vp]
        L.rala_hip_mg_local_group_create.argtypes = [u32, ctypes.POINTER(vp)]
        L.rala_hip_mg_local_group_destroy.argtypes = [vp]
        L.rala_hip_mg_local_group_destroy.restype = None
        L.rala_hip_mg_create.argtypes = [i32, u32, u32, i32, vp, ctypes.POINTER(vp)]
        L.rala_hip_mg_create_contexts.argtypes = [i32, u32, u32, ctypes.POINTER(vp)]
        L.rala_hip_mg_join.argtypes = [vp, i32, vp]
        L.rala_hip_mg_destroy.argtypes = [vp]
        L.rala_hip_mg_destroy.restype = None
        L.rala_hip_mg_last_error.argtypes = [vp]
        L.rala_hip_mg_last_error.restype = ctypes.c_char_p
        L.rala_hip_mg_set_reads.argtypes = [vp, vp, u64]
        L.rala_hip_mg_slice_cuts.argtypes = [vp, vp, u64, u32, vp]
        L.rala_hip_mg_set_overlaps.argtypes = [vp, ctypes.POINTER(OverlapsC), u64, u64, i32]
        L.rala_hip_mg_run.argtypes = [vp, ctypes.POINTER(OverlapsC), u64, ctypes.POINTER(u32)]
        L.rala_hip_mg_run_threads.argtypes = [vp, u32, vp, vp, ctypes.POINTER(u32)]
        L.rala_hip_mg_context.argtypes = [vp]
        L.rala_hip_mg_context.restype = vp
        L.rala_hip_mg_owner_context.argtypes = [vp]
        L.rala_hip_mg_owner_context.restype = vp
        L.rala_hip_mg_get_pile_data.argtypes = [vp, u64, vp]
        L.rala_hip_mg_get_pile_row_digests.argtypes = [vp, vp, vp, vp]
        L.rala_hip_mg_get_timings.argtypes = [vp, ctypes.POINTER(MgTimings)]
        L.rala_hip_get_gzip_timings.argtypes = [vp, ctypes.POINTER(GzipTimings)]
        L.rala_hip_gzip_head.argtypes = [vp, u64, ctypes.POINTER(u64), ctypes.POINTER(i32)]
        L.rala_hip_index_sequences.argtypes = [vp, ctypes.c_char_p, i32, u32, ctypes.POINTER(u64), ctypes.POINTER(u64), ctypes.POINTER(i32)]
        L.rala_hip_get_sequence_index.argtypes = [vp] + [vp] * 6
        L.rala_hip_get_sequence_timings.argtypes = [vp, ctypes.POINTER(IngestTimings)]
        L.rala_hip_set_name_table.argtypes = [vp, vp, u64, vp, u64]
        L.rala_hip_build_name_table.argtypes = [vp, ctypes.POINTER(u64), ctypes.POINTER(u64)]
        L.rala_hip_get_name_table.argtypes = [vp, vp, vp, ctypes.POINTER(u64), ctypes.POINTER(u64)]
        L.rala_hip_copy_name_table.argtypes = [vp, vp]
        L.rala_hip_name_hash.argtypes = [vp, u64]
        L.rala_hip_name_hash.restype = u64
        L.rala_hip_get_name_table_info.argtypes = [vp, ctypes.POINTER(NameTableInfo)]
# ... 663 lines not shown
```

Before: 6.411 billion.

## Compute per-overlap resolvable bitmap and a-side counts in dedupe pass, skip id reloads

The fused count+dedupe kernel now writes a packed bitmap marking which overlaps are resolvable and accumulates per-read a-side counts using DPP wave-level run sums. The L1 scatter and query-side kernels then read this bitmap with vectorized column loads instead of re-reading a_id for filtering and recomputing counts. This cuts redundant global reads of the id columns and the per-element atomics, at the cost of a small extra bitmap buffer, more complex wave-chain logic, and extra atomics inside the dedupe kernel.

```diff
diff --git a/include/rala_hip.h b/include/rala_hip.h
--- a/include/rala_hip.h
+++ b/include/rala_hip.h
@@ -43,7 +43,9 @@
     uint32_t pile_launches, death_rounds, pile_overflow_reads, pile_position_reads;
     uint32_t pile_unbounded_reads, pool_regrown;
     float repeats_ms;
+    uint32_t bucket_path;
 } rala_hip_timings;
+enum { RALA_HIP_BUCKET_EXACT = 1, RALA_HIP_BUCKET_FIXED = 2, RALA_HIP_BUCKET_PARTITIONED = 3, RALA_HIP_BUCKET_PARTITIONED_IDS_ONCE = 4 };
 
 int rala_hip_create(int device, rala_hip_ctx** out);
 void rala_hip_destroy(rala_hip_ctx* ctx);
diff --git a/rala_amd/csrc/bucket_bits.h b/rala_amd/csrc/bucket_bits.h
--- /dev/null
+++ b/rala_amd/csrc/bucket_bits.h
@@ -0,0 +1,36 @@
+#pragma once
+#include <stdint.h>
+
+#if defined(__HIPCC__) || defined(__CUDACC__)
+#define RALA_BITS_FN __host__ __device__ __forceinline__
+#else
+#define RALA_BITS_FN inline
+#endif
+
+namespace rala_hip {
+
+RALA_BITS_FN uint64_t resolvable_words32(uint64_t n) { return 2 * ((n + 63) / 64); }
+RALA_BITS_FN uint64_t resolvable_word32(uint64_t i0) { return i0 >> 5; }
+RALA_BITS_FN uint32_t resolvable_shift(uint64_t i0) { return (uint32_t)(i0 & 31u); }
+RALA_BITS_FN uint32_t resolvable_nibble(uint32_t word32, uint64_t i0) { return (word32 >> resolvable_shift(i0)) & 0xFu; }
+RALA_BITS_FN uint32_t resolvable_place(uint32_t nibble, uint64_t i0) { return (nibble & 0xFu) << resolvable_shift(i0); }
+
+struct LaneRuns {
+    uint32_t head_mask, tail_mask, mid_mask;
+    uint32_t head_cnt, tail_cnt;
+    bool uniform;
+};
+RALA_BITS_FN uint32_t bits_count4(uint32_t m) { return (m & 1u) + ((m >> 1) & 1u) + ((m >> 2) & 1u) + ((m >> 3) & 1u); }
+RALA_BITS_FN LaneRuns lane_runs(uint32_t x0, uint32_t x1, uint32_t x2, uint32_t x3, uint32_t ok) {
+    const bool e1 = x1 == x0, e2 = x2 == x1, e3 = x3 == x2;
+    LaneRuns r;
+    r.uniform = e1 && e2 && e3;
+    r.head_mask = 1u | (e1 ? 2u : 0u) | (e1 && e2 ? 4u : 0u) | (r.uniform ? 8u : 0u);
+    r.tail_mask = 8u | (e3 ? 4u : 0u) | (e3 && e2 ? 2u : 0u) | (r.uniform ? 1u : 0u);
+    r.mid_mask = 0xFu & ~(r.head_mask | r.tail_mask);
+    r.head_cnt = bits_count4(r.head_mask & ok);
+    r.tail_cnt = bits_count4(r.tail_mask & ok);
+    return r;
+}
+
+}
diff --git a/rala_amd/csrc/bucket_kernels.hip b/rala_amd/csrc/bucket_kernels.hip
--- a/rala_amd/csrc/bucket_kernels.hip
+++ b/rala_amd/csrc/bucket_kernels.hip
@@ -2,6 +2,7 @@
 
 #include <algorithm>
 
+#include "bucket_bits.h"
 #include "device_utils.h"
 #include "geom.h"
 #include "kernels.h"
@@ -61,6 +62,64 @@
     return head ? len : 0u;
 }
 
+struct WaveChain {
+    bool cont, start;
+    uint32_t total, src, before;
+};
+__device__ __forceinline__ WaveChain wave_chain(const LaneRuns& r, uint32_t x0, uint32_t x3, uint32_t lane) {
+    WaveChain w;
+    const uint32_t prev = lane_above(x3);
+    w.cont = lane > 0 && prev == x0;
+    w.start = !(r.uniform && w.cont);
+    const uint32_t c = w.cont ? r.head_cnt : 0u, tail = w.start ? r.tail_cnt : 0u;
+    const uint32_t p = wave_scan_incl(c, OpAdd());
+    const uint64_t stop = __ballot(!w.cont || !r.uniform), conts = __ballot(w.cont), starts = __ballot(w.start);
+    const uint64_t after = lane == 63 ? 0ull : stop >> (lane + 1);
+    uint32_t last = 63u;
+    if (after) {
+        const uint32_t j = lane + (uint32_t)__ffsll((unsigned long long)after);
+        last = (conts >> j) & 1ull ? j : j - 1u;
+    }
+    w.total = tail + (uint32_t)__shfl((int)p, (int)last, 64) - p;
+    const uint64_t below = starts & ((1ull << lane) - 1ull);
+    w.src = below ? 63u - (uint32_t)__clzll((long long)below) : 0u;
+    w.before = (uint32_t)__shfl((int)(tail - p), (int)w.src, 64) + p - c;
+    return w;
+}
+
+struct ChainSums {
+    bool cont;
+    uint32_t in, out;
+};
+template <int kCtrl, int kRowMask>
+__device__ __forceinline__ void chain_step(uint32_t& v, uint32_t& reset) {
+    const uint32_t sv = dpp_from<kCtrl, kRowMask>(0u, v), sr = dpp_from<kCtrl, kRowMask>(0u, reset);
+    v = reset ? v : v + sv;
+    reset |= sr;
+}
+__device__ __forceinline__ ChainSums wave_chain_sums(const LaneRuns& r, uint32_t x0, uint32_t below_key, uint32_t lane) {
+    ChainSums c;
+    c.cont = lane > 0 && below_key == x0;
+    uint32_t reset = (!r.uniform || !c.cont) ? 1u : 0u;
+    uint32_t v = reset ? r.tail_cnt : r.head_cnt;
+    chain_step<0x111, 0xF>(v, reset);
+    chain_step<0x112, 0xF>(v, reset);
+    chain_step<0x114, 0xF>(v, reset);
+    chain_step<0x118, 0xF>(v, reset);
+    chain_step<0x142, 0xA>(v, reset);
+    chain_step<0x143, 0xC>(v, reset);
+    c.out = v;
+    const uint32_t below = lane_above(v);
+    c.in = lane > 0 ? below : 0u;
+    return c;
+}
+__device__ __forceinline__ uint32_t or_over_eight_lanes(uint32_t v) {
+    v |= dpp_from<0xB1, 0xF>(0u, v);
+    v |= dpp_from<0x4E, 0xF>(0u, v);
+    v |= dpp_from<0x141, 0xF>(0u, v);
+    return v;
+}
+
 constexpr uint32_t kBlockC = 1024;
 constexpr uint32_t kCountPer = 8;
 __global__ __launch_bounds__(kBlockC) void group_count_kernel(OvlSoA o, uint32_t n_reads, uint32_t g_lo, uint32_t n_groups, uint32_t* group_count) {
@@ -107,7 +166,8 @@
 __global__ __launch_bounds__(kBlockC) void group_count_dedupe_kernel(OvlSoA o, uint32_t n_reads, uint32_t n_groups, uint32_t* group_count,
                                                                      uint8_t* __restrict__ suspect, uint8_t* __restrict__ valid, uint32_t* list_pos,
                                                                      uint32_t* list_query, uint32_t list_cap, uint32_t* list_count,
-                                                                     uint32_t world, uint32_t groups) {
+                                                                     uint32_t world, uint32_t groups, uint32_t* __restrict__ resolvable,
+                                                                     uint32_t* acount) {
     extern __shared__ uint32_t s_hist[];
     __shared__ uint32_t s_fpos[kFlagStage], s_fq[kFlagStage], s_fcnt, s_fbase;
     for (uint32_t g = threadIdx.x; g < n_groups; g += kBlockC) s_hist[g] = 0;
@@ -131,10 +191,11 @@
 #pragma unroll
         for (uint32_t u = 0; u < kCountVec; ++u) {
             const uint64_t i0 = c0 + ((uint64_t)u * kBlockC + threadIdx.x) * 4;
-            uint32_t pa = (uint32_t)__shfl_up((int)a[u][3], 1, 64), pb = (uint32_t)__shfl_up((int)b[u][3], 1, 64);
+            uint32_t pa = lane_above(a[u][3]), pb = lane_above(b[u][3]);
+            const uint32_t below_a = pa;
             if (lane == 0 && i0 > 0 && i0 < o.n) { pa = o.a_id[i0 - 1]; pb = o.b_id[i0 - 1]; }
             bool have_prev = i0 > 0;
-            uint32_t word = 0;
+            uint32_t word = 0, okbits = 0;
 #pragma unroll
             for (uint32_t e = 0; e < 4; ++e) {
                 const uint32_t x = a[u][e], y = b[u][e];
@@ -158,10 +219,27 @@
                     }
                 }
                 if (ok && x != y) word |= 1u << (8 * e);
+                if (ok) okbits |= 1u << e;
                 pa = x; pb = y; have_prev = true;
             }
             if (i0 + 4 <= o.n) *(uint32_t*)(valid + i0) = word;
             else for (uint32_t e = 0; e < 4 && i0 + e < o.n; ++e) valid[i0 + e] = (uint8_t)(word >> (8 * e));
+            if constexpr (!kShard) {
+                if (resolvable) {
+                    const uint32_t half = or_over_eight_lanes(resolvable_place(okbits, i0));
+                    if ((lane & 7u) == 0 && i0 < o.n) resolvable[resolvable_word32(i0)] = half;
+                    const LaneRuns r = lane_runs(a[u][0], a[u][1], a[u][2], a[u][3], okbits);
+                    const ChainSums c = wave_chain_sums(r, a[u][0], below_a, lane);
+                    if (lane > 0 && !c.cont && c.in) atomicAdd(&acount[below_a], c.in);
+                    if (c.cont && !r.uniform && c.in + r.head_cnt) atomicAdd(&acount[a[u][0]], c.in + r.head_cnt);
+                    if (lane == 63 && c.out) atomicAdd(&acount[a[u][3]], c.out);
+                    if (!r.uniform) {
+                        if (!c.cont && r.head_cnt) atomicAdd(&acount[a[u][0]], r.head_cnt);
+                        if (r.mid_mask & okbits & 2u) atomicAdd(&acount[a[u][1]], 1u);
+                        if (r.mid_mask & okbits & 4u) atomicAdd(&acount[a[u][2]], 1u);
+                    }
+                }
+            }
         }
         __syncthreads();
         const uint32_t staged = s_fcnt;
@@ -296,6 +374,50 @@
         uint32_t leader;
         const uint32_t seg = segment_of(a, in[u], lane, leader);
         if (seg) atomicAdd(&acount[a], seg);
+    }
+    stage_and_copy(L, n_part, rec, bin, in, part_cursor, rec1, tmp);
+}
+
+template <bool kStream>
+__device__ __forceinline__ void load4_column(const uint32_t* p, uint64_t i0, uint64_t n, uint32_t fill, uint32_t (&out)[4]) {
+    typedef uint32_t u32x4_t __attribute__((ext_vector_type(4)));
+    if (i0 + 4 <= n) {
+        const u32x4_t v = kStream ? __builtin_nontemporal_load((const u32x4_t*)(p + i0)) : *(const u32x4_t*)(p + i0);
+        out[0] = v.x; out[1] = v.y; out[2] = v.z; out[3] = v.w;
+    } else {
+#pragma unroll
+        for (uint32_t e = 0; e < 4; ++e) out[e] = i0 + e < n ? p[i0 + e] : fill;
+    }
+}
+
+template <bool kStream>
+__global__ __launch_bounds__(kBlockP) void l1_scatter_vec_kernel(OvlSoA o, uint32_t n_part, uint32_t shift, const uint32_t* __restrict__ resolvable,
+                                                                 uint32_t* part_cursor, uint64_t* __restrict__ rec1) {
+    extern __shared__ __align__(16) unsigned char s_raw[];
+    __shared__ uint32_t tmp[kBlockP / 64 + 1];
+    StageLds L(s_raw, n_part);
+    uint64_t rec[kPer];
+    uint32_t bin[kPer];
+    bool in[kPer];
+    static_assert(kPer % 4 == 0, "whole groups of four per thread");
+    uint32_t b[kPer / 4][4], begin[kPer / 4][4], end[kPer / 4][4], bits[kPer / 4];
+#pragma unroll
+    for (uint32_t g = 0; g < kPer / 4; ++g) {
+        const uint64_t i0 = (uint64_t)blockIdx.x * kTile + ((uint64_t)g * kBlockP + threadIdx.x) * 4;
+        load4_column<kStream>(o.b_id, i0, o.n, 0u, b[g]);
+        load4_column<kStream>(o.b_begin, i0, o.n, 0u, begin[g]);
+        load4_column<kStream>(o.b_end, i0, o.n, 0u, end[g]);
+        bits[g] = i0 < o.n ? resolvable_nibble(resolvable[resolvable_word32(i0)], i0) : 0u;
+    }
+#pragma unroll
+    for (uint32_t g = 0; g < kPer / 4; ++g) {
+#pragma unroll
+        for (uint32_t e = 0; e < 4; ++e) {
+            const uint32_t u = g * 4 + e;
+            in[u] = (bits[g] >> e) & 1u;
+            rec[u] = pack_record(b[g][e], begin[g][e], end[g][e]);
+            bin[u] = in[u] ? b[g][e] >> shift : 0u;
+        }
     }
     stage_and_copy(L, n_part, rec, bin, in, part_cursor, rec1, tmp);
 }
@@ -478,6 +600,43 @@
     for (uint32_t u = 0; u < kQ; ++u) {
         const uint32_t at = (uint32_t)__shfl((int)base[u], (int)leader[u], 64);
         if (ok[u]) *(uint2*)(ev + ((size_t)at << ev_shift) + 2u * (lane - leader[u])) = make_uint2((begin[u] + 15u) << 1, ((end[u] - 15u) << 1) | 1u);
+    }
+}
+
+template <uint32_t kV, bool kStream>
+__global__ __launch_bounds__(256) void query_side_vec_kernel(OvlSoA o, const uint32_t* __restrict__ resolvable, const uint32_t* __restrict__ ev_off,
+                                                             uint32_t* written, uint32_t* __restrict__ ev, uint32_t ev_shift) {
+    const uint32_t lane = threadIdx.x & 63;
+    uint32_t a[kV][4], begin[kV][4], end[kV][4], bits[kV];
+#pragma unroll
+    for (uint32_t u = 0; u < kV; ++u) {
+        const uint64_t i0 = (((uint64_t)blockIdx.x * kV + u) * 256 + threadIdx.x) * 4;
+        load4_column<kStream>(o.a_id, i0, o.n, kInf, a[u]);
+        load4_column<kStream>(o.a_begin, i0, o.n, 0u, begin[u]);
+        load4_column<kStream>(o.a_end, i0, o.n, 0u, end[u]);
+        bits[u] = i0 < o.n ? resolvable_nibble(resolvable[resolvable_word32(i0)], i0) : 0u;
+    }
+    const uint32_t unit = 2u >> ev_shift;
+#pragma unroll
+    for (uint32_t u = 0; u < kV; ++u) {
+        const LaneRuns r = lane_runs(a[u][0], a[u][1], a[u][2], a[u][3], bits[u]);
+        const WaveChain w = wave_chain(r, a[u][0], a[u][3], lane);
+        uint32_t at_tail = 0, at_head = 0;
+        if (w.start && w.total) at_tail = ev_off[a[u][3]] + atomicAdd(&written[a[u][3]], unit * w.total);
+        if (!r.uniform && !w.cont && r.head_cnt) at_head = ev_off[a[u][0]] + atomicAdd(&written[a[u][0]], unit * r.head_cnt);
+        const uint32_t at_src = (uint32_t)__shfl((int)at_tail, (int)w.src, 64);
+        if (w.cont) at_head = at_src;
+        uint32_t head_rank = w.cont ? w.before : 0u, tail_rank = 0;
+        const uint32_t head_mask = r.uniform ? (w.cont ? 0xFu : 0u) : r.head_mask, tail_mask = r.uniform ? (w.cont ? 0u : 0xFu) : r.tail_mask;
+#pragma unroll
+        for (uint32_t e = 0; e < 4; ++e) {
+            if (!((bits[u] >> e) & 1u)) continue;
+            uint32_t at, rank = 0;
+            if ((head_mask >> e) & 1u) { at = at_head; rank = head_rank++; }
+            else if ((tail_mask >> e) & 1u) { at = at_tail; rank = tail_rank++; }
+            else at = ev_off[a[u][e]] + atomicAdd(&written[a[u][e]], unit);
+            *(uint2*)(ev + ((size_t)at << ev_shift) + 2u * (size_t)rank) = make_uint2((begin[u][e] + 15u) << 1, ((end[u][e] - 15u) << 1) | 1u);
+        }
     }
 }
 
@@ -679,6 +838,10 @@
 }
 }
 
+size_t resolvable_bitmap_words(uint64_t n_overlaps) { return (size_t)resolvable_words32(n_overlaps) + 2; }
+bool bucket_columns_vector(const OvlSoA& o) {
+    return (((uintptr_t)o.a_id | (uintptr_t)o.b_id | (uintptr_t)o.a_begin | (uintptr_t)o.a_end | (uintptr_t)o.b_begin | (uintptr_t)o.b_end) & 15u) == 0;
+}
 bool bucket_count_can_dedupe(const OvlSoA& o, const uint8_t* valid) {
     return (((uintptr_t)o.a_id | (uintptr_t)o.b_id) & 15u) == 0 && ((uintptr_t)valid & 3u) == 0 && getenv("RALA_DEDUPE_APART") == nullptr;
 }
@@ -706,7 +869,7 @@
     if (dedupe) {
         hipLaunchKernelGGL(group_count_dedupe_kernel<false>, dim3(std::min<uint32_t>(count_groups, chunks)), dim3(kBlockC), lds_count, s, o,
                            n_reads, window, B.group_count, dedupe->suspect, dedupe->valid, dedupe->list_pos,
-                           dedupe->list_query, dedupe->list_cap, dedupe->list_count, 1u, 0u);
+                           dedupe->list_query, dedupe->list_cap, dedupe->list_count, 1u, 0u, dedupe->resolvable, acount);
         if (dedupe->counted) {
             e = hipEventRecord(dedupe->counted, s);
             if (e != hipSuccess) return e;
@@ -724,13 +887,30 @@
     const uint32_t tiles1 = (uint32_t)((o.n + kTile - 1) / kTile);
     e = wait_for(dedupe ? dedupe->b_coords : nullptr);
     if (e != hipSuccess) return e;
-    hipLaunchKernelGGL(l1_scatter_kernel, dim3(tiles1), dim3(kBlockP), stage_lds_bytes(B.n_part), s, o, n_reads, B.n_part, B.shift, part_cursor, rec1,
-                       acount);
+    const uint32_t* resolvable = dedupe ? dedupe->resolvable : nullptr;
+    static const bool plain_loads = getenv("RALA_BUCKET_PLAIN_LOADS") != nullptr;
+    if (resolvable && plain_loads) {
+        hipLaunchKernelGGL(l1_scatter_vec_kernel<false>, dim3(tiles1), dim3(kBlockP), stage_lds_bytes(B.n_part), s, o, B.n_part, B.shift, resolvable,
+                           part_cursor, rec1);
+    } else if (resolvable) {
+        hipLaunchKernelGGL(l1_scatter_vec_kernel<true>, dim3(tiles1), dim3(kBlockP), stage_lds_bytes(B.n_part), s, o, B.n_part, B.shift, resolvable,
+                           part_cursor, rec1);
+    } else {
+        hipLaunchKernelGGL(l1_scatter_kernel, dim3(tiles1), dim3(kBlockP), stage_lds_bytes(B.n_part), s, o, n_reads, B.n_part, B.shift, part_cursor, rec1,
+                           acount);
+    }
     launch_partition_rest(B, n_reads, acount, rec1, rec2, ev_off, ev, s, ev_shift);
     e = wait_for(dedupe ? dedupe->a_coords : nullptr);
     if (e != hipSuccess) return e;
     static const int q_per = getenv("RALA_QUERY_PER") ? atoi(getenv("RALA_QUERY_PER")) : 2;
-    if (q_per == 4) hipLaunchKernelGGL(query_side_kernel<4>, dim3((uint32_t)((o.n + 1023) / 1024)), dim3(256), 0, s, o, n_reads, (const uint32_t*)ev_off, written, ev, ev_shift);
+    if (resolvable) {
+        static const int q_vec = getenv("RALA_QUERY_VEC") ? atoi(getenv("RALA_QUERY_VEC")) : 2;
+        const uint32_t per = q_vec == 1 ? 1024u : 2048u;
+        const dim3 grid((uint32_t)((o.n + per - 1) / per));
+        if (q_vec == 1) hipLaunchKernelGGL((query_side_vec_kernel<1, true>), grid, dim3(256), 0, s, o, resolvable, (const uint32_t*)ev_off, written, ev, ev_shift);
+        else if (plain_loads) hipLaunchKernelGGL((query_side_vec_kernel<2, false>), grid, dim3(256), 0, s, o, resolvable, (const uint32_t*)ev_off, written, ev, ev_shift);
+        else hipLaunchKernelGGL((query_side_vec_kernel<2, true>), grid, dim3(256), 0, s, o, resolvable, (const uint32_t*)ev_off, written, ev, ev_shift);
+    } else if (q_per == 4) hipLaunchKernelGGL(query_side_kernel<4>, dim3((uint32_t)((o.n + 1023) / 1024)), dim3(256), 0, s, o, n_reads, (const uint32_t*)ev_off, written, ev, ev_shift);
     else if (q_per == 2) hipLaunchKernelGGL(query_side_kernel<2>, dim3((uint32_t)((o.n + 511) / 512)), dim3(256), 0, s, o, n_reads, (const uint32_t*)ev_off, written, ev, ev_shift);
     else hipLaunchKernelGGL(query_side_kernel<1>, dim3((uint32_t)((o.n + 255) / 256)), dim3(256), 0, s, o, n_reads, (const uint32_t*)ev_off, written, ev, ev_shift);
     return hipGetLastError();
@@ -808,7 +988,7 @@
         if (dedupe) {
             hipLaunchKernelGGL(group_count_dedupe_kernel<true>, dim3(std::min<uint32_t>(count_groups, chunks)), dim3(kBlockC), lds_count, s, o,
                                n_reads, n_bins, group_count, dedupe->suspect, dedupe->valid, dedupe->list_pos, dedupe->list_query,
-                               dedupe->list_cap, dedupe->list_count, g.world, g.groups);
+                               dedupe->list_cap, dedupe->list_count, g.world, g.groups, (uint32_t*)nullptr, (uint32_t*)nullptr);
             if (dedupe->counted) {
                 e = hipEventRecord(dedupe->counted, s);
                 if (e != hipSuccess) return e;
diff --git a/rala_amd/csrc/context.h b/rala_amd/csrc/context.h
--- a/rala_amd/csrc/context.h
+++ b/rala_amd/csrc/context.h
@@ -191,6 +191,7 @@
     int64_t debug_chunk_fail = -1;
     uint32_t debug_part_shift = 0;
     uint32_t debug_count_window = 0;
+    bool debug_bucket_scalar_loads = false;
     bool use_bound_records = true;
     bool use_round_batches = true;
     rala_hip::DevBuf<uint32_t> d_round_log;
@@ -361,6 +362,7 @@
     int64_t use_fixed_buckets = 1;
     bool use_partitioned_buckets = true;
     rala_hip::DevBuf<uint32_t> d_bk_u32[3], d_bk_part, d_bk_group, d_bk_tiles;
+    rala_hip::DevBuf<uint32_t> d_bk_bits;
     rala_hip::DevBuf<uint64_t> d_bk_rec[2];
     bool host_state_fresh = false;
     uint32_t pool_used = 0;
diff --git a/rala_amd/csrc/context.hip b/rala_amd/csrc/context.hip
--- a/rala_amd/csrc/context.hip
+++ b/rala_amd/csrc/context.hip
@@ -184,6 +184,7 @@
     if (!strcmp(key, "pile_chunk_mb")) { ctx->pile_chunk_mb = (uint32_t)std::max<int64_t>(0, std::min<int64_t>(value, 1 << 20)); return RALA_HIP_OK; }
     if (!strcmp(key, "debug_ev_events")) { ctx->debug_ev_events = value != 0; return RALA_HIP_OK; }
     if (!strcmp(key, "debug_count_window")) { ctx->debug_count_window = (uint32_t)std::max<int64_t>(0, value); return RALA_HIP_OK; }
+    if (!strcmp(key, "debug_bucket_scalar_loads")) { ctx->debug_bucket_scalar_loads = value != 0; return RALA_HIP_OK; }
     if (!strcmp(key, "debug_part_shift")) { ctx->debug_part_shift = (uint32_t)std::max<int64_t>(0, value); return RALA_HIP_OK; }
     if (!strcmp(key, "debug_pile_variant")) { ctx->debug_pile_variant = (uint32_t)std::max<int64_t>(0, value); return RALA_HIP_OK; }
     if (!strcmp(key, "debug_dedupe_list_cap")) { ctx->debug_dedupe_list_cap = (uint32_t)std::max<int64_t>(0, value); return RALA_HIP_OK; }
diff --git a/rala_amd/csrc/kernels.h b/rala_amd/csrc/kernels.h
--- a/rala_amd/csrc/kernels.h
+++ b/rala_amd/csrc/kernels.h
@@ -344,8 +344,11 @@
     uint32_t* list_count;
     hipEvent_t counted;
     hipEvent_t ids = nullptr, b_coords = nullptr, a_coords = nullptr;
+    uint32_t* resolvable = nullptr;
 };
 bool bucket_count_can_dedupe(const OvlSoA& o, const uint8_t* valid);
+bool bucket_columns_vector(const OvlSoA& o);
+size_t resolvable_bitmap_words(uint64_t n_overlaps);
 constexpr uint32_t kBucketPairShift = 1;
 hipError_t launch_bucket_partitioned(const OvlSoA& o, uint32_t n_reads, const BucketTuning& bt, uint32_t* acount, uint32_t* written,
                                      uint32_t* part_cursor, uint32_t* group, uint32_t* tiles, uint64_t* rec1, uint64_t* rec2,
diff --git a/rala_amd/csrc/pipeline.hip b/rala_amd/csrc/pipeline.hip
--- a/rala_amd/csrc/pipeline.hip
+++ b/rala_amd/csrc/pipeline.hip
@@ -1978,6 +1978,7 @@
     const uint64_t n_bounds = from_blocks ? ctx->n_block_records : from_records ? ctx->n_records : 2 * ctx->n_ovl;
     const uint32_t ev_shift = !partitioned || (ctx->debug_ev_events && 2 * n_bounds < 0xFFFFFFF0ull) ? 0u : kBucketPairShift;
     bool fixed = !partitioned && ctx->use_run_kernel && ctx->use_fixed_buckets && (uint64_t)n_reads * slot * 4ull <= (64ull << 30);
+    ctx->tm.bucket_path = partitioned ? RALA_HIP_BUCKET_PARTITIONED : fixed ? RALA_HIP_BUCKET_FIXED : RALA_HIP_BUCKET_EXACT;
     static const bool dedupe_late = getenv("RALA_DEDUPE_LATE") != nullptr;
     const bool dedupe_early = forked && partitioned && !dedupe_late;
     const bool dedupe_counted = dedupe_early && !from_records && !from_blocks && bucket_count_can_dedupe(ctx->ovl, ctx->d_valid.p);
@@ -2016,6 +2017,12 @@
                                ctx->debug_dedupe_list_cap ? std::min(kMarks, ctx->debug_dedupe_list_cap) : kMarks,
                                ctx->d_small.p + kInitDedupeMarks, ctx->ev[kEvBucketCounted]};
             if (fine_upload) { bd.ids = ctx->ev_up[0]; bd.b_coords = ctx->ev_up[1]; bd.a_coords = ctx->ev_up[2]; }
+            const bool ids_once = dedupe_counted && !ctx->debug_bucket_scalar_loads && bucket_columns_vector(ctx->ovl);
+            if (ids_once) {
+                HIPCHECK(ctx->d_bk_bits.ensure(resolvable_bitmap_words(ctx->n_ovl)));
+                bd.resolvable = ctx->d_bk_bits.p;
+                ctx->tm.bucket_path = RALA_HIP_BUCKET_PARTITIONED_IDS_ONCE;
+            }
             HIPCHECK(launch_bucket_partitioned(ctx->ovl, n_reads, bt, ctx->d_bk_u32[0].p, ctx->d_bk_u32[2].p,
                                                ctx->d_bk_part.p, ctx->d_bk_group.p, ctx->d_bk_tiles.p, ctx->d_bk_rec[0].p,
                                                ctx->d_bk_rec[1].p, ctx->d_ev_off.p, ctx->d_ev.p, ctx->n_compute_units, fills, s,
diff --git a/rala_amd/hip.py b/rala_amd/hip.py
--- a/rala_amd/hip.py
+++ b/rala_amd/hip.py
@@ -8,6 +8,7 @@
 TYPE_X, TYPE_A, TYPE_B, TYPE_AB, TYPE_BA = range(5)
 NO_READ = 0xFFFFFFFF
 MEM_HOST, MEM_DEVICE, MEM_HOST_ASYNC = 0, 1, 2
+BUCKET_EXACT, BUCKET_FIXED, BUCKET_PARTITIONED, BUCKET_PARTITIONED_IDS_ONCE = 1, 2, 3, 4
 
 ERRORS = {0: "OK", -1: "EDEVICE", -2: "EINVAL", -3: "ECAPACITY", -4: "EFILTERED", -5: "ENOMEM", -6: "ENOTAFILE", -7: "ETOOLARGE"}
 
@@ -59,7 +60,7 @@
                                   ("pile_overflow_reads", ctypes.c_uint32),
                                   ("pile_position_reads", ctypes.c_uint32),
                                   ("pile_unbounded_reads", ctypes.c_uint32), ("pool_regrown", ctypes.c_uint32),
-                                  ("repeats_ms", ctypes.c_float)]
+                                  ("repeats_ms", ctypes.c_float), ("bucket_path", ctypes.c_uint32)]
 
     def as_dict(self):
         return {n: getattr(self, n) for n, _ in self._fields_}
```

Result: no change. 6.407 billion, median of 2 (-0.1%).
